# kkaytekin/Supervised-Depth-Estimation-from-Polarized-Images

Measured on AMD Instinct MI355X. Metric: train images/sec (512x612, 3-encoder), higher is better.
Workload: dtype f32; 1 GPU; BASELINE configs[2]: full 3-encoder (augment_xolp+augment_normals), multi-scale loss scales=[0,1,2,3], batch 16 per GPU, 512x612 frames (network/loss on 512x640 padded), dropout 0.1, Adam lr 1e-4, fp32; global_batch=16, height=512, width=640, frame_width=612, parallelism=dp1

## Files before the change

include/polardepth.h:

```cpp
#ifndef POLARDEPTH_H
#define POLARDEPTH_H

#include <stddef.h>
#include <stdint.h>

#ifdef __cplusplus
extern "C" {
#endif

#define PD_OK 0
#define PD_EINVAL (-22)
#define PD_ELAUNCH (-5)

const char* pd_last_error(void);
int pd_version(void);

#define PD_POLAR_LS 0
#define PD_POLAR_STOKES 1
#define PD_POLAR_PRECISE_NORMALS 1
#define PD_POLAR_IEEE_RHO 2
#define PD_POLAR_NT_LOADS 4
#define PD_POLAR_PLAIN_LOADS 8

size_t pd_polar_tables_bytes(int n_d, int n_s1, int n_s2);
int pd_polar_tables_pack(const double* x_d, const double* y_d, int n_d,
                         const double* x_s1, const double* y_s1, int n_s1,
                         const double* x_s2, const double* y_s2, int n_s2,
                         void* host_blob, size_t blob_bytes);
int pd_polar_tables_build(double n, void* host_blob, size_t blob_bytes, size_t* blob_bytes_used);

int pd_polar_fwd(const void* pol, const void* mask, void* xolp, void* xolp_std, void* normals,
                 void* ints, const void* tables, size_t tables_bytes,
                 int B, int H, int W, int Wout, int mode, int flags, void* stream);

int pd_polar_normals_from_xolp(const void* xolp, void* normals, const void* tables, size_t tables_bytes,
                               int B, int H, int W, int flags, void* stream);

int pd_polar_calc_normals(const void* phi, const void* theta, void* out, int B, long P, int phi_f64, int theta_f64,
                          void* stream);

int pd_polar_theta(const void* rho, void* theta_d, void* theta_s1, void* theta_s2, void* bins,
                   const void* tables, size_t tables_bytes, long n, void* stream);

int pd_polar_fit_matrix(const double angles_rad[4], double coef_out[12]);

#define PD_POLAR_U8 0
#define PD_POLAR_U16 1
#define PD_POLAR_F32 2
int pd_polar_general_fwd(const void* pol, int dtype, const double* coef, void* iun, void* xolp, void* xolp_std,
                         void* normals, const void* tables, size_t tables_bytes,
                         int B, int H, int W, int Wout, int flags, void* stream);

#define PD_XOLP_STATS_BYTES 4184
size_t pd_xolp_stats_workspace(int B, int H, int W);
int pd_xolp_stats(const void* xolp, const void* mask, void* stats, void* workspace, size_t ws_bytes,
                  int B, int H, int W, int ld, const float thresholds[2], int accumulate, void* stream);

#define PD_CONV_AUTO 0u
#define PD_CONV_FP32_MFMA 1u
#define PD_CONV_BF16X3 2u
#define PD_CONV_WGRAD_SPLIT_IN_REGS 4u
#define PD_CONV_GENERAL_KERNELS 8u
#define PD_CONV_X3_IM2COL 16u
#define PD_CONV_WGRAD_ROW_WORKGROUPS 32u
#define PD_CONV_BF16 128u
#define PD_CONV_FLAGS_ALL 191u
int pd_conv2d_tile_m(long M, int Cout);
long pd_conv2d_stats_rows(long M, int Cout);
int pd_conv2d_uses_x3(long M, int Cout, int C, int KH, int KW, int stride, int pad, int mode, int act, int has_out_scale,
                      int Ho, int Wo, unsigned flags);
int pd_conv2d_uses_bf16(long M, int Cout, int C, int KH, int KW, int stride, int pad, int mode, int act, int has_out_scale,
                        int Ho, int Wo, unsigned flags);
int pd_conv2d_route(long M, int Cout, int C, int KH, int KW, int stride, int pad, int mode, int act, int has_out_scale,
                    int Ho, int Wo, unsigned flags);
int pd_conv2d(const void* x, const void* w, const void* bias, const void* out_scale, void* y, void* stats,
              int N, int H, int W, int C, long sN, long sH, long sW, long sC,
              int Ho, int Wo, int Cout, int KH, int KW, int stride, int pad, int mode, int act,
              int affine, float sub, float div, long ldy, unsigned flags, void* stream);

int pd_conv16(const void* x, const void* w, const void* bias, void* y, int N, int H, int W, int C,
              long sN, long sH, long sW, int Ho, int Wo, int Cout, long ldy, int mode, int act, void* stream);

size_t pd_conv16_wgrad_workspace(int C);
int pd_conv16_wgrad(const void* x, const void* dz, void* dw, void* dbias, void* workspace, size_t ws_bytes,
                    int N, int H, int W, int C, long sN, long sH, long sW, long ldd, int accumulate, void* stream);

int pd_dgrad_s2_filters(const void* wt, void* wsub, int Cin, int Cout, void* stream);
int pd_conv2d_rect(const void* x, const void* w, void* y, int N, int H, int W, int C, long sN, long sH, long sW, long sC,
                   int Ho, int Wo, int Cout, int KH, int KW, int pad_h, int pad_w, int mode, long ldy, unsigned flags,
                   void* stream);
int pd_interleave4(const void* sub, void* dx, int N, int Ho, int Wo, int C, void* stream);

int pd_conv2d_add(const void* x, const void* w, const void* addend, long ld_add, void* y,
                  int N, int H, int W, int C, long sN, long sH, long sW, long sC,
                  int Ho, int Wo, int Cout, int KH, int KW, int stride, int pad, int mode, long ldy, unsigned flags,
                  void* stream);

size_t pd_conv2d_wgrad_workspace(long M, int Cout, int K, unsigned flags);
int pd_conv2d_wgrad(const void* x, const void* dy, void* dw, void* dbias, void* workspace, size_t ws_bytes,
                    int N, int H, int W, int C, long sN, long sH, long sW, long sC,
                    int Ho, int Wo, int Cout, int KH, int KW, int stride, int pad, int mode,
                    int affine, float sub, float div, long ldd, int accumulate, unsigned flags, void* stream);
int pd_conv2d_wgrad_uses_x3(long M, int Cout, int C, int KH, int KW, int stride, int pad, int mode, int H, int W, int Ho, int Wo,
                            unsigned flags);
int pd_conv2d_wgrad_uses_bf16(long M, int Cout, int C, int KH, int KW, int stride, int pad, int mode, int H, int W, int Ho, int Wo,
                              unsigned flags);
int pd_conv2d_wgrad_route(long M, int Cout, int C, int KH, int KW, int stride, int pad, int mode, int H, int W, int Ho, int Wo,
                          unsigned flags);

int pd_stem_s2d_input(const void* x, void* out, int N, int C, int H, int W, long sN, long sC, long sH, long sW,
                      int affine, float sub, float div, void* stream);
int pd_stem_s2d_weight(const void* w, void* w2, int Cout, int C, void* stream);
int pd_stem_s2d_weight_grad(const void* dw2, void* dw, int Cout, int C, int accumulate, void* stream);

int pd_weight_transpose(const void* w, void* wt, int Cout, int T, int Cin, void* stream);
int pd_weight_transpose_batched(const void* src, void* dst, const void* table, const void* blk, int n, int nblocks,
                                void* stream);

int pd_bn_fwd_finalize(const void* partial, long R, int C, double count, const void* gamma, const void* beta,
                       void* running_mean, void* running_var, float momentum, float eps, void* acc_ws, long acc_len,
                       void* scale, void* shift, void* save_mean, void* save_invstd, int training, void* stream);
int pd_bn_bwd_finalize(const void* partial, long R, int C, double count, void* acc_ws, long acc_len, void* dgamma,
                       void* dbeta, void* coef, int accumulate, void* stream);
long pd_chain_bwd_rows(int N, int H, int W, int C);
int pd_chain_fwd(const void* x, const void* scale, const void* shift, const void* res, void* out,
                 int N, int H, int W, int C, long ld_res, long ld_out, int relu_pre, int pool,
                 float drop_p, uint64_t seed, uint64_t offset, const void* step_state, int relu_post, void* stream);
int pd_chain_bwd_reduce(const void* dy, long ld_dy, const void* x, const void* out, long ld_out,
                        const void* scale, const void* shift, const void* mean, const void* invstd,
                        void* partial, int N, int H, int W, int C, int relu_pre, int pool, float drop_p,
                        uint64_t seed, uint64_t offset, const void* step_state, int relu_post, void* stream);
int pd_chain_bwd_apply(const void* dy, long ld_dy, const void* x, const void* out, long ld_out,
                       const void* scale, const void* shift, const void* mean, const void* invstd,
                       const void* coef, void* dx, void* dres, int N, int H, int W, int C, int relu_pre,
                       int pool, float drop_p, uint64_t seed, uint64_t offset, const void* step_state, int relu_post,
                       void* stream);

int pd_maxpool3s2_fwd(const void* x, void* y, void* idx, int N, int H, int W, int C, void* stream);
int pd_maxpool3s2_bwd(const void* idx, const void* dy, void* dx, int N, int H, int W, int C, void* stream);
int pd_maxpool3s2_bwd_add(const void* idx, const void* dy, const void* addend, long ld_add, void* dx, int N, int H, int W,
                          int C, void* stream);

int pd_upcat_fwd(const void* a, const void* skip, long ld_skip, void* out, int N, int H, int W, int Ca, int Cs,
                 void* stream);
int pd_up_bwd(const void* dout, long ld_d, void* da, int N, int H, int W, int Ca, void* stream);
int pd_up_bwd_elu(const void* dout, long ld_d, const void* elu_y, void* da, int N, int H, int W, int Ca, void* stream);

int pd_up2x_ac_fwd(const void* a, void* out, int N, int H, int W, int C, void* stream);
int pd_up2x_ac_bwd(const void* dout, void* da, int N, int H, int W, int C, void* stream);
int pd_relu_add(const void* x, const void* res, void* out, long n, int relu, void* stream);

int pd_act_bwd(const void* dy, const void* y, void* dz, long n, int act, void* stream);
int pd_reflect_fold(const void* dxp, void* dx, int N, int H, int W, int C, void* stream);
int pd_reflect_fold_pad(const void* dxp, void* dx, int N, int H, int W, int C, int pad, void* stream);
int pd_reflect_dgrad_border(const void* dz, long ldd, const void* w, void* dx, int N, int H, int W, int Cout, int Cin,
                            void* stream);
int pd_adam_step(void* p, void* g, void* m, void* v, long n, float lr, float beta1, float beta2, float eps,
                 float weight_decay, long step, const void* step_state, float grad_scale, int zero_grad, void* stream);
int pd_step_tick(void* step_state, int bump_dropout, int bump_adam, void* stream);
int pd_step_set_hyper(void* step_state, float lr, float grad_scale, void* stream);

int pd_loss_rows(long n);
int pd_disp_to_depth(const void* disp, void* depth, void* updisp, int N, int hs, int ws, int H, int W,
                     float min_depth, float max_depth, void* stream);
int pd_up_gather_bwd(const void* gup, void* gdisp, int N, int hs, int ws, int H, int W, int accumulate, int generic,
                     void* stream);
int pd_gt_normals(const void* gt, const void* K, void* gt_normals, int N, int H, int W, float min_depth, float max_depth,
                  void* stream);
int pd_sup_loss_fwd(const void* pred, const void* gt, const void* K, const void* gt_normals, void* partial, int N, int H,
                    int W, float min_depth, float max_depth, int with_normals, void* stream);
int pd_normals_loss_masked(const void* pred, const void* gt, const void* K, const void* mask, void* partial_ws, void* out,
                           int N, int H, int W, void* stream);
int pd_normals_pred_loss_fwd(const void* pred, long ld, const void* gt_normals, const void* gt, void* partial_ws, void* out,
                             int N, int H, int W, float min_depth, float max_depth, void* stream);
int pd_normals_pred_loss_bwd(const void* pred, long ld, const void* gt_normals, const void* gt, const void* gout,
                             const void* loss_count, void* dpred, long ld_dpred, int N, int H, int W, float min_depth,
                             float max_depth, void* stream);
int pd_multiscale_loss_fwd(const void* const* disps, const void* const* colors, const int* hs, const int* ws, int S,
                           const void* gt, const void* K, const void* gt_normals, void* const* depths, void* const* means,
                           void* const* edge_ws, void* sup_part, void* sm_part, int part_stride, int N, int H, int W,
                           float min_depth, float max_depth, int with_normals, void* stream);
int pd_multiscale_loss_bwd(const void* const* disps, const void* const* colors, const void* const* depths,
                           const void* const* means, const void* const* edge_ws, const int* hs, const int* ws, int S,
                           const void* gt, const void* K, const void* gt_normals, const void* wts, const void* sums,
                           void* gup_ws, void* g_ws, void* gd_acc, void* const* gdisps, int N, int H, int W,
                           float min_depth, float max_depth, void* stream);
int pd_sup_loss_bwd(const void* pred, const void* gt, const void* K, const void* gt_normals, const void* wts,
                    const void* sums, void* ab_ws, void* gout, int N, int H, int W, float min_depth, float max_depth,
                    int with_normals, int to_disp, int two_pass_form, void* stream);
int pd_smooth_fwd(const void* disp, const void* img, void* mean, void* partial, void* edge_w, int N, int h, int w,
                  void* stream);
int pd_smooth_bwd(const void* disp, const void* img, const void* mean, const void* wts, const void* edge_w, void* g_ws,
                  void* gd_acc, void* gdisp, int N, int h, int w, int accumulate, void* stream);
int pd_loss_finalize(const void* sup_part, const int* sup_rows, const void* sm_part, const int* sm_rows,
                     const int* dims, const int* scale_ids, int S, int part_stride, float w_normals,
                     float w_smooth, void* sums, void* vals, void* stream);
int pd_loss_from_sums(const void* sums, const int* dims, const int* scale_ids, int S, float w_normals,
                      float w_smooth, void* vals, void* stream);
int pd_loss_weights(const void* gvals, const int* scale_ids, int S, float w_normals, float w_smooth, void* wts,
                    void* stream);

int pd_ssim_fwd(const void* x, const void* y, void* out, int N, int C, int H, int W, int mode, int no_ssim,
                void* stream);
int pd_ssim_bwd(const void* x, const void* y, const void* gout, void* coef_ws, void* gx, void* gy, int N, int C, int H, int W,
                int mode, int no_ssim, void* stream);

#define PD_REPROJ_MAX_FRAMES 8
int pd_view_synth_fwd(const void* depth, const void* src, const void* K, const void* inv_K, const void* T, void* warped,
                      void* coords, int N, int C, int H, int W, void* stream);
int pd_view_synth_bwd(const void* gwarped, const void* src, const void* coords, const void* depth, const void* K,
                      const void* inv_K, const void* T, void* gdepth, int N, int C, int H, int W, int accumulate,
                      void* stream);
int pd_view_synth_pose_rows(int H, int W);
int pd_view_synth_bwd_pose(const void* gwarped, const void* src, const void* coords, const void* depth, const void* K,
                           const void* inv_K, const void* T, void* gdepth, void* partial_ws, void* gP, void* gT, int N, int C,
                           int H, int W, int accumulate, void* stream);
int pd_depth_to_updisp_bwd(const void* gdepth, const void* depth, void* gup, long n, float min_depth, float max_depth,
                           void* stream);
int pd_reproj_combine_rows(int N, int H, int W);
int pd_reproj_combine_fwd(const void* const* reproj, const void* const* identity, int F, const void* noise,
                          const void* valid, void* sel, void* partial_ws, void* sums, void* loss, int N, int H, int W,
                          int avg, void* stream);
int pd_reproj_combine_bwd(const void* gloss, const void* sel, const void* sums, const void* valid, void* const* greproj,
                          int F, int N, int H, int W, int avg, void* stream);

int pd_pose_matrix_fwd(const void* axisangle, const void* translation, void* T, int N, int invert, void* stream);
int pd_pose_matrix_bwd(const void* gT, const void* axisangle, const void* translation, void* gaxisangle, void* gtranslation,
                       int N, int invert, void* stream);
int pd_pose_head_fwd(const void* x, const void* w, const void* b, void* axisangle, void* translation, void* T, void* T_inv,
                     void* mean, int N, int h, int wd, int Cin, int Co, int invert, void* stream);
int pd_pose_head_bwd(const void* gT, const void* gT_inv, const void* gaxisangle, const void* gtranslation,
                     const void* axisangle, const void* translation, const void* w, const void* mean, void* gx, void* gw,
                     void* gb, void* gpre_ws, int N, int h, int wd, int Cin, int Co, int invert, int accumulate, void* stream);

int pd_cost_volume(const void* cur, const void* lookup, const void* T, const void* K, const void* inv_K, const void* bins,
                   const void* valid, void* cost, long ldc, void* missing, void* confidence, void* argmin, void* lowest,
                   int B, int F, int h, int w, int C, int D, int apply_confidence, void* stream);

#define PD_BINS_LINEAR 0
#define PD_BINS_INVERSE 1
int pd_student_masks_rows(int N, int h, int w);
int pd_student_masks(const void* lowest, const void* confidence, const void* mono_depth, const void* aug, int motion_masking,
                     void* rmask, void* cmask, void* lowest_up, void* minmax, void* partial_ws, int N, int h, int w, int H,
                     int W, void* stream);
int pd_depth_bins_update(const void* minmax, int N, void* tracker, double floor_depth, int D, int binning, void* bins,
                         void* stream);
int pd_student_combine_rows(int N, int H, int W);
int pd_student_combine_fwd(const void* const* reproj, int F, const void* valid, const void* rmask, const void* multi_depth,
                           const void* mono_depth, void* sel, void* partial_ws, void* sums, void* loss, int N, int H, int W,
                           int avg, void* stream);
int pd_student_combine_bwd(const void* gloss, const void* sel, const void* sums, const void* valid, const void* multi_depth,
                           const void* mono_depth, void* const* greproj, void* gmulti, int F, int N, int H, int W, int avg,
                           void* stream);

int pd_depth_metrics(const void* gt, const void* pred, const void* mask, int mask_value, void* partial_ws,
                     void* metrics, int N, long P, float min_depth, float max_depth, void* stream);

#define PD_NSTAT_BINS         720
#define PD_NSTAT_MAX_CLASSES  16
#define PD_NSTAT_RECORD_BYTES 2912
size_t pd_normals_stats_workspace(int N, int H, int W, int K);
int pd_normals_stats(const void* pred, long ld, const void* gtn, const void* gt, const void* mask,
                     const int* classes, int K, const void* cos_edges, int gate, void* err_deg,
                     void* stats, void* workspace, size_t ws_bytes, int N, int H, int W,
                     float min_depth, float max_depth, void* stream);

#define PD_PCD_TILE         256
#define PD_PCD_BINS         512
#define PD_PCD_MAX_CLASSES  16
#define PD_PCD_RECORD_BYTES 2096
// ... 82 lines not shown
```

supervised-depth-estimation-from-polarized-images_amd/csrc/conv.hip:

```cpp
#include "pd_common.h"
#include <cstdlib>
#include <type_traits>

namespace {

typedef float f32x16 __attribute__((ext_vector_type(16)));
typedef unsigned int u32x4 __attribute__((ext_vector_type(4)));

constexpr int BK = 32;
constexpr int LDT = BK;
constexpr int NT = 256;
constexpr unsigned OOB = 0x80000000u;

enum { MODE_ZERO = 0, MODE_REFLECT = 1, MODE_TRANSPOSED = 2 };
enum { ACT_NONE = 0, ACT_RELU = 1, ACT_ELU = 2, ACT_SIGMOID = 3 };

#define PD_I(n) std::integral_constant<int, n>{}
#define PD_SB __builtin_amdgcn_sched_barrier(0);

template <typename F> void with_mode(int mode, F&& f) {
    if (mode == MODE_ZERO) f(PD_I(MODE_ZERO)); else if (mode == MODE_REFLECT) f(PD_I(MODE_REFLECT)); else f(PD_I(MODE_TRANSPOSED));
}
template <typename F> void with_bool(bool b, F&& f) { if (b) f(std::true_type{}); else f(std::false_type{}); }

inline bool vec16_ok(const void* x, int C, long sN, long sH, long sW, long sC, int affine) {
    return (C % 4 == 0) && sC == 1 && (sW % 4 == 0) && (sH % 4 == 0) && (sN % 4 == 0) && !affine && pd::aligned16(x);
}

struct ConvArgs {
    const float* x;
    const float* w;
    const float* bias;
    const float* oscale;
    float* y;
    float* stats;
    const float* add;
    long ld_add;
    int N, H, W, C;
    long sN, sH, sW, sC;
    int Ho, Wo, Co;
    int KH, KW, stride, pad;
    int pad_w;
    int mode, act;
    int affine;
    float sub, div;
    int K;
    long M;
    long ldy;
    int mtiles, ntiles;
    int sshift;
    unsigned w_bytes;
    unsigned mg_hw, sh_hw, mg_wo, sh_wo;
    unsigned flags;
    int stats_rows;
    int nmajor;
};

__device__ __forceinline__ float4 ldg4(const float* p) { return *reinterpret_cast<const float4*>(p); }

__device__ __forceinline__ int swz(int row, int slot) { return 4 * (slot ^ ((row >> 1) & 7)); }

__device__ __forceinline__ __amdgpu_buffer_rsrc_t make_rsrc(const void* p, unsigned bytes) {
    return __builtin_amdgcn_make_buffer_rsrc(const_cast<void*>(p), 0, bytes, 0x00020000);
}
__device__ __forceinline__ float4 buf_ld4(__amdgpu_buffer_rsrc_t r, unsigned off) {
    return __builtin_bit_cast(float4, __builtin_amdgcn_raw_buffer_load_b128(r, off, 0, 0));
}
__device__ __forceinline__ float buf_ld1(__amdgpu_buffer_rsrc_t r, unsigned off) {
    return __builtin_bit_cast(float, __builtin_amdgcn_raw_buffer_load_b32(r, off, 0, 0));
}

template <int MODE>
__device__ __forceinline__ bool tap_in(int rh, int rw, int kh, int kw, int H, int W, int sshift, int& ih, int& iw) {
    if (MODE == MODE_TRANSPOSED) {
        const int th = rh - kh, tw = rw - kw;
        const int smask = (1 << sshift) - 1;
        ih = th >> sshift; iw = tw >> sshift;
        return ((th | tw) >= 0) & (((th | tw) & smask) == 0) & (ih < H) & (iw < W);
    }
    ih = rh + kh; iw = rw + kw;
    if (MODE == MODE_REFLECT) {
        ih = ih < 0 ? -ih : ih; ih = ih >= H ? 2 * H - 2 - ih : ih;
        iw = iw < 0 ? -iw : iw; iw = iw >= W ? 2 * W - 2 - iw : iw;
        return true;
    }
    return ((unsigned)ih < (unsigned)H) & ((unsigned)iw < (unsigned)W);
}

typedef __attribute__((address_space(3))) void lds_ptr_t;

__device__ __forceinline__ void dma16(__amdgpu_buffer_rsrc_t r, const void* lds_wave_base, unsigned voff) {
    const unsigned m0v = __builtin_amdgcn_readfirstlane((unsigned)(size_t)(lds_ptr_t*)lds_wave_base);
    asm volatile("s_mov_b32 m0, %0\n\ts_nop 0\n\tbuffer_load_dwordx4 %1, %2, 0 offen lds"
                 :: "s"(m0v), "v"(voff), "s"(r) : "memory");
}
__device__ __forceinline__ void dma_wait() { asm volatile("s_waitcnt vmcnt(0)" ::: "memory"); }

template <int BM, int BN, int WM, int WN, int MT, typename AccT>
__device__ __forceinline__ void conv_epilogue(const ConvArgs& a, AccT (&acc)[WM / MT][WN / MT], float* scratch, int mt,
                                              long m0, int n0, int wm, int wn, int lane, int wave, int tid) {
    constexpr int TM = WM / MT, TN = WN / MT, ACCN = MT == 32 ? 16 : 4, WAVES_N = BN / WN;
    float (*red)[WN][2] = reinterpret_cast<float (*)[WN][2]>(scratch);
    if constexpr (MT == 32 && WN == 32) {
        const bool lean = a.M - m0 >= BM && n0 + BN <= a.Co && !a.bias && !a.oscale && a.act == ACT_NONE &&
                          (a.ldy & 3) == 0 && ((size_t)a.y & 15) == 0 &&
                          (!a.add || ((a.ld_add & 3) == 0 && ((size_t)a.add & 15) == 0));
        if (lean) {
            float* T = scratch + wave * (WM * WN);
            red = reinterpret_cast<float (*)[WN][2]>(scratch + 4 * WM * WN);
            const int col_l = lane & 31, rbase = 4 * (lane >> 5);
            float4 addv[WM / 8];
            if (a.add) {
                const __amdgpu_buffer_rsrc_t ra = make_rsrc(a.add + m0 * a.ld_add, (unsigned)((long)BM * a.ld_add * 4));
                const unsigned off_a = (unsigned)((wm * WM + (lane >> 3)) * (int)a.ld_add + n0 + wn * WN + 4 * (lane & 7)) * 4u;
#pragma unroll
                for (int t = 0; t < WM / 8; ++t) addv[t] = buf_ld4(ra, off_a + (unsigned)(t * 8 * (int)a.ld_add * 4));
            }
            float s1 = 0.f, s2 = 0.f;
#pragma unroll
            for (int i = 0; i < TM; ++i)
#pragma unroll
                for (int r = 0; r < 16; ++r) {
                    const float v = acc[i][0][r];
                    T[(MT * i + (r & 3) + 8 * (r >> 2) + rbase) * WN + col_l] = v;
                    s1 += v;
                    s2 = __builtin_fmaf(v, v, s2);
                }
            const __amdgpu_buffer_rsrc_t ry = make_rsrc(a.y + m0 * a.ldy, (unsigned)((long)BM * a.ldy * 4));
            const unsigned off_l = (unsigned)((wm * WM + (lane >> 3)) * (int)a.ldy + n0 + wn * WN + 4 * (lane & 7)) * 4u;
            const float4* Tq = reinterpret_cast<const float4*>(T) + lane;
#pragma unroll
            for (int t = 0; t < WM / 8; ++t) {
                float4 v = Tq[t * 64];
                if (a.add) { v.x += addv[t].x; v.y += addv[t].y; v.z += addv[t].z; v.w += addv[t].w; }
                __builtin_amdgcn_raw_buffer_store_b128(__builtin_bit_cast(u32x4, v), ry, off_l, t * 8 * (int)a.ldy * 4, 0);
            }
            if (a.stats) {
                s1 += __shfl_xor(s1, 32); s2 += __shfl_xor(s2, 32);
                if (lane < 32) { red[wave][col_l][0] = s1; red[wave][col_l][1] = s2; }
                __syncthreads();
                if (tid < BN) {
                    const int w_n = tid / WN, cl = tid - w_n * WN;
                    float t1 = 0.f, t2 = 0.f;
#pragma unroll
                    for (int w_m = 0; w_m < BM / WM; ++w_m) {
                        t1 += red[w_m * WAVES_N + w_n][cl][0];
                        t2 += red[w_m * WAVES_N + w_n][cl][1];
                    }
                    float* o = a.stats + ((long)mt * a.Co + n0 + tid) * 2;
                    o[0] = t1; o[1] = t2;
                }
            }
            return;
        }
    }
    const int col_l = lane % MT;
    const int rbase = 4 * (lane / MT);
    {
        const long rows_left = a.M - m0;
        const int rows = rows_left < BM ? (int)rows_left : BM;
        const __amdgpu_buffer_rsrc_t ry = make_rsrc(a.y + m0 * a.ldy, (unsigned)((long)rows * a.ldy * 4));
        const __amdgpu_buffer_rsrc_t rb_ = make_rsrc(a.bias ? a.bias : a.w, a.bias ? (unsigned)a.Co * 4u : 0u);
        const __amdgpu_buffer_rsrc_t rs_ = make_rsrc(a.oscale ? a.oscale : a.w, a.oscale ? (unsigned)a.Co * 4u : 0u);
        const __amdgpu_buffer_rsrc_t ra_ = make_rsrc(a.add ? a.add + m0 * a.ld_add : a.w, a.add ? (unsigned)((long)rows * a.ld_add * 4) : 0u);
        auto body = [&](auto act_tag) {
            constexpr int ACT = decltype(act_tag)::value;
#pragma unroll
            for (int j = 0; j < TN; ++j) {
                const int col = n0 + wn * WN + MT * j + col_l;
                const bool cv = col < a.Co;
                const float bv = a.bias ? buf_ld1(rb_, cv ? (unsigned)col * 4u : OOB) : 0.f;
                const float sv = a.oscale ? buf_ld1(rs_, cv ? (unsigned)col * 4u : OOB) : 1.f;
                float s1 = 0.f, s2 = 0.f;
                const int row_l = wm * WM + rbase;
                const unsigned off_l = (unsigned)(row_l * (int)a.ldy + col) * 4u;
#pragma unroll
                for (int i = 0; i < TM; ++i) {
#pragma unroll
                    for (int r = 0; r < ACCN; ++r) {
                        const int rr = MT * i + (MT == 32 ? (r & 3) + 8 * (r >> 2) : r);
                        const bool ok = cv & (row_l < rows - rr);
                        float v = fmaf(acc[i][j][r], sv, bv);
                        const float vs = ok ? v : 0.f;
                        s1 += vs;
                        s2 += vs * vs;
                        if (ACT == ACT_RELU) v = fmaxf(v, 0.f);
                        else if (ACT == ACT_ELU) v = v > 0.f ? v : __builtin_amdgcn_exp2f(v * 1.44269504088896341f) - 1.f;
                        else if (ACT == ACT_SIGMOID) v = 1.f / (1.f + expf(-v));
                        if (a.add) v += buf_ld1(ra_, ok ? (unsigned)((row_l + rr) * (int)a.ld_add + col) * 4u : OOB);
                        __builtin_amdgcn_raw_buffer_store_b32(__builtin_bit_cast(unsigned, v), ry, ok ? off_l : OOB,
                                                              rr * (int)a.ldy * 4, 0);
                    }
                }
                if (a.stats) {
#pragma unroll
                    for (int m = MT; m < 64; m <<= 1) { s1 += __shfl_xor(s1, m); s2 += __shfl_xor(s2, m); }
                    if (lane < MT) { red[wave][MT * j + col_l][0] = s1; red[wave][MT * j + col_l][1] = s2; }
                }
            }
        };
        if (a.act == ACT_NONE) body(std::integral_constant<int, ACT_NONE>{});
        else if (a.act == ACT_RELU) body(std::integral_constant<int, ACT_RELU>{});
        else if (a.act == ACT_ELU) body(std::integral_constant<int, ACT_ELU>{});
        else body(std::integral_constant<int, ACT_SIGMOID>{});
    }
    if (a.stats) {
        __syncthreads();
        if (tid < BN) {
// ... 761 lines not shown
        const bool elu = a.act == ACT_ELU;
        const long rows_here = a.M - m0 < BM ? a.M - m0 : BM;
        const __amdgpu_buffer_rsrc_t ry = make_rsrc(a.y + m0 * a.ldy, (unsigned)(rows_here * a.ldy * 4));
        const __amdgpu_buffer_rsrc_t ra = make_rsrc(a.add ? a.add + m0 * a.ld_add : a.y, a.add ? (unsigned)(rows_here * a.ld_add * 4) : 0u);
#pragma unroll
        for (int j = 0; j < 2; ++j) {
            float4 addv[4 * RB];
            if (a.add) {
                const unsigned off_a = (unsigned)((RW * wave + (lane >> 3)) * (int)a.ld_add + n0 + 32 * j + 4 * (lane & 7)) * 4u;
#pragma unroll
                for (int t = 0; t < 4 * RB; ++t) addv[t] = buf_ld4(ra, off_a + (unsigned)(t * 8 * (int)a.ld_add * 4));
            }
            float s1 = 0.f, s2 = 0.f;
            const float bv = a.bias ? a.bias[n0 + 32 * j + col_l] : 0.f;
#pragma unroll
            for (int i = 0; i < RB; ++i)
#pragma unroll
                for (int r = 0; r < 16; ++r) {
                    const float v = (wsign ? -acc[i][j][r] : acc[i][j][r]) + bv;
                    T[(32 * i + (r & 3) + 8 * (r >> 2) + rbase) * 32 + col_l] =
                        elu ? (v > 0.f ? v : __builtin_amdgcn_exp2f(v * 1.44269504088896341f) - 1.f) : v;
                    s1 += v;
                    s2 = __builtin_fmaf(v, v, s2);
                }
            const unsigned off_l = (unsigned)((RW * wave + (lane >> 3)) * (int)a.ldy + n0 + 32 * j + 4 * (lane & 7)) * 4u;
            const float4* Tq = reinterpret_cast<const float4*>(T) + lane;
            float4 v[4 * RB];
#pragma unroll
            for (int t = 0; t < 4 * RB; ++t) {
                v[t] = Tq[t * 64];
                if (a.add) { v[t].x += addv[t].x; v[t].y += addv[t].y; v[t].z += addv[t].z; v[t].w += addv[t].w; }
            }
            __builtin_amdgcn_sched_barrier(0);
            if (rows_here == BM) {
#pragma unroll
                for (int t = 0; t < 4 * RB; ++t)
                    __builtin_amdgcn_raw_buffer_store_b128(__builtin_bit_cast(u32x4, v[t]), ry, off_l, t * 8 * (int)a.ldy * 4, 0);
            } else {
#pragma unroll
                for (int t = 0; t < 4 * RB; ++t)
                    if (RW * wave + (lane >> 3) + 8 * t < rows_here)
                        __builtin_amdgcn_raw_buffer_store_b128(__builtin_bit_cast(u32x4, v[t]), ry, off_l + (unsigned)(t * 8 * (int)a.ldy * 4), 0, 0);
            }
            asm volatile("s_nop 1");
            __builtin_amdgcn_sched_barrier(0);
            if (a.stats) {
                s1 += __shfl_xor(s1, 32); s2 += __shfl_xor(s2, 32);
                if (lane < 32) { red[wave][32 * j + col_l][0] = s1; red[wave][32 * j + col_l][1] = s2; }
            }
        }
        if (a.stats) {
            const int sgr = a.stats_rows, wps = sgr / RW, nrow = BM / sgr;
            __syncthreads();
            if (tid < nrow * BN) {
                const int row_l = tid >> 6, cl = tid & 63;
                float t1 = 0.f, t2 = 0.f;
                for (int w = 0; w < wps; ++w) { t1 += red[row_l * wps + w][cl][0]; t2 += red[row_l * wps + w][cl][1]; }
                float* o = a.stats + ((long)(mt * nrow + row_l) * a.Co + n0 + cl) * 2;
                o[0] = t1; o[1] = t2;
            }
        }
    }
}

constexpr long X3_MIN_WG = 512, X3_MIN_WG1 = 320;

static bool x3_common_ok(const ConvArgs& a, bool vec, bool has_scale) {
    const bool on = !(a.flags & PD_CONV_FP32_MFMA);
    return on && vec && a.KH * a.KW <= 31 && a.pad < a.KH && a.pad_w < a.KW &&
           (a.mode == MODE_ZERO || (a.mode == MODE_TRANSPOSED && a.sshift == 0) ||
            (a.mode == MODE_REFLECT && a.KH == 3 && a.KW == 3 && a.pad == 1 && a.pad_w == 1 && a.stride == 1 && a.Ho == a.H &&
             a.Wo == a.W && a.H >= 3 && a.W >= 3)) &&
           !has_scale && (a.act == ACT_NONE || a.act == ACT_ELU) && (a.ldy & 3) == 0 && ((size_t)a.y & 15) == 0 &&
           (!a.add || ((a.ld_add & 3) == 0 && ((size_t)a.add & 15) == 0)) && (long)a.Co * a.K * 4 < 0x7fffffffL;
}
static int x3_eligible(const ConvArgs& a) {
    const bool force = (a.flags & PD_CONV_BF16X3) != 0;
    if (!((a.C + x3::CK - 1) / x3::CK * x3::CK <= 2 * a.C && a.Co % x3::BN == 0 &&
          (a.M % 128 == 0 || (a.mode == MODE_TRANSPOSED && !a.stats))))
        return 0;
    const long ct = a.Co / x3::BN;
    if (a.M % 256 == 0 && (a.M / 256) * ct >= X3_MIN_WG) return 2;
    return (force || (a.M / 128) * ct >= X3_MIN_WG1) ? 1 : 0;
}

static int x3_nmajor(const ConvArgs& a, int ntiles) { return (long)a.Co * a.K * 4 > (3L << 20) && ntiles >= 8 && ntiles % 8 == 0; }
#include "conv_x3_halo.hpp"

enum ConvFamily { CONV_NONE = -1, CONV_GENERAL = 0, CONV_UNI = 1, CONV_X3 = 2, CONV_HALO = 3 };
struct ConvRoute {
    int family;
    int bm, bn, wm, wn;
    int mtiles, ntiles, nmajor;
    bool vec;
    int ns, rb;
    HaloPlan halo;
    int terms;
};

static ConvRoute route_conv(const ConvArgs& a, bool vec, bool has_scale) {
    ConvRoute r{};
    r.vec = vec; r.ns = 2; r.terms = 3;
    const auto tiles = [&](int family, int bm, int bn, int wm, int wn, long mtiles) {
        r.family = family; r.bm = bm; r.bn = bn; r.wm = wm; r.wn = wn;
        r.mtiles = (int)mtiles; r.ntiles = (a.Co + bn - 1) / bn;
    };
    if (x3_common_ok(a, vec, has_scale)) {
        if (!(a.flags & PD_CONV_X3_IM2COL) && x3_halo_plan(a, r.halo)) {
            tiles(CONV_HALO, 256, 32 * r.halo.ncb, 0, 0, (long)a.N * (a.Ho / (256 / r.halo.tw)) * (a.Wo / r.halo.tw));
            r.terms = (a.flags & PD_CONV_BF16) ? 1 : 3;
        } else if ((r.rb = x3_eligible(a)) != 0) {
            tiles(CONV_X3, 128 * r.rb, x3::BN, 32 * r.rb, x3::BN, (a.M + 128 * r.rb - 1) / (128 * r.rb));
        }
        if (r.rb || r.family == CONV_HALO) { r.nmajor = x3_nmajor(a, r.ntiles); return r; }
    }
    const int bm = pd_conv2d_tile_m(a.M, a.Co);
    const long mt = (a.M + bm - 1) / bm;
    if (a.Co == 96 && bm == 128) tiles(CONV_GENERAL, 128, 32, 32, 32, mt);
    else if (a.Co > 32 && bm == 128) tiles(CONV_GENERAL, 128, 64, 64, 32, mt);
    else if (a.Co > 32) tiles(CONV_GENERAL, 64, 64, 32, 32, mt);
    else if (a.Co > 16) tiles(CONV_GENERAL, 128, 32, 32, 32, mt);
    else tiles(CONV_GENERAL, 128, 16, 32, 16, mt);
    if (vec && !(a.flags & PD_CONV_GENERAL_KERNELS) && r.wn == 32 && a.C % BK == 0 && a.KH * a.KW <= 31 && a.pad < a.KH &&
        a.pad_w < a.KW && (a.mode == MODE_ZERO || a.mode == MODE_REFLECT || (a.mode == MODE_TRANSPOSED && a.sshift == 0))) {
        r.family = CONV_UNI;
        r.ns = (r.bm == 64 && a.mode != MODE_REFLECT) ? 3 : 2;
    } else if (a.pad_w != a.pad) {
        r.family = CONV_NONE;
    }
    return r;
}

template <int BM, int BN, int WM, int WN>
void launch_conv_fp32(const ConvArgs& a, const ConvRoute& r, dim3 grid, hipStream_t st) {
    const dim3 block(NT);
    constexpr bool dma = true;
    if constexpr (WN == 32)
        if (r.family == CONV_UNI) return with_mode(a.mode, [&](auto md) {
            constexpr int MD = decltype(md)::value;
            if (r.ns == 2) hipLaunchKernelGGL((conv_igemm_uni_kernel<BM, BN, WM, WN, MD, 2>), grid, block, 0, st, a);
            else if constexpr (MD != MODE_REFLECT) hipLaunchKernelGGL((conv_igemm_uni_kernel<BM, BN, WM, WN, MD, 3>), grid, block, 0, st, a);
        });
    with_mode(a.mode, [&](auto md) {
        constexpr int MD = decltype(md)::value;
        if (r.vec && dma) hipLaunchKernelGGL((conv_igemm_kernel<BM, BN, WM, WN, true, MD, true>), grid, block, 0, st, a);
        else if (r.vec) hipLaunchKernelGGL((conv_igemm_kernel<BM, BN, WM, WN, true, MD>), grid, block, 0, st, a);
        else hipLaunchKernelGGL((conv_igemm_kernel<BM, BN, WM, WN, false, MD>), grid, block, 0, st, a);
    });
}

static int launch_conv(ConvArgs& a, const ConvRoute& r, hipStream_t st) {
    a.mtiles = r.mtiles; a.ntiles = r.ntiles; a.nmajor = r.nmajor;
    const dim3 grid((unsigned)(((long)r.mtiles * r.ntiles + 7) / 8 * 8)), block(NT);
    if (r.family == CONV_HALO) {
        if (r.terms == 1) launch_conv_x3_halo<1>(a, r.halo, grid, st); else launch_conv_x3_halo<3>(a, r.halo, grid, st);
    } else if (r.family == CONV_X3) {
        with_mode(a.mode, [&](auto md) {
            constexpr int MD = decltype(md)::value;
            if (r.rb == 2) hipLaunchKernelGGL((conv_igemm_x3_kernel<MD, 2>), grid, block, 0, st, a);
            else hipLaunchKernelGGL((conv_igemm_x3_kernel<MD, 1>), grid, block, 0, st, a);
        });
    } else if (r.bn == 64 && r.bm == 128) launch_conv_fp32<128, 64, 64, 32>(a, r, grid, st);
    else if (r.bn == 64) launch_conv_fp32<64, 64, 32, 32>(a, r, grid, st);
    else if (r.bn == 32) launch_conv_fp32<128, 32, 32, 32>(a, r, grid, st);
    else launch_conv_fp32<128, 16, 32, 16>(a, r, grid, st);
    return pd::check_launch("pd_conv2d");
}

static void fill_conv_args(ConvArgs& a, int N, int H, int W, int C, long sN, long sH, long sW, long sC, int Ho, int Wo, int Co,
                           int KH, int KW, int stride, int pad, int pad_w, int mode, int act, int affine, float sub, float div,
                           long ldy, unsigned flags) {
    a.N = N; a.H = H; a.W = W; a.C = C; a.sN = sN; a.sH = sH; a.sW = sW; a.sC = sC;
    a.Ho = Ho; a.Wo = Wo; a.Co = Co; a.KH = KH; a.KW = KW; a.stride = stride; a.pad = pad; a.pad_w = pad_w;
    a.mode = mode; a.act = act; a.affine = affine; a.sub = sub; a.div = div;
    a.K = KH * KW * C; a.M = (long)N * Ho * Wo; a.ldy = ldy; a.flags = flags;
    a.sshift = 0;
    while ((1 << a.sshift) < stride) ++a.sshift;
    a.stats_rows = pd_conv2d_tile_m(a.M, Co);
    a.w_bytes = (unsigned)((long)Co * a.K * 4);
    const auto magic = [](long d, unsigned& mg, unsigned& sh) {
        if (d <= 1 || d >= (1L << 31)) { mg = 0; sh = 0; return; }
        int l = 0;
        while ((1L << l) < d) ++l;
        mg = (unsigned)((((unsigned long long)1 << (31 + l)) + (unsigned long long)d - 1) / (unsigned long long)d);
        sh = (unsigned)(l - 1);
    };
    magic((long)Ho * Wo, a.mg_hw, a.sh_hw);
    magic(Wo, a.mg_wo, a.sh_wo);
}
static bool conv_vec(const ConvArgs& a) { return vec16_ok(a.x, a.C, a.sN, a.sH, a.sW, a.sC, a.affine) && pd::aligned16(a.w); }

}

extern "C" int pd_conv2d_route(long M, int Co, int C, int KH, int KW, int stride, int pad, int mode, int act,
                               int has_out_scale, int Ho, int Wo, unsigned flags) {
    if (!pd::conv_flags_ok(flags)) flags &= ~PD_CONV_BF16;
    const bool grid = Ho > 0 && Wo > 0;
    const int H = grid ? Ho : 3, W = grid ? Wo : 3;
    ConvArgs a{};
    fill_conv_args(a, grid ? (int)(M / ((long)H * W)) : 1, H, W, C, (long)H * W * C, (long)W * C, C, 1, H, W, Co, KH, KW, stride, pad, pad,
                   mode, act, 0, 0.f, 1.f, Co, flags);
    a.M = M; a.stats_rows = pd_conv2d_tile_m(M, Co);
    const ConvRoute r = route_conv(a, conv_vec(a), has_out_scale != 0);
    return (r.family == CONV_HALO && r.terms == 1 ? 4 : r.family) | r.bn << 4 | r.bm << 12;
}

extern "C" int pd_conv2d_uses_x3(long M, int Co, int C, int KH, int KW, int stride, int pad, int mode, int act,
                                 int has_out_scale, int Ho, int Wo, unsigned flags) {
    const int r = pd_conv2d_route(M, Co, C, KH, KW, stride, pad, mode, act, has_out_scale, Ho, Wo, flags), family = r & 15;
    return family >= CONV_HALO ? 3 : family == CONV_X3 ? (r >> 12) / 128 : 0;
}

extern "C" int pd_conv2d_uses_bf16(long M, int Co, int C, int KH, int KW, int stride, int pad, int mode, int act,
                                   int has_out_scale, int Ho, int Wo, unsigned flags) {
    return (pd_conv2d_route(M, Co, C, KH, KW, stride, pad, mode, act, has_out_scale, Ho, Wo, flags) & 15) == 4 ? 3 : 0;
}

extern "C" int pd_conv2d_tile_m(long M, int Co) {
    if (Co <= 32) return 128;
    return M >= 64 * 1024 ? 128 : 64;
}

extern "C" long pd_conv2d_stats_rows(long M, int Co) {
    const int bm = pd_conv2d_tile_m(M, Co);
    return (M + bm - 1) / bm;
}

static int conv2d_impl(const void* x, const void* w, const void* bias, const void* out_scale, void* y, void* stats,
                       const void* addend, long ld_add,
                       int N, int H, int W, int C, long sN, long sH, long sW, long sC,
                       int Ho, int Wo, int Co, int KH, int KW, int stride, int pad, int mode, int act,
                       int affine, float sub, float div, long ldy, unsigned flags, void* stream, int pad_w = -1) {
    if (pad_w < 0) pad_w = pad;
    PD_REQUIRE(pd::conv_flags_ok(flags), "pd_conv2d: bad flags 0x%x", flags);
    PD_REQUIRE(x && w && y, "pd_conv2d: null tensor");
    PD_REQUIRE(N >= 0 && H > 0 && W > 0 && C > 0 && Ho > 0 && Wo > 0 && Co > 0, "pd_conv2d: bad dims");
    PD_REQUIRE(KH > 0 && KW > 0 && stride > 0 && pad >= 0, "pd_conv2d: bad filter geometry");
    PD_REQUIRE(mode >= 0 && mode <= 2 && act >= 0 && act <= 3, "pd_conv2d: bad mode/act");
    PD_REQUIRE(mode != MODE_REFLECT || (pad < H && pad < W), "pd_conv2d: reflect pad must be < input size");
    PD_REQUIRE(ldy >= Co && ldy < (1L << 22), "pd_conv2d: bad output row stride %ld (Cout=%d)", ldy, Co);
    if (mode == MODE_TRANSPOSED) {
        PD_REQUIRE((stride & (stride - 1)) == 0, "pd_conv2d: transposed mode needs a power-of-two stride");
        PD_REQUIRE(H <= (Ho + 2 * pad - KH) / stride + 1 && W <= (Wo + 2 * pad_w - KW) / stride + 1,
                   "pd_conv2d: transposed: x grid exceeds the forward output grid of a %dx%d input", Ho, Wo);
    } else {
        PD_REQUIRE(Ho <= (H + 2 * pad - KH) / stride + 1 && Wo <= (W + 2 * pad_w - KW) / stride + 1,
                   "pd_conv2d: output grid does not match input/filter geometry");
    }
    if (N == 0) return PD_OK;
    ConvArgs a;
    a.x = (const float*)x; a.w = (const float*)w; a.bias = (const float*)bias; a.oscale = (const float*)out_scale; a.y = (float*)y; a.stats = (float*)stats;
    a.add = (const float*)addend; a.ld_add = ld_add;
    fill_conv_args(a, N, H, W, C, sN, sH, sW, sC, Ho, Wo, Co, KH, KW, stride, pad, pad_w, mode, act, affine, sub, div, ldy, flags);
    PD_REQUIRE((long)Co * a.K * 4 < 0x7fffffffL, "pd_conv2d: weight tensor too large for 32-bit offsets");
    const long span = 256 / ((long)Ho * Wo) + 2;
    PD_REQUIRE(span * sN * 4 < 0x7fffffffL, "pd_conv2d: image too large for 32-bit offsets (%ld bytes per image)", sN * 4);
    const ConvRoute r = route_conv(a, conv_vec(a), out_scale != nullptr);
    if (r.family == CONV_NONE) return pd::fail(PD_EINVAL, "pd_conv2d_rect: shape outside the uniform-tap kernel (C %% 32, 16-byte aligned NHWC)");
    return launch_conv(a, r, (hipStream_t)stream);
}

extern "C" int pd_conv2d(const void* x, const void* w, const void* bias, const void* out_scale, void* y, void* stats,
                         int N, int H, int W, int C, long sN, long sH, long sW, long sC,
                         int Ho, int Wo, int Co, int KH, int KW, int stride, int pad, int mode, int act,
                         int affine, float sub, float div, long ldy, unsigned flags, void* stream) {
    return conv2d_impl(x, w, bias, out_scale, y, stats, nullptr, 0, N, H, W, C, sN, sH, sW, sC, Ho, Wo, Co, KH, KW, stride,
                       pad, mode, act, affine, sub, div, ldy, flags, stream);
}

extern "C" int pd_conv2d_add(const void* x, const void* w, const void* addend, long ld_add, void* y,
                             int N, int H, int W, int C, long sN, long sH, long sW, long sC,
                             int Ho, int Wo, int Co, int KH, int KW, int stride, int pad, int mode, long ldy, unsigned flags,
                             void* stream) {
    PD_REQUIRE(addend && ld_add >= Co, "pd_conv2d_add: bad addend");
    return conv2d_impl(x, w, nullptr, nullptr, y, nullptr, addend, ld_add, N, H, W, C, sN, sH, sW, sC, Ho, Wo, Co, KH, KW,
                       stride, pad, mode, ACT_NONE, 0, 0.f, 1.f, ldy, flags, stream);
}

extern "C" int pd_conv2d_rect(const void* x, const void* w, void* y, int N, int H, int W, int C, long sN, long sH, long sW,
                              long sC, int Ho, int Wo, int Co, int KH, int KW, int pad_h, int pad_w, int mode, long ldy,
                              unsigned flags, void* stream) {
    PD_REQUIRE(pad_w >= 0 && mode != MODE_REFLECT, "pd_conv2d_rect: bad padding / mode");
    PD_REQUIRE(!(flags & PD_CONV_GENERAL_KERNELS), "pd_conv2d_rect: the general kernel has no separate column padding");
    return conv2d_impl(x, w, nullptr, nullptr, y, nullptr, nullptr, 0, N, H, W, C, sN, sH, sW, sC, Ho, Wo, Co, KH, KW, 1,
                       pad_h, mode, ACT_NONE, 0, 0.f, 1.f, ldy, flags, stream, pad_w);
}

namespace {

constexpr int WG_K = 128;
constexpr int WG_MC = 32;
constexpr int WG_LDX = WG_K + 8;

struct WgradArgs {
    const float* x;
    const float* dy;
    float* part;
    float* bpart;
    int N, H, W, C;
    long sN, sH, sW, sC;
    int Ho, Wo, Co;
    int KH, KW, stride, pad, mode;
    int affine;
    float sub, div;
    int K;
    long M, ldd;
    long mper;
    int S, ktiles, ctiles;
};

template <int TCO, bool VEC, int MODE>
__global__ __launch_bounds__(NT) void conv_wgrad_kernel(const WgradArgs a) {
    constexpr int LDD = TCO + 8;
    constexpr int MT = TCO == 16 ? 16 : 32;
    constexpr int ACCN = MT == 32 ? 16 : 4;
    constexpr int WAVES_CO = TCO / MT;
    constexpr int WAVES_K = 4 / WAVES_CO;
    constexpr int TK = WG_K / WAVES_K / MT;
    constexpr int DY_ITERS = (WG_MC * TCO / 4 + NT - 1) / NT;
    constexpr int DY_PPR = TCO / 4;
    constexpr bool DY_ALL = WG_MC * TCO / 4 >= NT;
    __shared__ __attribute__((aligned(16))) float Ds[2][WG_MC][LDD];
    __shared__ __attribute__((aligned(16))) float Xs[2][WG_MC][WG_LDX];
    __shared__ int ktab[VEC ? 1 : WG_K][3];

    const int tid = threadIdx.x, lane = tid & 63, wave = tid >> 6;
    const int wm = wave / WAVES_K, wn = wave - wm * WAVES_K;
    const int nwg = a.ktiles * a.ctiles * a.S;
    int b = ((int)blockIdx.x & 7) * ((int)gridDim.x >> 3) + ((int)blockIdx.x >> 3);
    if (b >= nwg) return;
    const int kt = b % a.ktiles; b /= a.ktiles;
    const int ct = b % a.ctiles; b /= a.ctiles;
    const int s = b;
    const int co0 = ct * TCO, k0 = kt * WG_K;
    const long mbeg = (long)s * a.mper;
    const long mend = (mbeg + a.mper < a.M) ? mbeg + a.mper : a.M;
    const int nrows = (int)(mend - mbeg);
    const int nchunks = nrows > 0 ? (nrows + WG_MC - 1) / WG_MC : 0;
    const int hw = a.Ho * a.Wo;

    const int img0 = (int)(mbeg / hw);
    const long rest = ((long)a.N - img0) * a.sN * 4;
    const __amdgpu_buffer_rsrc_t rx = make_rsrc(a.x + (long)img0 * a.sN, rest > 0x7fffffffL ? 0x7fffffffu : (unsigned)rest);
    const long dbytes = (long)nrows * a.ldd * 4;
    const __amdgpu_buffer_rsrc_t rd = make_rsrc(a.dy + mbeg * a.ldd, dbytes > 0 ? (unsigned)dbytes : 0u);

    int vkh = 0, vkw = 0, vc = 0; bool vkv = false;
    if (VEC) {
        const int k = k0 + 4 * (tid & 31);
        vkv = k < a.K;
        const int tap = k / a.C;
        vc = k - tap * a.C; vkh = tap / a.KW; vkw = tap - vkh * a.KW;
    } else {
        if (tid < WG_K) {
            const int k = k0 + tid;
            const int tap = k / a.C;
            const int kh = tap / a.KW;
            ktab[tid][0] = k < a.K ? kh : -1; ktab[tid][1] = tap - kh * a.KW; ktab[tid][2] = (k - tap * a.C) * (int)a.sC;
        }
        __syncthreads();
    }
    constexpr int XR = VEC ? 4 : 1;
    int rb[XR], rloc[XR];
    int roh[XR], row_[XR];
    for (int i = 0; i < XR; ++i) {
        rloc[i] = VEC ? (tid >> 5) + 8 * i : (tid >> 3);
        const int m = (int)(mbeg - (long)img0 * hw) + rloc[i];
        const int n = m / hw;
        const int rem = m - n * hw;
        roh[i] = rem / a.Wo; row_[i] = rem - roh[i] * a.Wo;
        rb[i] = n * (int)a.sN;
    }
    constexpr bool INC = VEC && MODE == MODE_ZERO;
    int xih[INC ? XR : 1], xiw[INC ? XR : 1], xoff[INC ? XR : 1];
    const int c_w = WG_MC * a.stride, c_wo = c_w * (int)a.sW;
    const int c_row = a.Wo * a.stride, c_rowo = a.stride * (int)a.sH - c_row * (int)a.sW;
    const int c_img = a.Ho * a.stride, c_imgo = (int)a.sN - c_img * (int)a.sH;
    if (INC) {
        for (int i = 0; i < XR; ++i) {
            xih[i] = roh[i] * a.stride - a.pad + vkh;
            xiw[i] = row_[i] * a.stride - a.pad + vkw;
            xoff[i] = rb[i] + xih[i] * (int)a.sH + xiw[i] * (int)a.sW + vc;
        }
    }
    auto advance = [&](int i) {
        rloc[i] += WG_MC;
        row_[i] += WG_MC;
        if (INC) { xiw[i] += c_w; xoff[i] += c_wo; }
        while (row_[i] >= a.Wo) {
            row_[i] -= a.Wo;
            if (INC) { xiw[i] -= c_row; xih[i] += a.stride; xoff[i] += c_rowo; }
            if (++roh[i] == a.Ho) {
                roh[i] = 0; rb[i] += (int)a.sN;
                if (INC) { xih[i] -= c_img; xoff[i] += c_imgo; }
            }
        }
    };

    float4 pd[DY_ITERS], px[VEC ? 4 : 1];
    float sx[VEC ? 1 : 16];

    auto load_chunk = [&](int q) {
        const int rbase = q * WG_MC;
#pragma unroll
        for (int i = 0; i < DY_ITERS; ++i) {
            const int r = rbase + tid / DY_PPR + (NT / DY_PPR) * i;
            const int co = co0 + 4 * (tid % DY_PPR);
            const unsigned off = (unsigned)(r * (int)a.ldd + co) * 4u;
            if (!DY_ALL && tid >= WG_MC * DY_PPR) {
                pd[i] = make_float4(0.f, 0.f, 0.f, 0.f);
            } else if ((a.Co & 3) == 0) {
                pd[i] = buf_ld4(rd, (r < nrows && co < a.Co) ? off : OOB);
            } else {
                float4 v;
                v.x = buf_ld1(rd, (r < nrows && co < a.Co) ? off : OOB);
                v.y = buf_ld1(rd, (r < nrows && co + 1 < a.Co) ? off + 4 : OOB);
                v.z = buf_ld1(rd, (r < nrows && co + 2 < a.Co) ? off + 8 : OOB);
                v.w = buf_ld1(rd, (r < nrows && co + 3 < a.Co) ? off + 12 : OOB);
                pd[i] = v;
            }
        }
        if (VEC) {
#pragma unroll
            for (int i = 0; i < 4; ++i) {
                if (INC) {
                    const bool ok = ((unsigned)xih[i] < (unsigned)a.H) & ((unsigned)xiw[i] < (unsigned)a.W) & vkv & (rloc[i] < nrows);
                    px[i] = buf_ld4(rx, ok ? (unsigned)xoff[i] * 4u : OOB);
                } else {
                    int ih, iw;
// ... 600 lines not shown
                    fa[g][blk][t] = *reinterpret_cast<const u32x4*>(lds_c + pa_off + (BUF * P_BYTES + (unsigned)((t * 2 + g) * 2) * 1024u + blk * 512u));
#pragma unroll
        for (int e = 0; e < 8; ++e) x1[e] = *reinterpret_cast<const float*>(lds_c + fx_off + (BUF * X_BYTES + (unsigned)(8 + e) * 2 * X_ROW));
#pragma unroll
        for (int e = 0; e < 8; ++e) dv[e] = *reinterpret_cast<const float*>(lds_c + sd_off + (NXT * D_BYTES + (unsigned)e * 2 * D_ROW));
        x3::Terms t0, t1, td;
        auto mm = [&](const x3::Terms& t, auto g_tag, auto n_tag) {
            constexpr int G = decltype(g_tag)::value, N = decltype(n_tag)::value, T = N / 2, BLK = N % 2;
            const unsigned* bv = T < 3 ? t.h : T < 5 ? t.m : t.l;
            const u32x4 av = T == 0 ? fa[G][BLK][0] : T == 1 ? fa[G][BLK][1] : T == 2 ? fa[G][BLK][2] : T == 3 ? fa[G][BLK][0] : T == 4 ? fa[G][BLK][1] : fa[G][BLK][0];
            acc[BLK] = __builtin_amdgcn_mfma_f32_32x32x16_bf16(bf(av), bf(u32x4{bv[0], bv[1], bv[2], bv[3]}), acc[BLK], 0, 0, 0);
        };
        x3::sp_h<0>(x0, t0); x3::sp_h<1>(x0, t0); x3::sp_h<2>(x0, t0); x3::sp_h<3>(x0, t0);
        PD_SB
#define PD_XP(j) if constexpr (SPREAD) load_x_piece(nxt, PD_I(j));
#define PD_DP(j) if constexpr (SPREAD) load_d_piece(buf_tag, PD_I(j));
        mm(t0, PD_I(0), PD_I(0)); x3::sp_m<0>(x0, t0); PD_XP(0) PD_SB
        mm(t0, PD_I(0), PD_I(1)); x3::sp_m<1>(x0, t0); PD_XP(1) PD_SB
        mm(t0, PD_I(0), PD_I(2)); x3::sp_m<2>(x0, t0); PD_XP(2) PD_SB
        mm(t0, PD_I(0), PD_I(3)); x3::sp_m<3>(x0, t0); PD_XP(3) PD_SB
        mm(t0, PD_I(0), PD_I(4)); x3::sp_h<0>(dv, td); x3::sp_h<1>(dv, td); x3::sp_h<2>(dv, td); x3::sp_h<3>(dv, td); PD_DP(0) PD_SB
        mm(t0, PD_I(0), PD_I(5)); x3::sp_m<0>(dv, td); PD_DP(1) PD_SB
#undef PD_XP
#undef PD_DP
        mm(t0, PD_I(0), PD_I(6)); x3::sp_l<0>(t0); x3::sp_h<0>(x1, t1); PD_SB
        mm(t0, PD_I(0), PD_I(7)); x3::sp_l<1>(t0); x3::sp_h<1>(x1, t1); PD_SB
        mm(t0, PD_I(0), PD_I(8)); x3::sp_l<2>(t0); x3::sp_h<2>(x1, t1); PD_SB
        mm(t0, PD_I(0), PD_I(9)); x3::sp_l<3>(t0); x3::sp_h<3>(x1, t1); PD_SB
        mm(t0, PD_I(0), PD_I(10)); x3::sp_m<1>(dv, td); PD_SB
        mm(t0, PD_I(0), PD_I(11)); x3::sp_m<2>(dv, td); PD_SB
        mm(t1, PD_I(1), PD_I(0)); x3::sp_m<0>(x1, t1); PD_SB
        mm(t1, PD_I(1), PD_I(1)); x3::sp_m<1>(x1, t1); PD_SB
        mm(t1, PD_I(1), PD_I(2)); x3::sp_m<2>(x1, t1); PD_SB
        mm(t1, PD_I(1), PD_I(3)); x3::sp_m<3>(x1, t1); PD_SB
        mm(t1, PD_I(1), PD_I(4)); x3::sp_m<3>(dv, td); PD_SB
        mm(t1, PD_I(1), PD_I(5)); x3::sp_l<0>(td); x3::sp_l<1>(td); PD_SB
        mm(t1, PD_I(1), PD_I(6)); x3::sp_l<0>(t1); PD_SB
        mm(t1, PD_I(1), PD_I(7)); x3::sp_l<1>(t1); PD_SB
        mm(t1, PD_I(1), PD_I(8)); x3::sp_l<2>(t1); PD_SB
        mm(t1, PD_I(1), PD_I(9)); x3::sp_l<3>(t1); PD_SB
        mm(t1, PD_I(1), PD_I(10)); x3::sp_l<2>(td); x3::sp_l<3>(td); PD_SB
        mm(t1, PD_I(1), PD_I(11));
        if constexpr (BIAS) bsum += ((dv[0] + dv[1]) + (dv[2] + dv[3])) + ((dv[4] + dv[5]) + (dv[6] + dv[7]));
        *reinterpret_cast<u32x4*>(lds_c + sp_off + (NXT * P_BYTES + 0 * 4096u)) = u32x4{td.h[0], td.h[1], td.h[2], td.h[3]};
        *reinterpret_cast<u32x4*>(lds_c + sp_off + (NXT * P_BYTES + 1 * 4096u)) = u32x4{td.m[0], td.m[1], td.m[2], td.m[3]};
        *reinterpret_cast<u32x4*>(lds_c + sp_off + (NXT * P_BYTES + 2 * 4096u)) = u32x4{td.l[0], td.l[1], td.l[2], td.l[3]};
        dma_wait();
        __syncthreads();
    };

    {
        const std::integral_constant<unsigned, 0> d0{};
        const std::integral_constant<unsigned, 1> d1{};
        load_x_all(d0);
        load_d(d0);
        load_d(d1);
        dma_wait();
        __syncthreads();
        split_d(d0);
        __syncthreads();
    }
    for (int q = 0; q < nchunks; q += 2) {
        chunk(std::integral_constant<unsigned, 0>{});
        if (q + 1 < nchunks) chunk(std::integral_constant<unsigned, 1>{});
        if ((q & (FLUSH - 2)) == FLUSH - 2) flush();
    }
    flush();

#pragma unroll
    for (int blk = 0; blk < 2; ++blk) {
        const int k = k0 + wave * 32 + fi;
#pragma unroll
        for (int r = 0; r < 16; ++r) {
            const int co = co0 + 32 * blk + (r & 3) + 8 * (r >> 2) + 4 * fk;
            if (co < a.Co && k < a.K) a.part[((long)s * a.Co + co) * a.K + k] = acc_sum[blk][r];
        }
    }
    if constexpr (BIAS) {
        if (do_bias) {
            float* red = smem_all;
            red[wave * 64 + lane] = bsum;
            __syncthreads();
            if (tid < 64 && co0 + tid < a.Co) a.bpart[(long)s * a.Co + co0 + tid] = (red[tid] + red[64 + tid]) + (red[128 + tid] + red[192 + tid]);
        }
    }
}

#include "conv_wgrad_halo.hpp"
#include "conv_wgrad_roll.hpp"

__global__ __launch_bounds__(256) void reduce_rows_kernel(const float* __restrict__ part, float* __restrict__ out,
                                                          int S, long n, int accumulate) {
    __shared__ float red[4][64];
    const int col = threadIdx.x & 63, sl = threadIdx.x >> 6;
    const long i = blockIdx.x * 64L + col;
    float a0 = 0.f, a1 = 0.f, a2 = 0.f, a3 = 0.f;
    if (i < n) {
        int j = sl;
        for (; j + 12 < S; j += 16) {
            a0 += part[(long)j * n + i];
            a1 += part[(long)(j + 4) * n + i];
            a2 += part[(long)(j + 8) * n + i];
            a3 += part[(long)(j + 12) * n + i];
        }
        for (; j < S; j += 4) a0 += part[(long)j * n + i];
    }
    red[sl][col] = (a0 + a1) + (a2 + a3);
    __syncthreads();
    if (sl == 0 && i < n) {
        const float s = (red[0][col] + red[1][col]) + (red[2][col] + red[3][col]);
        out[i] = accumulate ? out[i] + s : s;
    }
}

__global__ __launch_bounds__(256) void weight_transpose_kernel(const float* __restrict__ w, float* __restrict__ wt,
                                                               int Co, int T, int Ci) {
    const long n = (long)Co * T * Ci;
    for (long i = blockIdx.x * 256L + threadIdx.x; i < n; i += (long)gridDim.x * 256) {
        const int co = (int)(i % Co);
        const long r = i / Co;
        const int t = (int)(r % T);
        const int ci = (int)(r / T);
        wt[i] = w[((long)co * T + t) * Ci + ci];
    }
}

__global__ __launch_bounds__(256) void weight_transpose_batched_kernel(const float* __restrict__ src, float* __restrict__ dst,
                                                                       const int* __restrict__ table,
                                                                       const int* __restrict__ blk, int n) {
    __shared__ float tile[32][33];
    int lo = 0, hi = n;
    while (hi - lo > 1) {
        const int mid = (lo + hi) >> 1;
        if (blk[mid] <= (int)blockIdx.x) lo = mid; else hi = mid;
    }
    const int off = table[4 * lo], Co = table[4 * lo + 1], T = table[4 * lo + 2], Ci = table[4 * lo + 3];
    const float* w = src + off;
    float* wt = dst + off;
    int lb = (int)blockIdx.x - blk[lo];
    const int tiles_ci = (Ci + 31) >> 5, tiles_co = (Co + 31) >> 5;
    const int ci0 = (lb % tiles_ci) << 5; lb /= tiles_ci;
    const int co0 = (lb % tiles_co) << 5;
    const int t = lb / tiles_co;
    const int x = threadIdx.x & 31, y = threadIdx.x >> 5;
#pragma unroll
    for (int r = y; r < 32; r += 8)
        if (co0 + r < Co && ci0 + x < Ci) tile[r][x] = w[((long)(co0 + r) * T + t) * Ci + ci0 + x];
    __syncthreads();
#pragma unroll
    for (int r = y; r < 32; r += 8)
        if (ci0 + r < Ci && co0 + x < Co) wt[((long)(ci0 + r) * T + t) * Co + co0 + x] = tile[x][r];
}

inline int wgrad_tco(int Co) { return Co > 32 ? 64 : (Co > 16 ? 32 : 16); }

inline bool wgrad_x3c_enabled(unsigned flags) { return !(flags & (PD_CONV_FP32_MFMA | PD_CONV_WGRAD_SPLIT_IN_REGS)); }
inline bool wgrad_x3_on(unsigned flags) { return (flags & PD_CONV_WGRAD_SPLIT_IN_REGS) && !(flags & PD_CONV_FP32_MFMA); }

void wgrad_plan(long M, int Co, int K, unsigned flags, int* S, long* mper) {
    const int tco = wgrad_tco(Co);
    const long tiles = (long)((Co + tco - 1) / tco) * ((K + WG_K - 1) / WG_K);
    const bool x3c = tco == 64 && wgrad_x3c_enabled(flags) && !(flags & PD_CONV_GENERAL_KERNELS);
    const long total = x3c ? (512 / tiles < 4 ? 1536 : M >= (1L << 20) ? 1024 : 512) : (tiles <= 32 ? 768 : 1536);
    long s = total / tiles;
    const long smax = (M + 511) / 512;
    if (s > smax) s = smax;
    if (s < 1) s = 1;
    long per = (M + s - 1) / s;
    per = (per + WG_MC - 1) / WG_MC * WG_MC;
    s = (M + per - 1) / per;
    if (s < 1) s = 1;
    *S = (int)s; *mper = per;
}

inline bool wgrad_halo_enabled(unsigned flags) { return wgrad_x3c_enabled(flags) && !(flags & (PD_CONV_GENERAL_KERNELS | PD_CONV_X3_IM2COL)); }

static int wgrad_rows_cap(long M, int Co, int K, unsigned flags) {
    int S; long mper;
    wgrad_plan(M, Co, K, flags, &S, &mper);
    if (!wgrad_halo_enabled(flags)) return S;
    const long own = std::min<long>(std::max(wgrad_halo_slices_bound(Co, K), wgrad_roll_slices_bound(Co, K)), (M + 63) / 64);
    return S > own ? S : (int)own;
}

enum WgradFamily { WGRAD_GENERAL = 0, WGRAD_UNI, WGRAD_UNI_X3, WGRAD_X3C, WGRAD_HALO, WGRAD_ROLL };
struct WgradRoute {
    int family;
    int rows;
    int tco, S; long mper;
    bool vec, row8;
    int nb, nbw;
    bool bf16;
    WgradHaloPlan halo;
    WgradRollPlan roll;
};

static WgradRoute route_wgrad(const WgradArgs& a, bool vec, unsigned flags) {
    WgradRoute r{};
    r.vec = vec; r.tco = wgrad_tco(a.Co);
    wgrad_plan(a.M, a.Co, a.K, flags, &r.S, &r.mper);
    r.rows = r.S;
    const bool refl_ok = a.mode == MODE_REFLECT && a.pad == 1 && a.KH == 3 && a.KW == 3 && a.stride == 1 && a.Ho == a.H && a.Wo == a.W && a.H >= 3;
    if (!(a.mode == MODE_ZERO || refl_ok)) return r;
    if (wgrad_halo_enabled(flags) && wgrad_halo_eligible(a, vec)) {
        r.bf16 = (flags & PD_CONV_BF16) != 0;
        const int cap = wgrad_rows_cap(a.M, a.Co, a.K, flags);
        if (!(flags & PD_CONV_WGRAD_ROW_WORKGROUPS) && wgrad_roll_eligible(a, vec, cap, r.roll)) {
            r.family = WGRAD_ROLL; r.rows = r.roll.S;
        } else {
            r.family = WGRAD_HALO; wgrad_halo_plan(a, cap, r.halo); r.rows = r.halo.S * r.halo.rps;
        }
        return r;
    }
    r.nb = (a.pad + a.stride - 1) / a.stride; r.nbw = (r.nb + 1) / 2;
    if (!(flags & PD_CONV_GENERAL_KERNELS) && (r.tco == 64 || r.tco == 32) && vec && a.Co % 4 == 0 && a.Wo % 2 == 0 && a.ldd % 4 == 0 &&
        a.Ho >= 2 * r.nb && a.Wo >= 4 * r.nbw && a.Wo >= 14 && (2 * r.nb + 1) * (2 * r.nbw + 1) <= 31 && r.mper % WG_MC == 0 &&
        a.M % 4 == 0 && a.K >= 4) {
        r.family = r.tco == 32 ? WGRAD_UNI : wgrad_x3c_enabled(flags) ? WGRAD_X3C : wgrad_x3_on(flags) ? WGRAD_UNI_X3 : WGRAD_UNI;
        r.row8 = a.Wo % 8 == 0 && r.mper % 8 == 0 && a.M % 8 == 0;
    }
    return r;
}

static int launch_wgrad_slices(const WgradArgs& a, const WgradRoute& r, bool bias, hipStream_t st) {
    const dim3 grid((unsigned)(((long)a.ktiles * a.ctiles * a.S + 7) / 8 * 8)), block(NT);
    const bool reflect = a.mode == MODE_REFLECT;
    if (r.family == WGRAD_GENERAL) {
        const auto gen = [&](auto tco) { with_bool(r.vec, [&](auto v) { with_bool(reflect, [&](auto refl) {
            hipLaunchKernelGGL((conv_wgrad_kernel<decltype(tco)::value, decltype(v)::value, decltype(refl)::value ? MODE_REFLECT : MODE_ZERO>), grid, block, 0, st, a);
        }); }); };
        if (r.tco == 64) gen(PD_I(64)); else if (r.tco == 32) gen(PD_I(32)); else gen(PD_I(16));
        return PD_OK;
    }
    WgradUniArgs ua; ua.g = a; ua.nb = r.nb; ua.nbw = r.nbw;
    if (r.family == WGRAD_X3C) {
        static const hipError_t lds_ok = [] {
            hipError_t e = hipSuccess;
            for (const void* f : {reinterpret_cast<const void*>(conv_wgrad_x3c_kernel<true, true>), reinterpret_cast<const void*>(conv_wgrad_x3c_kernel<false, true>),
                                  reinterpret_cast<const void*>(conv_wgrad_x3c_kernel<true, false>), reinterpret_cast<const void*>(conv_wgrad_x3c_kernel<false, false>),
                                  reinterpret_cast<const void*>(conv_wgrad_x3c_kernel<true, false, true>), reinterpret_cast<const void*>(conv_wgrad_x3c_kernel<false, false, true>)}) {
                const hipError_t rc = hipFuncSetAttribute(f, hipFuncAttributeMaxDynamicSharedMemorySize, x3c::LDS_BYTES);
                if (rc != hipSuccess) e = rc;
            }
            return e;
        }();
        PD_REQUIRE(lds_ok == hipSuccess, "pd_conv2d_wgrad: cannot reserve %u bytes of LDS", x3c::LDS_BYTES);
        with_bool(bias, [&](auto b) {
            constexpr bool B = decltype(b)::value;
            if (reflect) hipLaunchKernelGGL((conv_wgrad_x3c_kernel<B, false, true>), grid, block, x3c::LDS_BYTES, st, ua);
            else if (r.row8) hipLaunchKernelGGL((conv_wgrad_x3c_kernel<B, true>), grid, block, x3c::LDS_BYTES, st, ua);
            else hipLaunchKernelGGL((conv_wgrad_x3c_kernel<B, false>), grid, block, x3c::LDS_BYTES, st, ua);
        });
    } else if (r.tco == 32) {
        with_bool(reflect, [&](auto refl) { hipLaunchKernelGGL((conv_wgrad_uni_kernel<decltype(refl)::value, true, 32>), grid, block, 0, st, ua); });
    } else {
        with_bool(reflect, [&](auto refl) { with_bool(bias, [&](auto b) {
            constexpr bool R = decltype(refl)::value, B = decltype(b)::value;
            if (r.family == WGRAD_UNI_X3) hipLaunchKernelGGL((conv_wgrad_uni_kernel<R, B, 64, true>), grid, block, 0, st, ua);
            else hipLaunchKernelGGL((conv_wgrad_uni_kernel<R, B>), grid, block, 0, st, ua);
        }); });
    }
    return PD_OK;
}

static void fill_wgrad_args(WgradArgs& a, int N, int H, int W, int C, long sN, long sH, long sW, long sC, int Ho, int Wo, int Co,
                            int KH, int KW, int stride, int pad, int mode, int affine, float sub, float div, long ldd) {
    a.N = N; a.H = H; a.W = W; a.C = C; a.sN = sN; a.sH = sH; a.sW = sW; a.sC = sC;
    a.Ho = Ho; a.Wo = Wo; a.Co = Co; a.KH = KH; a.KW = KW; a.stride = stride; a.pad = pad; a.mode = mode;
    a.affine = affine; a.sub = sub; a.div = div;
    a.K = KH * KW * C; a.M = (long)N * Ho * Wo; a.ldd = ldd;
}

}

extern "C" size_t pd_conv2d_wgrad_workspace(long M, int Co, int K, unsigned flags) {
    const size_t rows = (size_t)wgrad_rows_cap(M, Co, K, flags);
    return (rows * Co * K + rows * Co) * sizeof(float);
}

extern "C" int pd_conv2d_wgrad_route(long M, int Co, int C, int KH, int KW, int stride, int pad, int mode, int H, int W, int Ho,
                                     int Wo, unsigned flags) {
    if (Ho <= 0 || Wo <= 0) return 1 << 4;
    if (!pd::conv_flags_ok(flags)) flags &= ~PD_CONV_BF16;
    WgradArgs a{};
    fill_wgrad_args(a, std::max(1, (int)(M / ((long)Ho * Wo))), H, W, C, (long)H * W * C, (long)W * C, C, 1, Ho, Wo, Co, KH, KW, stride,
                    pad, mode, 0, 0.f, 1.f, Co);
    a.M = M;
    const WgradRoute r = route_wgrad(a, vec16_ok(a.x, C, a.sN, a.sH, a.sW, a.sC, a.affine), flags);
    const int code = r.family == WGRAD_ROLL ? 3 : r.family == WGRAD_HALO ? 2 : r.family == WGRAD_X3C ? 1 : 0;
    return code | (r.bf16 ? 4 : 0) | r.rows << 4;
}

extern "C" int pd_conv2d_wgrad_uses_x3(long M, int Co, int C, int KH, int KW, int stride, int pad, int mode, int H, int W, int Ho,
                                       int Wo, unsigned flags) {
    return pd_conv2d_wgrad_route(M, Co, C, KH, KW, stride, pad, mode, H, W, Ho, Wo, flags) & 3;
}

extern "C" int pd_conv2d_wgrad_uses_bf16(long M, int Co, int C, int KH, int KW, int stride, int pad, int mode, int H, int W, int Ho,
                                         int Wo, unsigned flags) {
    const int r = pd_conv2d_wgrad_route(M, Co, C, KH, KW, stride, pad, mode, H, W, Ho, Wo, flags);
    return r & 4 ? r & 3 : 0;
}

extern "C" int pd_conv2d_wgrad(const void* x, const void* dy, void* dw, void* dbias, void* workspace, size_t ws_bytes,
                               int N, int H, int W, int C, long sN, long sH, long sW, long sC,
                               int Ho, int Wo, int Co, int KH, int KW, int stride, int pad, int mode,
                               int affine, float sub, float div, long ldd, int accumulate, unsigned flags, void* stream) {
    PD_REQUIRE(x && dy && dw && workspace, "pd_conv2d_wgrad: null tensor");
    PD_REQUIRE(pd::conv_flags_ok(flags), "pd_conv2d_wgrad: bad flags 0x%x", flags);
    PD_REQUIRE(mode == MODE_ZERO || mode == MODE_REFLECT, "pd_conv2d_wgrad: mode must be 0 or 1");
    PD_REQUIRE(Ho <= (H + 2 * pad - KH) / stride + 1 && Wo <= (W + 2 * pad - KW) / stride + 1,
               "pd_conv2d_wgrad: output grid does not match input/filter geometry");
    PD_REQUIRE(ldd >= Co && (ldd % 4 == 0 || Co < 4) , "pd_conv2d_wgrad: bad dy row stride");
    if (N == 0) return PD_OK;
    WgradArgs a;
    a.x = (const float*)x; a.dy = (const float*)dy;
    fill_wgrad_args(a, N, H, W, C, sN, sH, sW, sC, Ho, Wo, Co, KH, KW, stride, pad, mode, affine, sub, div, ldd);
    const size_t need = pd_conv2d_wgrad_workspace(a.M, Co, a.K, flags);
    PD_REQUIRE(ws_bytes >= need, "pd_conv2d_wgrad: workspace too small (%zu < %zu)", ws_bytes, need);
    PD_REQUIRE(pd::aligned16(dy) && (ldd % 4 == 0 || Co < 4), "pd_conv2d_wgrad: dy must be 16-byte aligned rows");
    const WgradRoute r = route_wgrad(a, vec16_ok(x, C, sN, sH, sW, sC, affine), flags);
    const int cap = wgrad_rows_cap(a.M, Co, a.K, flags);
    PD_REQUIRE(r.rows <= cap, "pd_conv2d_wgrad: %d partial rows planned, the workspace holds %d", r.rows, cap);
    a.S = r.S; a.mper = r.mper;
    PD_REQUIRE(a.mper * ldd * 4 < 0x7fffffffL, "pd_conv2d_wgrad: slice too large for 32-bit offsets");
    PD_REQUIRE((a.mper / ((long)Ho * Wo) + 2) * sN * 4 < 0x7fffffffL, "pd_conv2d_wgrad: image too large for 32-bit offsets");
    a.part = (float*)workspace;
    a.bpart = dbias ? a.part + (size_t)r.rows * Co * a.K : nullptr;
    a.ktiles = (a.K + WG_K - 1) / WG_K; a.ctiles = (Co + r.tco - 1) / r.tco;
    hipStream_t st = (hipStream_t)stream;
    if (r.family == WGRAD_ROLL) launch_wgrad_roll(a, r.roll, st, dbias != nullptr, r.bf16);
    else if (r.family == WGRAD_HALO) launch_wgrad_halo(a, r.halo, st, dbias != nullptr, r.bf16);
    else if (int rc = launch_wgrad_slices(a, r, dbias != nullptr, st)) return rc;
    if (int rc = pd::check_launch("pd_conv2d_wgrad")) return rc;
    const long nw = (long)Co * a.K;
    hipLaunchKernelGGL(reduce_rows_kernel, dim3((unsigned)((nw + 63) / 64)), dim3(256), 0, st, a.part, (float*)dw, r.rows, nw, accumulate);
    if (dbias)
        hipLaunchKernelGGL(reduce_rows_kernel, dim3((unsigned)((Co + 63) / 64)), dim3(256), 0, st, a.bpart, (float*)dbias, r.rows, (long)Co, accumulate);
    return pd::check_launch("pd_conv2d_wgrad/reduce");
}

extern "C" int pd_weight_transpose(const void* w, void* wt, int Co, int T, int Ci, void* stream) {
    PD_REQUIRE(w && wt && Co > 0 && T > 0 && Ci > 0, "pd_weight_transpose: bad arguments");
    const long n = (long)Co * T * Ci;
    const long blocks = (n + 255) / 256;
    hipLaunchKernelGGL(weight_transpose_kernel, dim3((unsigned)(blocks > 4096 ? 4096 : blocks)), dim3(256), 0,
                       (hipStream_t)stream, (const float*)w, (float*)wt, Co, T, Ci);
    return pd::check_launch("pd_weight_transpose");
}

extern "C" int pd_weight_transpose_batched(const void* src, void* dst, const void* table, const void* blk, int n,
                                           int nblocks, void* stream) {
    PD_REQUIRE(src && dst && table && blk && n > 0 && nblocks > 0, "pd_weight_transpose_batched: bad arguments");
    hipLaunchKernelGGL(weight_transpose_batched_kernel, dim3((unsigned)nblocks), dim3(256), 0, (hipStream_t)stream,
                       (const float*)src, (float*)dst, (const int*)table, (const int*)blk, n);
    return pd::check_launch("pd_weight_transpose_batched");
}

namespace {
__global__ __launch_bounds__(256) void dgrad_s2_filters_kernel(const float* __restrict__ wt, float* __restrict__ wsub,
                                                               int Ci, int Co) {
    const long cc = (long)Ci * Co, total = 9 * cc;
    for (long i = blockIdx.x * 256L + threadIdx.x; i < total; i += (long)gridDim.x * 256) {
        const int cls = i < cc ? 0 : i < 3 * cc ? 1 : i < 5 * cc ? 2 : 3, ph = cls >> 1, pw = cls & 1;
        const long base = cc * (cls == 0 ? 0 : cls == 1 ? 1 : cls == 2 ? 3 : 5);
        long r = i - base;
        const int co = (int)(r % Co); r /= Co;
        const int kw2 = pw ? (int)(r & 1) : 0; r >>= pw;
        const int kh2 = ph ? (int)(r & 1) : 0; r >>= ph;
        const int ci = (int)r;
        const int kh = ph ? (kh2 ? 2 : 0) : 1, kw = pw ? (kw2 ? 2 : 0) : 1;
        wsub[i] = wt[(((long)ci * 3 + kh) * 3 + kw) * Co + co];
    }
}
__global__ __launch_bounds__(256) void interleave4_kernel(const float* __restrict__ sub, float* __restrict__ dx, int N, int Ho,
                                                          int Wo, int C) {
    const int cq = C >> 2;
    const long per = (long)N * Ho * Wo * cq, total = 4 * per;
    for (long i = blockIdx.x * 256L + threadIdx.x; i < total; i += (long)gridDim.x * 256) {
        const int c4 = (int)(i % cq) * 4;
        long r = i / cq;
        const int pw = (int)(r & 1); r >>= 1;
        const int j = (int)(r % Wo); r /= Wo;
        const int ph = (int)(r & 1); r >>= 1;
        const int ii = (int)(r % Ho);
        const long n = r / Ho;
        const float4 v = ldg4(sub + ((long)(ph * 2 + pw) * N * Ho * Wo + (n * Ho + ii) * (long)Wo + j) * C + c4);
        *reinterpret_cast<float4*>(dx + ((n * 2 * Ho + 2 * ii + ph) * (long)(2 * Wo) + 2 * j + pw) * C + c4) = v;
    }
}
}

extern "C" int pd_dgrad_s2_filters(const void* wt, void* wsub, int Ci, int Co, void* stream) {
    PD_REQUIRE(wt && wsub && Ci > 0 && Co > 0, "pd_dgrad_s2_filters: bad arguments");
    const long total = 9L * Ci * Co, blocks = (total + 255) / 256;
    hipLaunchKernelGGL(dgrad_s2_filters_kernel, dim3((unsigned)(blocks > 2048 ? 2048 : blocks)), dim3(256), 0,
                       (hipStream_t)stream, (const float*)wt, (float*)wsub, Ci, Co);
    return pd::check_launch("pd_dgrad_s2_filters");
}

extern "C" int pd_interleave4(const void* sub, void* dx, int N, int Ho, int Wo, int C, void* stream) {
    PD_REQUIRE(sub && dx && N > 0 && Ho > 0 && Wo > 0 && C > 0 && C % 4 == 0, "pd_interleave4: bad arguments");
    const long total = 4L * N * Ho * Wo * (C / 4), blocks = (total + 255) / 256;
    hipLaunchKernelGGL(interleave4_kernel, dim3((unsigned)(blocks > 8192 ? 8192 : blocks)), dim3(256), 0,
                       (hipStream_t)stream, (const float*)sub, (float*)dx, N, Ho, Wo, C);
    return pd::check_launch("pd_interleave4");
}

namespace {

__global__ __launch_bounds__(256) void s2d_input_kernel(const float* __restrict__ x, float* __restrict__ out, int N,
                                                        int C, int H, int W, long sN, long sC, long sH, long sW,
                                                        int affine, float sub, float div) {
    const int H2 = H >> 1, W2 = W >> 1, C4 = 4 * C;
    const long total = (long)N * H2 * W2 * C4;
    for (long i = blockIdx.x * 256L + threadIdx.x; i < total; i += (long)gridDim.x * 256) {
        const int q = (int)(i % C4);
        long pix = i / C4;
        const int j = (int)(pix % W2); pix /= W2;
        const int ii = (int)(pix % H2);
        const long n = pix / H2;
        const int d = q / C, c = q - d * C;
        float v = x[n * sN + c * sC + (2 * ii + (d >> 1)) * sH + (2 * j + (d & 1)) * sW];
        if (affine) v = (v - sub) / div;
        out[i] = v;
    }
}

__global__ __launch_bounds__(256) void s2d_weight_kernel(const float* __restrict__ w, float* __restrict__ w2, int Co,
                                                         int C, int inverse, int accumulate, float* __restrict__ dw) {
    const int C4 = 4 * C;
    const long total = (long)Co * 16 * C4;
    for (long i = blockIdx.x * 256L + threadIdx.x; i < total; i += (long)gridDim.x * 256) {
        const int q = (int)(i % C4);
        long r = i / C4;
        const int b = (int)(r & 3); r >>= 2;
        const int a = (int)(r & 3);
        const long co = r >> 2;
        const int d = q / C, c = q - d * C;
        const int kh = 2 * a + (d >> 1) - 1, kw = 2 * b + (d & 1) - 1;
        const bool ok = kh >= 0 && kw >= 0;
        const long src = ((co * 7 + kh) * 7 + kw) * C + c;
        if (!inverse) w2[i] = ok ? w[src] : 0.f;
        else if (ok) dw[src] = (accumulate ? dw[src] : 0.f) + w2[i];
    }
}

constexpr int S2D_TW = 64;
__global__ __launch_bounds__(256) void s2d_input_tile_kernel(const float* __restrict__ x, float* __restrict__ out, int N,
                                                             int C, int H, int W, long sN, long sC, long sH, int affine,
                                                             float sub, float div, int tiles_w) {
    extern __shared__ float s2d_lds[];
    const int H2 = H >> 1, W2 = W >> 1, C4 = 4 * C, LDP = C4 + 1;
    const int tw = blockIdx.x % tiles_w;
    long r = blockIdx.x / tiles_w;
    const int ii = (int)(r % H2);
    const long n = r / H2;
    const int j0 = tw * S2D_TW, nj = min(S2D_TW, W2 - j0);
    const float* xb = x + n * sN + (long)(2 * ii) * sH + 2 * j0;
    for (int e = threadIdx.x; e < 2 * C * 2 * S2D_TW; e += 256) {
        const int col = e & (2 * S2D_TW - 1), cd = e >> 7;
        const int dy = cd & 1, c = cd >> 1;
        const int j = col >> 1, dx = col & 1;
        if (j < nj) {
            float v = xb[c * sC + dy * sH + col];
            if (affine) v = (v - sub) / div;
            s2d_lds[j * LDP + (dy * 2 + dx) * C + c] = v;
        }
    }
    __syncthreads();
    float* ob = out + ((n * H2 + ii) * (long)W2 + j0) * C4;
    for (int t = threadIdx.x; t < nj * C4; t += 256) {
        const int j = t / C4, q = t - j * C4;
        ob[t] = s2d_lds[j * LDP + q];
    }
}

}

extern "C" int pd_stem_s2d_input(const void* x, void* out, int N, int C, int H, int W, long sN, long sC, long sH,
                                 long sW, int affine, float sub, float div, void* stream) {
    PD_REQUIRE(x && out && N >= 0 && C > 0 && H > 0 && W > 0 && H % 2 == 0 && W % 2 == 0, "pd_stem_s2d_input: bad arguments");
    if (N == 0) return PD_OK;
    const long total = (long)N * H * W * C;
    const int tiles_w = (W / 2 + S2D_TW - 1) / S2D_TW;
    const long blocks = (long)N * (H / 2) * tiles_w;
    const size_t lds = (size_t)S2D_TW * (4 * C + 1) * sizeof(float);
    if (sW == 1 && lds <= 48 * 1024 && blocks < (1L << 31)) {
        hipLaunchKernelGGL(s2d_input_tile_kernel, dim3((unsigned)blocks), dim3(256), lds, (hipStream_t)stream, (const float*)x,
                           (float*)out, N, C, H, W, sN, sC, sH, affine, sub, div, tiles_w);
        return pd::check_launch("pd_stem_s2d_input");
    }
    hipLaunchKernelGGL(s2d_input_kernel, dim3((unsigned)((total + 255) / 256 > 8192 ? 8192 : (total + 255) / 256)), dim3(256),
                       0, (hipStream_t)stream, (const float*)x, (float*)out, N, C, H, W, sN, sC, sH, sW, affine, sub, div);
    return pd::check_launch("pd_stem_s2d_input");
}

extern "C" int pd_stem_s2d_weight(const void* w, void* w2, int Co, int C, void* stream) {
    PD_REQUIRE(w && w2 && Co > 0 && C > 0, "pd_stem_s2d_weight: bad arguments");
    const long total = (long)Co * 64 * C;
    hipLaunchKernelGGL(s2d_weight_kernel, dim3((unsigned)((total + 255) / 256)), dim3(256), 0, (hipStream_t)stream,
                       (const float*)w, (float*)w2, Co, C, 0, 0, (float*)nullptr);
    return pd::check_launch("pd_stem_s2d_weight");
}

extern "C" int pd_stem_s2d_weight_grad(const void* dw2, void* dw, int Co, int C, int accumulate, void* stream) {
    PD_REQUIRE(dw2 && dw && Co > 0 && C > 0, "pd_stem_s2d_weight_grad: bad arguments");
    const long total = (long)Co * 64 * C;
    hipLaunchKernelGGL(s2d_weight_kernel, dim3((unsigned)((total + 255) / 256)), dim3(256), 0, (hipStream_t)stream,
                       (const float*)nullptr, (float*)dw2, Co, C, 1, accumulate, (float*)dw);
    return pd::check_launch("pd_stem_s2d_weight_grad");
// ... 2 lines not shown
```

supervised-depth-estimation-from-polarized-images_amd/csrc/conv_x3_halo.hpp:

```cpp
namespace x3h {
constexpr int CK = 16;
template <int KH, int KW, int TW, int NCB, int TERMS = 3> struct Geo {
    static constexpr int TR = 256 / TW, BR = 32 / TW;
    static constexpr int HW = TW + KW - 1, HH = TR + KH - 1, HP = HW * HH;
    static constexpr unsigned BP_BYTES = 32 * NCB * CK * 2;
    static constexpr int NI = (HP * 4 + NT - 1) / NT;
    static constexpr unsigned AP_BYTES = TERMS * 2 * HP * 16;
    static constexpr unsigned BP_BASE = AP_BYTES;
    static constexpr unsigned EPI_BYTES = 4 * 64 * 32 * 4 + 4 * 64 * 2 * 4;
    static constexpr unsigned PLANE_BYTES = BP_BASE + 2 * TERMS * BP_BYTES;
    static constexpr unsigned LDS_BYTES = PLANE_BYTES > EPI_BYTES ? PLANE_BYTES : EPI_BYTES;
};
}

template <int MODE, int KH, int KW, int TW, int NCB, bool ROWWIN, int TERMS = 3>
__global__ __launch_bounds__(NT, 3) void conv_halo_x3_kernel(const ConvArgs a) {
    using namespace x3h;
    using G = Geo<KH, KW, TW, NCB, TERMS>;
    static_assert(TERMS == 1 || TERMS == 3, "bf16 terms per operand");
    constexpr int HW = G::HW, HP = G::HP, NI = G::NI, T = KH * KW, TR = G::TR, BR = G::BR, BNW = 32 * NCB;
    constexpr unsigned BP_BASE = G::BP_BASE, BP_BYTES = G::BP_BYTES;
    static_assert(!ROWWIN || (KW == 1 && MODE == MODE_ZERO), "row windows: zero padding, the filter row folded into the channels");
    __shared__ __attribute__((aligned(16))) float smem_all[G::LDS_BYTES / 4];

    const int tiles_w = a.Wo / TW, tiles_h = a.Ho / TR;
    const int ntile_m = a.N * tiles_h * tiles_w;
    const int nblk = ntile_m * a.ntiles;
    const int per_xcd = (int)gridDim.x >> 3;
    const int logical = ((int)blockIdx.x & 7) * per_xcd + ((int)blockIdx.x >> 3);
    if (logical >= nblk) return;
    const int mt = a.nmajor ? logical % ntile_m : logical / a.ntiles, nt = a.nmajor ? logical / ntile_m : logical - mt * a.ntiles;
    const int n0 = nt * BNW;
    const int img = mt / (tiles_h * tiles_w);
    const int trem = mt - img * (tiles_h * tiles_w);
    const int ty = trem / tiles_w, tx = trem - ty * tiles_w;
    const int oy0 = ty * TR, ox0 = tx * TW;
    const unsigned wsign = (mt & 1) ? 0x80008000u : 0u;

    const int tid = threadIdx.x;
    const int lane = tid & 63;
    const int wave = __builtin_amdgcn_readfirstlane(tid >> 6);
    const int padh = MODE == MODE_TRANSPOSED ? KH - 1 - a.pad : a.pad, padw = MODE == MODE_TRANSPOSED ? KW - 1 - a.pad_w : a.pad_w;

    const int by = oy0 - padh, bx = ox0 - padw;
    const long base_f = (long)by * a.sH + (long)bx * a.sW;
    const long left_bytes = ((long)a.sN - base_f) * 4;
    constexpr long XSPAN = ROWWIN ? 0xffff0L : 0x3fffc0L;
    const __amdgpu_buffer_rsrc_t rx = make_rsrc(a.x + (long)img * a.sN + base_f, (unsigned)(left_bytes < XSPAN ? left_bytes : XSPAN));
    const __amdgpu_buffer_rsrc_t rw_ = make_rsrc(a.w, a.w_bytes);

    unsigned hpk[(NI + 1) / 2];
    unsigned hmask = 0;
    const int hquad = tid & 3;
    const unsigned hdst0 = (unsigned)(((hquad >> 1) * HP + (tid >> 2)) * 16 + (hquad & 1) * 8);
    const bool hlast_ok = (tid >> 2) + 64 * (NI - 1) < HP;
    static_assert(64 * (NI - 1) < HP, "only the last halo item of a thread may be empty");
    const int sH16 = (int)a.sH >> (ROWWIN ? 2 : 4), sW16 = (int)a.sW >> (ROWWIN ? 2 : 4);
#pragma unroll
    for (int i = 0; i < NI; ++i) {
        const int p = (tid >> 2) + 64 * i;
        const int hy = p / HW, hx = p - hy * HW;
        int iy = by + hy, ix = bx + hx;
        if constexpr (MODE == MODE_REFLECT) {
            iy = iy < 0 ? -iy : iy; iy = iy >= a.H ? 2 * a.H - 2 - iy : iy;
            ix = ix < 0 ? -ix : ix; ix = ix >= a.W ? 2 * a.W - 2 - ix : ix;
        }
        bool ok = p < HP && (unsigned)iy < (unsigned)a.H;
        if constexpr (ROWWIN) {
            const int lo = ix < 0 ? -ix : 0, hi = ix + a.KW > a.W ? ix + a.KW - a.W : 0;
            ok = ok && lo < a.KW && hi < a.KW;
            hmask |= (unsigned)((lo & 3) | ((hi & 3) << 2)) << (4 * i);
        } else {
            ok = ok && (unsigned)ix < (unsigned)a.W;
        }
        const unsigned u = ok ? (unsigned)((iy - by) * sH16 + (ix - bx) * sW16) : 0xffffu;
        if (i & 1) hpk[i >> 1] |= u << 16; else hpk[i >> 1] = u;
    }
    const unsigned hq16 = 16u * (unsigned)hquad;
    const bool border_tile = ROWWIN && (tx == 0 || tx == tiles_w - 1);
    const int srow = NCB == 2 ? tid >> 2 : tid >> 3, sls = NCB == 2 ? tid & 3 : tid & 7;
    const unsigned vb = (unsigned)((n0 + srow) * a.K) * 4u + (NCB == 2 ? 16u : 8u) * (unsigned)sls;

    const int ngroups = (ROWWIN ? a.KW * a.C : a.C) / CK;
    const unsigned tap_bytes = (unsigned)(ROWWIN ? a.KW * a.C : a.C) * 4u;
    const int nchunks = ngroups * T;
    int s_qb = 0, sb_tap = 0;
    unsigned s_boff = 0, sb_c4 = 0;
    float4 wq;
    float2 wq2[2];
    auto load_b = [&](auto set_tag) {
        if constexpr (NCB == 2) {
            wq = __builtin_bit_cast(float4, __builtin_amdgcn_raw_buffer_load_b128(rw_, vb, s_qb < nchunks ? s_boff : 0u, 0));
        } else {
            wq2[decltype(set_tag)::value] = __builtin_bit_cast(float2, __builtin_amdgcn_raw_buffer_load_b64(rw_, vb, s_qb < nchunks ? s_boff : 0u, 0));
        }
        ++s_qb;
        s_boff += tap_bytes;
        if (++sb_tap == T) { sb_tap = 0; sb_c4 += CK * 4; s_boff = sb_c4; }
    };

    const int frow = lane & 31, fh = lane >> 5;
    const unsigned fa_base = (unsigned)((fh * HP + (2 * wave * BR + frow / TW) * HW + frow % TW) * 16);
    unsigned fb_off = BP_BASE + (unsigned)frow * (CK * 2) + 16u * (fh ^ ((frow >> 3) & 1));
    asm volatile("" : "+v"(fb_off));
    const unsigned sp_off = NCB == 2 ? BP_BASE + (unsigned)srow * (CK * 2) + 16u * ((sls >> 1) ^ ((srow >> 3) & 1)) + 8u * (sls & 1)
                                     : BP_BASE + (unsigned)srow * (CK * 2) + 16u * ((sls >> 2) ^ ((srow >> 3) & 1)) + 4u * (sls & 3);
    char* lds_c = reinterpret_cast<char*>(smem_all);

    typedef float accv_t __attribute__((ext_vector_type(16)));
    accv_t acc[2][NCB];
#pragma unroll
    for (int i = 0; i < 2; ++i)
#pragma unroll
        for (int j = 0; j < NCB; ++j)
#pragma unroll
            for (int r = 0; r < 16; ++r) acc[i][j][r] = 0.f;
    auto bf = [](u32x4 v) { return __builtin_bit_cast(x3::bf16x8, v); };

    float4 hv[NI];
    auto halo_load = [&](int g) {
        if constexpr (ROWWIN) {
            if (border_tile) {
                const int f = g * CK + 4 * hquad;
#pragma unroll
                for (int i = 0; i < NI; ++i) {
                    const unsigned u = (i & 1) ? hpk[i >> 1] >> 16 : hpk[i >> 1] & 0xffffu;
                    const int lo = (int)((hmask >> (4 * i)) & 3u) * a.C, hi = (a.KW - (int)((hmask >> (4 * i + 2)) & 3u)) * a.C;
                    hv[i] = __builtin_bit_cast(float4, __builtin_amdgcn_raw_buffer_load_b128(
                        rx, (f >= lo && f < hi) ? (u << 4) + hq16 : OOB, g * (CK * 4), 0));
                }
                return;
            }
        }
#pragma unroll
        for (int i = 0; i < NI; ++i)
            hv[i] = __builtin_bit_cast(float4, __builtin_amdgcn_raw_buffer_load_b128(
                rx, (((i & 1) ? hpk[i >> 1] >> 16 : hpk[i >> 1] & 0xffffu) << (ROWWIN ? 4 : 6)) + hq16, g * (CK * 4), 0));
    };

    auto split_b0 = [&]() {
        const float4 w4 = NCB == 2 ? wq : make_float4(wq2[0].x, wq2[0].y, 0.f, 0.f);
        uint2 h, m, l;
        if constexpr (TERMS == 1) {
            h.x = x3::cvt_pk_bf16(w4.x, w4.y);
            if constexpr (NCB == 2) {
                h.y = x3::cvt_pk_bf16(w4.z, w4.w);
                *reinterpret_cast<uint2*>(lds_c + sp_off) = uint2{h.x ^ wsign, h.y ^ wsign};
            } else {
                *reinterpret_cast<unsigned*>(lds_c + sp_off) = h.x ^ wsign;
            }
            return;
        }
        x3::split2(w4.x, w4.y, h.x, m.x, l.x);
        if constexpr (NCB == 2) {
            x3::split2(w4.z, w4.w, h.y, m.y, l.y);
            *reinterpret_cast<uint2*>(lds_c + sp_off + 0 * BP_BYTES) = uint2{h.x ^ wsign, h.y ^ wsign};
            *reinterpret_cast<uint2*>(lds_c + sp_off + 1 * BP_BYTES) = uint2{m.x ^ wsign, m.y ^ wsign};
            *reinterpret_cast<uint2*>(lds_c + sp_off + 2 * BP_BYTES) = uint2{l.x ^ wsign, l.y ^ wsign};
        } else {
            *reinterpret_cast<unsigned*>(lds_c + sp_off + 0 * BP_BYTES) = h.x ^ wsign;
            *reinterpret_cast<unsigned*>(lds_c + sp_off + 1 * BP_BYTES) = m.x ^ wsign;
            *reinterpret_cast<unsigned*>(lds_c + sp_off + 2 * BP_BYTES) = l.x ^ wsign;
        }
    };
    auto halo_item = [&](auto i_tag) {
        constexpr int I = decltype(i_tag)::value;
        if constexpr (I < NI && TERMS == 1) {
            const uint2 h = {x3::cvt_pk_bf16(hv[I].x, hv[I].y), x3::cvt_pk_bf16(hv[I].z, hv[I].w)};
            if (I < NI - 1 || hlast_ok) *reinterpret_cast<uint2*>(lds_c + hdst0 + 1024u * I) = h;
        } else if constexpr (I < NI) {
            uint2 h, m, l;
            x3::split2(hv[I].x, hv[I].y, h.x, m.x, l.x);
            x3::split2(hv[I].z, hv[I].w, h.y, m.y, l.y);
            if (I < NI - 1 || hlast_ok) {
                *reinterpret_cast<uint2*>(lds_c + hdst0 + (1024u * I + 0 * (2 * HP * 16))) = h;
                *reinterpret_cast<uint2*>(lds_c + hdst0 + (1024u * I + 1 * (2 * HP * 16))) = m;
                *reinterpret_cast<uint2*>(lds_c + hdst0 + (1024u * I + 2 * (2 * HP * 16))) = l;
            }
        }
    };
    auto halo_split = [&]() {
        halo_item(PD_I(0)); halo_item(PD_I(1)); halo_item(PD_I(2)); halo_item(PD_I(3)); halo_item(PD_I(4)); halo_item(PD_I(5)); halo_item(PD_I(6));
    };

    int s_kh = 0, s_kw = 0, s_g = 0;

    auto chunk = [&](auto buf_tag) {
        constexpr unsigned BUF = decltype(buf_tag)::value, NXT = BUF ^ 1;
        const bool LAST = s_kh == KH - 1 && s_kw == KW - 1 && s_g + 1 < ngroups;
        const bool halo_issue = (s_kh | s_kw) == 0 && s_g + 1 < ngroups;
        float ws[4];
        if constexpr (NCB == 2) {
            asm volatile("" : "+v"(wq.x), "+v"(wq.y), "+v"(wq.z), "+v"(wq.w));
            ws[0] = wq.x; ws[1] = wq.y; ws[2] = wq.z; ws[3] = wq.w;
        } else {
            asm volatile("" : "+v"(wq2[NXT].x), "+v"(wq2[NXT].y));
            ws[0] = wq2[NXT].x; ws[1] = wq2[NXT].y; ws[2] = 0.f; ws[3] = 0.f;
        }
        if (halo_issue) halo_load(s_g + 1);
        const int ey = MODE == MODE_TRANSPOSED ? KH - 1 - s_kh : s_kh, ex = MODE == MODE_TRANSPOSED ? KW - 1 - s_kw : s_kw;
        const unsigned fa = fa_base + (unsigned)((ey * HW + ex) * 16);
        if constexpr (TERMS == 1) {
            u32x4 a1[2], b1[NCB];
#pragma unroll
            for (int i = 0; i < 2; ++i) a1[i] = *reinterpret_cast<const u32x4*>(lds_c + fa + (unsigned)(i * BR * HW * 16));
#pragma unroll
            for (int j = 0; j < NCB; ++j)
                b1[j] = *reinterpret_cast<const u32x4*>(lds_c + fb_off + (BUF * BP_BYTES + (unsigned)j * 32 * CK * 2));
            if (LAST) __syncthreads();
#pragma unroll
            for (int j = 0; j < NCB; ++j)
#pragma unroll
                for (int i = 0; i < 2; ++i)
                    acc[i][j] = __builtin_amdgcn_mfma_f32_32x32x16_bf16(bf(a1[i]), bf(b1[j]), acc[i][j], 0, 0, 0);
            if constexpr (NCB == 2) {
                const uint2 h = {x3::cvt_pk_bf16(ws[0], ws[1]), x3::cvt_pk_bf16(ws[2], ws[3])};
                load_b(std::integral_constant<int, 0>{});
                *reinterpret_cast<uint2*>(lds_c + sp_off + NXT * BP_BYTES) = uint2{h.x ^ wsign, h.y ^ wsign};
            } else {
                const unsigned h = x3::cvt_pk_bf16(ws[0], ws[1]);
                load_b(std::integral_constant<int, (int)NXT>{});
                *reinterpret_cast<unsigned*>(lds_c + sp_off + NXT * BP_BYTES) = h ^ wsign;
            }
            if (LAST) {
                halo_item(PD_I(0)); halo_item(PD_I(1)); halo_item(PD_I(2)); halo_item(PD_I(3)); halo_item(PD_I(4)); halo_item(PD_I(5)); halo_item(PD_I(6));
            }
            static_assert(NI <= 7, "halo items per thread");
            if (++s_kw == KW) { s_kw = 0; if (++s_kh == KH) { s_kh = 0; ++s_g; } }
            __syncthreads();
            return;
        }
        u32x4 av[2][3], fb[NCB][3];
#pragma unroll
        for (int i = 0; i < 2; ++i)
#pragma unroll
            for (int t = 0; t < 3; ++t)
                av[i][t] = *reinterpret_cast<const u32x4*>(lds_c + fa + (unsigned)((t * 2 * HP + i * BR * HW) * 16));
        auto load_fb = [&](int j, int t) { fb[j][t] = *reinterpret_cast<const u32x4*>(lds_c + fb_off + ((BUF * 3 + t) * BP_BYTES + (unsigned)j * 32 * CK * 2)); };
        load_fb(0, 0); load_fb(0, 1);
        if constexpr (NCB == 2) { load_fb(1, 0); load_fb(1, 1); }
        if (LAST) __syncthreads();
        x3::Terms tw;
        auto mm = [&](auto i_tag, auto n_tag) {
            constexpr int I = decltype(i_tag)::value, N = decltype(n_tag)::value, TT = N / NCB, J = N % NCB;
            constexpr int TA = TT < 2 ? 0 : TT == 2 ? 2 : TT < 5 ? 1 : 0, TB = TT == 0 ? 0 : TT == 1 ? 1 : TT == 2 ? 0 : TT == 3 ? 0 : TT == 4 ? 1 : 2;
            acc[I][J] = __builtin_amdgcn_mfma_f32_32x32x16_bf16(bf(av[I][TA]), bf(fb[J][TB]), acc[I][J], 0, 0, 0);
        };
        if constexpr (NCB == 2) {
        PD_SB
        mm(PD_I(0), PD_I(0)); x3::sp_h<0, true>(ws, tw); PD_SB
        mm(PD_I(0), PD_I(1)); x3::sp_h<1, true>(ws, tw); PD_SB
        mm(PD_I(1), PD_I(0)); x3::sp_m<0, true>(ws, tw); PD_SB
        mm(PD_I(1), PD_I(1)); PD_SB
        mm(PD_I(0), PD_I(2)); x3::sp_m<1, true>(ws, tw); PD_SB
        mm(PD_I(0), PD_I(3)); PD_SB
        mm(PD_I(1), PD_I(2)); x3::sp_l<0, true>(tw); PD_SB
        mm(PD_I(1), PD_I(3)); x3::sp_l<1, true>(tw); PD_SB
        load_b(std::integral_constant<int, 0>{});
        mm(PD_I(0), PD_I(4)); PD_SB
        mm(PD_I(0), PD_I(5));
        *reinterpret_cast<uint2*>(lds_c + sp_off + (NXT * 3 + 0) * BP_BYTES) = uint2{tw.h[0] ^ wsign, tw.h[1] ^ wsign};
        *reinterpret_cast<uint2*>(lds_c + sp_off + (NXT * 3 + 1) * BP_BYTES) = uint2{tw.m[0] ^ wsign, tw.m[1] ^ wsign};
        *reinterpret_cast<uint2*>(lds_c + sp_off + (NXT * 3 + 2) * BP_BYTES) = uint2{tw.l[0] ^ wsign, tw.l[1] ^ wsign};
        PD_SB
        mm(PD_I(1), PD_I(4)); mm(PD_I(1), PD_I(5)); load_fb(0, 2); load_fb(1, 2); if (LAST) halo_item(PD_I(0)); PD_SB
        mm(PD_I(0), PD_I(6)); mm(PD_I(0), PD_I(7)); if (LAST) halo_item(PD_I(1)); PD_SB
        mm(PD_I(1), PD_I(6)); mm(PD_I(1), PD_I(7)); if (LAST) halo_item(PD_I(2)); PD_SB
        mm(PD_I(0), PD_I(8)); mm(PD_I(0), PD_I(9)); if (LAST) halo_item(PD_I(3)); PD_SB
        mm(PD_I(1), PD_I(8)); mm(PD_I(1), PD_I(9)); if (LAST) halo_item(PD_I(4)); PD_SB
        mm(PD_I(0), PD_I(10)); mm(PD_I(0), PD_I(11)); if (LAST) halo_item(PD_I(5)); PD_SB
        mm(PD_I(1), PD_I(10)); mm(PD_I(1), PD_I(11)); if (LAST) halo_item(PD_I(6));
        } else {
        PD_SB
        mm(PD_I(0), PD_I(0)); x3::sp_h<0, true>(ws, tw); PD_SB
        mm(PD_I(1), PD_I(0)); PD_SB
        mm(PD_I(0), PD_I(1)); x3::sp_m<0, true>(ws, tw); PD_SB
        mm(PD_I(1), PD_I(1)); PD_SB
        mm(PD_I(0), PD_I(2)); x3::sp_l<0, true>(tw); PD_SB
        mm(PD_I(1), PD_I(2)); PD_SB
        load_b(std::integral_constant<int, (int)NXT>{});
        mm(PD_I(0), PD_I(3));
        *reinterpret_cast<unsigned*>(lds_c + sp_off + (NXT * 3 + 0) * BP_BYTES) = tw.h[0] ^ wsign;
        *reinterpret_cast<unsigned*>(lds_c + sp_off + (NXT * 3 + 1) * BP_BYTES) = tw.m[0] ^ wsign;
        *reinterpret_cast<unsigned*>(lds_c + sp_off + (NXT * 3 + 2) * BP_BYTES) = tw.l[0] ^ wsign;
        PD_SB
        mm(PD_I(1), PD_I(3)); load_fb(0, 2); if (LAST) halo_item(PD_I(0)); PD_SB
        mm(PD_I(0), PD_I(4)); if (LAST) { halo_item(PD_I(1)); halo_item(PD_I(2)); } PD_SB
        mm(PD_I(1), PD_I(4)); if (LAST) { halo_item(PD_I(3)); halo_item(PD_I(4)); } PD_SB
        mm(PD_I(0), PD_I(5)); if (LAST) halo_item(PD_I(5)); PD_SB
        mm(PD_I(1), PD_I(5)); if (LAST) halo_item(PD_I(6));
        }
        static_assert(NI <= 7, "halo items per thread");
        if (++s_kw == KW) { s_kw = 0; if (++s_kh == KH) { s_kh = 0; ++s_g; } }
        __syncthreads();
    };

    {
        halo_load(0);
        load_b(std::integral_constant<int, 0>{});
        halo_split();
        split_b0();
        load_b(std::integral_constant<int, 1>{});
        if constexpr (NCB == 1) load_b(std::integral_constant<int, 0>{});
        __syncthreads();
    }
    for (int q = 0; q < nchunks; q += 2) {
        chunk(std::integral_constant<unsigned, 0>{});
        if (q + 1 < nchunks) chunk(std::integral_constant<unsigned, 1>{});
    }
    __syncthreads();

    {
        float* Tt = smem_all + wave * (64 * 32);
        float (*red)[64][2] = reinterpret_cast<float (*)[64][2]>(smem_all + 4 * 64 * 32);
        const int col_l = lane & 31, rbase = 4 * (lane >> 5);
        const bool elu = a.act == ACT_ELU;
        const long img_m = (long)img * a.Ho * a.Wo;
        const __amdgpu_buffer_rsrc_t ry = make_rsrc(a.y + img_m * a.ldy, (unsigned)((long)a.Ho * a.Wo * a.ldy * 4));
        const __amdgpu_buffer_rsrc_t ra = make_rsrc(a.add ? a.add + img_m * a.ld_add : a.y, a.add ? (unsigned)((long)a.Ho * a.Wo * a.ld_add * 4) : 0u);
        auto pix_of = [&](int t) {
            const int r = (t & 3) * 8 + (lane >> 3);
            return (oy0 + (2 * wave + (t >> 2)) * BR + r / TW) * a.Wo + ox0 + r % TW;
        };
#pragma unroll
        for (int j = 0; j < NCB; ++j) {
            float4 addv[8];
            if (a.add) {
#pragma unroll
                for (int t = 0; t < 8; ++t) {
                    const int pix = pix_of(t);
                    addv[t] = buf_ld4(ra, (unsigned)(pix * (int)a.ld_add + n0 + 32 * j + 4 * (lane & 7)) * 4u);
                }
            }
            float s1 = 0.f, s2 = 0.f;
            const float bv = a.bias ? a.bias[n0 + 32 * j + col_l] : 0.f;
#pragma unroll
            for (int i = 0; i < 2; ++i)
#pragma unroll
                for (int r = 0; r < 16; ++r) {
                    const float v = (wsign ? -acc[i][j][r] : acc[i][j][r]) + bv;
                    Tt[(32 * i + (r & 3) + 8 * (r >> 2) + rbase) * 32 + col_l] =
                        elu ? (v > 0.f ? v : __builtin_amdgcn_exp2f(v * 1.44269504088896341f) - 1.f) : v;
                    s1 += v;
                    s2 = __builtin_fmaf(v, v, s2);
                }
            const float4* Tq = reinterpret_cast<const float4*>(Tt) + lane;
            float4 v[8];
#pragma unroll
            for (int t = 0; t < 8; ++t) {
                v[t] = Tq[t * 64];
                if (a.add) { v[t].x += addv[t].x; v[t].y += addv[t].y; v[t].z += addv[t].z; v[t].w += addv[t].w; }
            }
            __builtin_amdgcn_sched_barrier(0);
#pragma unroll
            for (int t = 0; t < 8; ++t) {
                const int pix = pix_of(t);
                __builtin_amdgcn_raw_buffer_store_b128(__builtin_bit_cast(u32x4, v[t]), ry,
                                                      (unsigned)(pix * (int)a.ldy + n0 + 32 * j + 4 * (lane & 7)) * 4u, 0, 0);
            }
            asm volatile("s_nop 1");
            __builtin_amdgcn_sched_barrier(0);
            if (a.stats) {
                s1 += __shfl_xor(s1, 32); s2 += __shfl_xor(s2, 32);
                if (lane < 32) { red[wave][32 * j + col_l][0] = s1; red[wave][32 * j + col_l][1] = s2; }
            }
        }
        if (a.stats) {
            __syncthreads();
            if (a.stats_rows == 128) {
                if (tid < 2 * 64 && (tid & 63) < BNW) {
                    const int row_l = tid >> 6, cl = tid & 63;
                    const float t1 = red[2 * row_l][cl][0] + red[2 * row_l + 1][cl][0];
                    const float t2 = red[2 * row_l][cl][1] + red[2 * row_l + 1][cl][1];
                    float* o = a.stats + ((long)(mt * 2 + row_l) * a.Co + n0 + cl) * 2;
                    o[0] = t1; o[1] = t2;
                }
            } else {
                const int row_l = tid >> 6, cl = tid & 63;
                if (cl < BNW) {
                    float* o = a.stats + ((long)(mt * 4 + row_l) * a.Co + n0 + cl) * 2;
                    o[0] = red[row_l][cl][0]; o[1] = red[row_l][cl][1];
                }
            }
        }
    }
}

static int x3_halo_tw(int Ho, int Wo) {
    return (Wo % 32 == 0 && Ho % 8 == 0) ? 32 : (Wo % 16 == 0 && Ho % 16 == 0) ? 16 : (Wo % 8 == 0 && Ho % 32 == 0) ? 8 : 0;
}
struct HaloPlan { int tw, ncb; bool rowwin; };
static bool x3_halo_plan(const ConvArgs& a, HaloPlan& p) {
    p.tw = x3_halo_tw(a.Ho, a.Wo);
    p.rowwin = a.KH == 4 && a.KW == 4;
    p.ncb = (a.Co % 64 == 0 && (a.M / 256) * (a.Co / 64) >= 512) ? 2 : 1;
    if (p.tw == 0 || a.stride != 1 || a.sC != 1 || !(a.stats_rows == 128 || a.stats_rows == 64) || a.Co % 32 != 0) return false;
    if (!((long)a.sN * 4 < 0x7fffffffL && (long)a.Ho * a.Wo * a.ldy * 4 < 0x7fffffffL && (!a.add || (long)a.Ho * a.Wo * a.ld_add * 4 < 0x7fffffffL)))
        return false;
    if ((a.M / 256) * (a.Co / (32 * p.ncb)) < 512) return false;
    const long unit = p.rowwin ? 4 : 16;
    const long hh = 256 / p.tw + a.KH - 1, hw = p.tw + a.KW - 1;
    if (a.sH % unit != 0 || a.sW % unit != 0 || (hh + 1) * (a.sH / unit) + (hw + 1) * (a.sW / unit) >= 0xffffL) return false;
    if (p.rowwin)
        return a.mode == MODE_ZERO && a.sW == a.C && (a.KW * a.C) % x3h::CK == 0 && p.ncb == 2 && p.tw == 32 && a.pad < a.KH && a.pad_w < a.KW;
    if (!((a.KH == 3 || a.KH == 5) && a.KW == a.KH && a.C % x3h::CK == 0)) return false;
    if (!(a.mode == MODE_ZERO || (a.mode == MODE_TRANSPOSED && a.sshift == 0) || (a.mode == MODE_REFLECT && a.pad < a.H && a.pad_w < a.W))) return false;
    return p.ncb == 2 || (a.KH == 3 && p.tw != 8) || (a.KH == 5 && p.tw == 8);
}

template <int TERMS>
static void launch_conv_x3_halo(const ConvArgs& a, const HaloPlan& p, dim3 grid, hipStream_t st) {
    const int tw = p.tw;
    const dim3 block(NT);
#define PD_HALO(KHV, KWV, TWV, NCBV, RW) do { \
        if (a.mode == MODE_ZERO) hipLaunchKernelGGL((conv_halo_x3_kernel<MODE_ZERO, KHV, KWV, TWV, NCBV, RW, TERMS>), grid, block, 0, st, a); \
        else if constexpr (!RW) { \
            if (a.mode == MODE_REFLECT) hipLaunchKernelGGL((conv_halo_x3_kernel<MODE_REFLECT, KHV, KWV, TWV, NCBV, false, TERMS>), grid, block, 0, st, a); \
            else hipLaunchKernelGGL((conv_halo_x3_kernel<MODE_TRANSPOSED, KHV, KWV, TWV, NCBV, false, TERMS>), grid, block, 0, st, a); } } while (0)
    if (p.rowwin) PD_HALO(4, 1, 32, 2, true);
    else if (p.ncb == 1 && a.KH == 3) { if (tw == 32) PD_HALO(3, 3, 32, 1, false); else PD_HALO(3, 3, 16, 1, false); }
    else if (p.ncb == 1) PD_HALO(5, 5, 8, 1, false);
    else if (a.KH == 3) { if (tw == 32) PD_HALO(3, 3, 32, 2, false); else if (tw == 16) PD_HALO(3, 3, 16, 2, false); else PD_HALO(3, 3, 8, 2, false); }
    else { if (tw == 32) PD_HALO(5, 5, 32, 2, false); else if (tw == 16) PD_HALO(5, 5, 16, 2, false); else PD_HALO(5, 5, 8, 2, false); }
#undef PD_HALO
}
```

supervised-depth-estimation-from-polarized-images_amd/polardepth/_lib.py:

```python
import ctypes
import os

_HERE = os.path.dirname(os.path.abspath(__file__))
_SO = os.environ.get("PD_LIB") or os.path.join(_HERE, "libpolardepth.so")


class LibraryMissing(RuntimeError):
    pass


class PolarDepthError(RuntimeError):
    pass


_c = ctypes
_vp, _i, _sz, _dbl = _c.c_void_p, _c.c_int, _c.c_size_t, _c.c_double
_dp = _c.POINTER(_c.c_double)
_l, _f = _c.c_long, _c.c_float
_u64 = _c.c_uint64
_ip = _c.POINTER(_c.c_int)
_u = _c.c_uint
_vpp = _c.POINTER(_c.c_void_p)

SIGNATURES = {
    "pd_last_error": (_c.c_char_p, []),
    "pd_version": (_i, []),
    "pd_polar_tables_bytes": (_sz, [_i, _i, _i]),
    "pd_polar_tables_pack": (_i, [_dp, _dp, _i, _dp, _dp, _i, _dp, _dp, _i, _vp, _sz]),
    "pd_polar_tables_build": (_i, [_dbl, _vp, _sz, _c.POINTER(_sz)]),
    "pd_polar_fwd": (_i, [_vp, _vp, _vp, _vp, _vp, _vp, _vp, _sz, _i, _i, _i, _i, _i, _i, _vp]),
    "pd_polar_normals_from_xolp": (_i, [_vp, _vp, _vp, _sz, _i, _i, _i, _i, _vp]),
    "pd_polar_theta": (_i, [_vp, _vp, _vp, _vp, _vp, _vp, _sz, _l, _vp]),
    "pd_polar_calc_normals": (_i, [_vp, _vp, _vp, _i, _l, _i, _i, _vp]),
    "pd_polar_fit_matrix": (_i, [_dp, _dp]),
    "pd_polar_general_fwd": (_i, [_vp, _i, _dp, _vp, _vp, _vp, _vp, _vp, _sz, _i, _i, _i, _i, _i, _vp]),
    "pd_xolp_stats_workspace": (_sz, [_i, _i, _i]),
    "pd_xolp_stats": (_i, [_vp, _vp, _vp, _vp, _sz, _i, _i, _i, _i, _c.POINTER(_f), _i, _vp]),
    "pd_conv2d_tile_m": (_i, [_l, _i]),
    "pd_conv2d_stats_rows": (_l, [_l, _i]),
    "pd_conv2d_uses_x3": (_i, [_l, _i, _i, _i, _i, _i, _i, _i, _i, _i, _i, _i, _u]),
    "pd_conv2d_wgrad_uses_x3": (_i, [_l, _i, _i, _i, _i, _i, _i, _i, _i, _i, _i, _i, _u]),
    "pd_conv2d_uses_bf16": (_i, [_l, _i, _i, _i, _i, _i, _i, _i, _i, _i, _i, _i, _u]),
    "pd_conv2d_route": (_i, [_l, _i, _i, _i, _i, _i, _i, _i, _i, _i, _i, _i, _u]),
    "pd_conv2d_wgrad_uses_bf16": (_i, [_l, _i, _i, _i, _i, _i, _i, _i, _i, _i, _i, _i, _u]),
    "pd_conv2d_wgrad_route": (_i, [_l, _i, _i, _i, _i, _i, _i, _i, _i, _i, _i, _i, _u]),
    "pd_conv2d": (_i, [_vp, _vp, _vp, _vp, _vp, _vp, _i, _i, _i, _i, _l, _l, _l, _l, _i, _i, _i, _i, _i, _i, _i, _i, _i,
                       _i, _f, _f, _l, _u, _vp]),
    "pd_conv16": (_i, [_vp, _vp, _vp, _vp, _i, _i, _i, _i, _l, _l, _l, _i, _i, _i, _l, _i, _i, _vp]),
    "pd_conv16_wgrad_workspace": (_sz, [_i]),
    "pd_conv16_wgrad": (_i, [_vp, _vp, _vp, _vp, _vp, _sz, _i, _i, _i, _i, _l, _l, _l, _l, _i, _vp]),
    "pd_dgrad_s2_filters": (_i, [_vp, _vp, _i, _i, _vp]),
    "pd_conv2d_rect": (_i, [_vp, _vp, _vp, _i, _i, _i, _i, _l, _l, _l, _l, _i, _i, _i, _i, _i, _i, _i, _i, _l, _u, _vp]),
    "pd_interleave4": (_i, [_vp, _vp, _i, _i, _i, _i, _vp]),
    "pd_conv2d_add": (_i, [_vp, _vp, _vp, _l, _vp, _i, _i, _i, _i, _l, _l, _l, _l, _i, _i, _i, _i, _i, _i, _i, _i, _l, _u, _vp]),
    "pd_conv2d_wgrad_workspace": (_sz, [_l, _i, _i, _u]),
    "pd_conv2d_wgrad": (_i, [_vp, _vp, _vp, _vp, _vp, _sz, _i, _i, _i, _i, _l, _l, _l, _l, _i, _i, _i, _i, _i, _i, _i,
                             _i, _i, _f, _f, _l, _i, _u, _vp]),
    "pd_weight_transpose": (_i, [_vp, _vp, _i, _i, _i, _vp]),
    "pd_weight_transpose_batched": (_i, [_vp, _vp, _vp, _vp, _i, _i, _vp]),
    "pd_stem_s2d_input": (_i, [_vp, _vp, _i, _i, _i, _i, _l, _l, _l, _l, _i, _f, _f, _vp]),
    "pd_stem_s2d_weight": (_i, [_vp, _vp, _i, _i, _vp]),
    "pd_stem_s2d_weight_grad": (_i, [_vp, _vp, _i, _i, _i, _vp]),
    "pd_bn_fwd_finalize": (_i, [_vp, _l, _i, _dbl, _vp, _vp, _vp, _vp, _f, _f, _vp, _l, _vp, _vp, _vp, _vp, _i, _vp]),
    "pd_bn_bwd_finalize": (_i, [_vp, _l, _i, _dbl, _vp, _l, _vp, _vp, _vp, _i, _vp]),
    "pd_chain_bwd_rows": (_l, [_i, _i, _i, _i]),
    "pd_chain_fwd": (_i, [_vp, _vp, _vp, _vp, _vp, _i, _i, _i, _i, _l, _l, _i, _i, _f, _u64, _u64, _vp, _i, _vp]),
    "pd_chain_bwd_reduce": (_i, [_vp, _l, _vp, _vp, _l, _vp, _vp, _vp, _vp, _vp, _i, _i, _i, _i, _i, _i, _f, _u64,
                                 _u64, _vp, _i, _vp]),
    "pd_chain_bwd_apply": (_i, [_vp, _l, _vp, _vp, _l, _vp, _vp, _vp, _vp, _vp, _vp, _vp, _i, _i, _i, _i, _i, _i, _f,
                                _u64, _u64, _vp, _i, _vp]),
    "pd_maxpool3s2_fwd": (_i, [_vp, _vp, _vp, _i, _i, _i, _i, _vp]),
    "pd_maxpool3s2_bwd": (_i, [_vp, _vp, _vp, _i, _i, _i, _i, _vp]),
    "pd_maxpool3s2_bwd_add": (_i, [_vp, _vp, _vp, _l, _vp, _i, _i, _i, _i, _vp]),
    "pd_upcat_fwd": (_i, [_vp, _vp, _l, _vp, _i, _i, _i, _i, _i, _vp]),
    "pd_up_bwd": (_i, [_vp, _l, _vp, _i, _i, _i, _i, _vp]),
    "pd_up_bwd_elu": (_i, [_vp, _l, _vp, _vp, _i, _i, _i, _i, _vp]),
    "pd_act_bwd": (_i, [_vp, _vp, _vp, _l, _i, _vp]),
    "pd_up2x_ac_fwd": (_i, [_vp, _vp, _i, _i, _i, _i, _vp]),
    "pd_up2x_ac_bwd": (_i, [_vp, _vp, _i, _i, _i, _i, _vp]),
    "pd_relu_add": (_i, [_vp, _vp, _vp, _l, _i, _vp]),
    "pd_reflect_fold": (_i, [_vp, _vp, _i, _i, _i, _i, _vp]),
    "pd_reflect_fold_pad": (_i, [_vp, _vp, _i, _i, _i, _i, _i, _vp]),
    "pd_reflect_dgrad_border": (_i, [_vp, _l, _vp, _vp, _i, _i, _i, _i, _i, _vp]),
    "pd_adam_step": (_i, [_vp, _vp, _vp, _vp, _l, _f, _f, _f, _f, _f, _l, _vp, _f, _i, _vp]),
    "pd_step_tick": (_i, [_vp, _i, _i, _vp]),
    "pd_step_set_hyper": (_i, [_vp, _f, _f, _vp]),
    "pd_loss_rows": (_i, [_l]),
    "pd_disp_to_depth": (_i, [_vp, _vp, _vp, _i, _i, _i, _i, _i, _f, _f, _vp]),
    "pd_up_gather_bwd": (_i, [_vp, _vp, _i, _i, _i, _i, _i, _i, _i, _vp]),
    "pd_gt_normals": (_i, [_vp, _vp, _vp, _i, _i, _i, _f, _f, _vp]),
    "pd_sup_loss_fwd": (_i, [_vp, _vp, _vp, _vp, _vp, _i, _i, _i, _f, _f, _i, _vp]),
    "pd_normals_loss_masked": (_i, [_vp, _vp, _vp, _vp, _vp, _vp, _i, _i, _i, _vp]),
    "pd_normals_pred_loss_fwd": (_i, [_vp, _l, _vp, _vp, _vp, _vp, _i, _i, _i, _f, _f, _vp]),
    "pd_normals_pred_loss_bwd": (_i, [_vp, _l, _vp, _vp, _vp, _vp, _vp, _l, _i, _i, _i, _f, _f, _vp]),
    "pd_multiscale_loss_fwd": (_i, [_vpp, _vpp, _ip, _ip, _i, _vp, _vp, _vp, _vpp, _vpp, _vpp, _vp, _vp, _i, _i, _i, _i, _f, _f,
                                    _i, _vp]),
    "pd_multiscale_loss_bwd": (_i, [_vpp, _vpp, _vpp, _vpp, _vpp, _ip, _ip, _i, _vp, _vp, _vp, _vp, _vp, _vp, _vp, _vp, _vpp,
                                    _i, _i, _i, _f, _f, _vp]),
    "pd_sup_loss_bwd": (_i, [_vp, _vp, _vp, _vp, _vp, _vp, _vp, _vp, _i, _i, _i, _f, _f, _i, _i, _i, _vp]),
    "pd_smooth_fwd": (_i, [_vp, _vp, _vp, _vp, _vp, _i, _i, _i, _vp]),
    "pd_smooth_bwd": (_i, [_vp, _vp, _vp, _vp, _vp, _vp, _vp, _vp, _i, _i, _i, _i, _vp]),
    "pd_loss_finalize": (_i, [_vp, _ip, _vp, _ip, _ip, _ip, _i, _i, _f, _f, _vp, _vp, _vp]),
    "pd_loss_from_sums": (_i, [_vp, _ip, _ip, _i, _f, _f, _vp, _vp]),
    "pd_loss_weights": (_i, [_vp, _ip, _i, _f, _f, _vp, _vp]),
    "pd_softmax_rows_fwd": (_i, [_vp, _l, _l, _f, _vp]),
    "pd_softmax_rows_bwd": (_i, [_vp, _vp, _l, _l, _f, _vp]),
    "pd_resize_u8_pass": (_i, [_vp, _vp, _vp, _vp, _i, _i, _i, _i, _i, _i, _vp]),
    "pd_resize_wide_pass": (_i, [_vp, _vp, _i, _vp, _vp, _i, _i, _i, _i, _i, _i, _vp]),
    "pd_dofp_demosaic": (_i, [_vp, _i, _vp, _i, _ip, _i, _i, _i, _vp]),
    "pd_cdofp_demosaic": (_i, [_vp, _i, _ip, _ip, _dp, _dbl, _vp, _vp, _vp, _i, _i, _i, _vp]),
    "pd_frame_moments": (_i, [_vp, _i, _vp, _vp, _vp, _i, _i, _i, _i, _i, _vp]),
    "pd_dofp_cal_solve": (_i, [_vp, _dp, _dp, _dbl, _vp, _vp, _i, _i, _vp]),
    "pd_dofp_calibrate": (_i, [_vp, _i, _vp, _vp, _i, _vp, _i, _i, _i, _vp]),
    "pd_color_jitter_u8": (_i, [_vp, _vp, _vp, _vp, _vp, _i, _i, _i, _vp]),
    "pd_attn_fwd": (_i, [_vp, _vp, _vp, _vp, _vp, _i, _i, _i, _f, _vp]),
    "pd_attn_bwd": (_i, [_vp, _vp, _vp, _vp, _vp, _vp, _vp, _vp, _vp, _vp, _i, _i, _i, _f, _vp]),
    "pd_attn_bf16_workspace": (_sz, [_i, _i, _i, _i]),
    "pd_attn_bf16_fwd": (_i, [_vp, _vp, _vp, _vp, _vp, _vp, _sz, _i, _i, _i, _f, _vp]),
    "pd_attn_bf16_bwd": (_i, [_vp, _vp, _vp, _vp, _vp, _vp, _vp, _vp, _vp, _vp, _vp, _sz, _i, _i, _i, _f, _vp]),
    "pd_attn_bf16_bwd_parts": (_i, [_vp, _vp, _vp, _vp, _vp, _vp, _vp, _vp, _vp, _vp, _vp, _sz, _i, _i, _i, _f, _i, _vp]),
    "pd_disphead_fwd": (_i, [_vp, _vp, _vp, _vp, _i, _i, _i, _i, _vp]),
    "pd_disphead_bwd_data": (_i, [_vp, _vp, _vp, _vp, _i, _i, _i, _i, _vp]),
    "pd_disphead_workspace": (_sz, [_i]),
    "pd_disphead_bwd_weight": (_i, [_vp, _vp, _vp, _vp, _vp, _vp, _sz, _i, _i, _i, _i, _i, _vp]),
    "pd_disphead_bwd": (_i, [_vp, _vp, _vp, _vp, _vp, _i, _vp, _vp, _vp, _vp, _sz, _i, _i, _i, _i, _i, _vp]),
    "pd_ssim_bwd": (_i, [_vp, _vp, _vp, _vp, _vp, _vp, _i, _i, _i, _i, _i, _i, _vp]),
    "pd_ssim_fwd": (_i, [_vp, _vp, _vp, _i, _i, _i, _i, _i, _i, _vp]),
    "pd_depth_metrics": (_i, [_vp, _vp, _vp, _i, _vp, _vp, _i, _l, _f, _f, _vp]),
    "pd_view_synth_fwd": (_i, [_vp, _vp, _vp, _vp, _vp, _vp, _vp, _i, _i, _i, _i, _vp]),
    "pd_view_synth_bwd": (_i, [_vp, _vp, _vp, _vp, _vp, _vp, _vp, _vp, _i, _i, _i, _i, _i, _vp]),
    "pd_view_synth_pose_rows": (_i, [_i, _i]),
    "pd_view_synth_bwd_pose": (_i, [_vp, _vp, _vp, _vp, _vp, _vp, _vp, _vp, _vp, _vp, _vp, _i, _i, _i, _i, _i, _vp]),
    "pd_pose_matrix_fwd": (_i, [_vp, _vp, _vp, _i, _i, _vp]),
    "pd_pose_matrix_bwd": (_i, [_vp, _vp, _vp, _vp, _vp, _i, _i, _vp]),
    "pd_pose_head_fwd": (_i, [_vp, _vp, _vp, _vp, _vp, _vp, _vp, _vp, _i, _i, _i, _i, _i, _i, _vp]),
    "pd_pose_head_bwd": (_i, [_vp, _vp, _vp, _vp, _vp, _vp, _vp, _vp, _vp, _vp, _vp, _vp, _i, _i, _i, _i, _i, _i, _i, _vp]),
    "pd_depth_to_updisp_bwd": (_i, [_vp, _vp, _vp, _l, _f, _f, _vp]),
    "pd_reproj_combine_rows": (_i, [_i, _i, _i]),
    "pd_reproj_combine_fwd": (_i, [_vpp, _vpp, _i, _vp, _vp, _vp, _vp, _vp, _vp, _i, _i, _i, _i, _vp]),
    "pd_reproj_combine_bwd": (_i, [_vp, _vp, _vp, _vp, _vpp, _i, _i, _i, _i, _i, _vp]),
    "pd_cost_volume": (_i, [_vp, _vp, _vp, _vp, _vp, _vp, _vp, _vp, _l, _vp, _vp, _vp, _vp, _i, _i, _i, _i, _i, _i, _i, _vp]),
    "pd_student_masks_rows": (_i, [_i, _i, _i]),
    "pd_student_masks": (_i, [_vp, _vp, _vp, _vp, _i, _vp, _vp, _vp, _vp, _vp, _i, _i, _i, _i, _i, _vp]),
    "pd_depth_bins_update": (_i, [_vp, _i, _vp, _dbl, _i, _i, _vp, _vp]),
    "pd_student_combine_rows": (_i, [_i, _i, _i]),
    "pd_student_combine_fwd": (_i, [_vpp, _i, _vp, _vp, _vp, _vp, _vp, _vp, _vp, _vp, _i, _i, _i, _i, _vp]),
    "pd_student_combine_bwd": (_i, [_vp, _vp, _vp, _vp, _vp, _vp, _vpp, _vp, _i, _i, _i, _i, _i, _vp]),
    "pd_normals_stats_workspace": (_sz, [_i, _i, _i, _i]),
    "pd_normals_stats": (_i, [_vp, _l, _vp, _vp, _vp, _ip, _i, _vp, _i, _vp, _vp, _vp, _sz, _i, _i, _i, _f, _f, _vp]),
    "pd_backproject": (_i, [_vp, _vp, _vp, _vp, _vp, _i, _i, _i, _f, _f, _vp]),
    "pd_cloud_nn": (_i, [_vp, _vp, _i, _vp, _vp, _i, _vp, _vp, _u, _i, _vp]),
    "pd_cloud_stats_workspace": (_sz, [_i, _i, _i, _i]),
    "pd_cloud_stats": (_i, [_vp, _vp, _vp, _ip, _i, _vp, _vp, _vp, _vp, _sz, _i, _i, _i, _vp]),
    "pd_depth_medians_workspace": (_sz, [_i, _i]),
    "pd_depth_medians": (_i, [_vp, _vp, _vp, _ip, _i, _vp, _vp, _vp, _sz, _i, _i, _i, _f, _f, _vp]),
    "pd_depth_stats_workspace": (_sz, [_i, _i, _i, _i]),
    "pd_depth_stats": (_i, [_vp, _vp, _vp, _ip, _i, _vp, _vp, _vp, _vp, _vp, _sz, _i, _i, _i, _f, _f, _vp]),
}


class _Lib:

    def __init__(self):
        self._h = None

    def _load(self):
        if self._h is None:
            if not os.path.exists(_SO):
                raise LibraryMissing(
                    f"{_SO} not found: build it with `make -C {os.path.join(os.path.dirname(_HERE), 'csrc')}` "
                    "(or python -c 'import __graft_entry__ as g; g.build()'). There is no CPU fallback.")
            import torch
            h = ctypes.CDLL(_SO)
            for name, (res, args) in SIGNATURES.items():
                fn = getattr(h, name)
                fn.restype = res
                fn.argtypes = args
            self._h = h
        return self._h

    def __getattr__(self, name):
        return getattr(self._load(), name)

    @property
    def path(self):
        return _SO


lib = _Lib()


def check(rc, what=""):
    if rc != 0:
        msg = lib.pd_last_error()
        raise PolarDepthError(f"{what} failed ({rc}): {msg.decode() if msg else ''}")


def ptr(t):
    return None if t is None else ctypes.c_void_p(t.data_ptr())


def stream_ptr():
    import torch
    return ctypes.c_void_p(torch.cuda.current_stream().cuda_stream)
```

supervised-depth-estimation-from-polarized-images_amd/polardepth/engine.py:

```python
import os

import torch
import torch.distributed as dist

from ._lib import lib, check, ptr, stream_ptr


class ParamStore:
    def __init__(self, models, order=None, unused=lambda model_name, param_name: False, device=None):
        names = list(order) if order is not None else list(models.keys())
        fwd, tail = [], []
        for mn in names:
            for pn, p in models[mn].named_parameters():
                (tail if unused(mn, pn) else fwd).append((f"{mn}.{pn}", p))
        used = list(reversed(fwd))
        self.entries = used + tail
        self.n_used_params = len(used)
        device = device or self.entries[0][1].device
        align = 4
        offs, total = [], 0
        for _, p in self.entries:
            offs.append(total)
            total += (p.numel() + align - 1) // align * align
        self.models = models
        self.numel = total
        self.n_used = offs[self.n_used_params] if self.n_used_params < len(offs) else total
        self.flat = torch.zeros(total, dtype=torch.float32, device=device)
        self.grad = torch.zeros(total, dtype=torch.float32, device=device)
        self.grad_is_zero = True
        self._zero_version = self.grad._version
        self.offsets = {}
        for (name, p), off in zip(self.entries, offs):
            self.offsets[name] = (off, p.numel())
            self._adopt(p, off)
        self.flat_t = None
        self._wt_epoch = -1
        self._wt_index, rows, blk = {}, [], [0]
        for (name, p), off in zip(self.entries, offs):
            if p.dim() == 4 and p.numel() < 2 ** 31:
                co, ci, kh, kw = p.shape
                self._wt_index[self.flat.data_ptr() + 4 * off] = (off, co, ci, kh, kw)
                rows.append([off, co, kh * kw, ci])
                blk.append(blk[-1] + kh * kw * ((co + 31) // 32) * ((ci + 31) // 32))
        if rows:
            self._wt_table = torch.tensor(rows, dtype=torch.int32, device=device)
            self._wt_blk = torch.tensor(blk, dtype=torch.int32, device=device)
            self._wt_n, self._wt_blocks = len(rows), blk[-1]
            from . import ops as _ops
            _ops.WT_PROVIDERS[:] = [pr for pr in _ops.WT_PROVIDERS if pr.flat.data_ptr() != self.flat.data_ptr()]
            _ops.WT_PROVIDERS.append(self)

    def weights_changed(self):
        self._wt_epoch = -1

    def transposed(self, w):
        e = self._wt_index.get(w.data_ptr())
        if e is None or tuple(w.shape) != (e[1], e[2], e[3], e[4]) or not w.is_cuda:
            return None
        off, co, ci, kh, kw = e
        from . import ops as _ops
        if self._wt_epoch != _ops.FWD_EPOCH:
            if self.flat_t is None:
                self.flat_t = torch.empty_like(self.flat)
            from ._lib import lib, check, ptr, stream_ptr
            check(lib.pd_weight_transpose_batched(ptr(self.flat), ptr(self.flat_t), ptr(self._wt_table), ptr(self._wt_blk),
                                                  self._wt_n, self._wt_blocks, stream_ptr()), "pd_weight_transpose_batched")
            self._wt_epoch = _ops.FWD_EPOCH
            self._wt_event = torch.cuda.Event()
            self._wt_event.record()
        else:
            torch.cuda.current_stream().wait_event(self._wt_event)
        return self.flat_t[off:off + co * ci * kh * kw].view(ci, kh, kw, co).permute(0, 3, 1, 2)

    def _view(self, buf, p, off):
        flat = buf[off:off + p.numel()]
        if p.dim() == 4 and p.data.is_contiguous(memory_format=torch.channels_last) and not p.data.is_contiguous():
            co, ci, kh, kw = p.shape
            return flat.view(co, kh, kw, ci).permute(0, 3, 1, 2)
        return flat.view(p.shape)

    def _adopt(self, p, off):
        src = p.data
        if p.dim() == 4:
            src = src.contiguous(memory_format=torch.channels_last)
            pv = self.flat[off:off + p.numel()].view(p.shape[0], p.shape[2], p.shape[3], p.shape[1]).permute(0, 3, 1, 2)
            gv = self.grad[off:off + p.numel()].view(p.shape[0], p.shape[2], p.shape[3], p.shape[1]).permute(0, 3, 1, 2)
        else:
            pv = self.flat[off:off + p.numel()].view(p.shape)
            gv = self.grad[off:off + p.numel()].view(p.shape)
        pv.copy_(src.to(self.flat.device))
        p.data = pv
        p.grad = gv
        p._pd_store = self

    def zero_grad(self):
        if not (self.grad_is_zero and self.grad._version == self._zero_version):
            self.grad.zero_()
        self.mark_zeroed()

    def mark_zeroed(self):
        self.grad_is_zero = True
        self._zero_version = self.grad._version

    def used_params(self):
        return [p for _, p in self.entries[:self.n_used_params]]


class FusedAdam(torch.optim.Optimizer):

    def __init__(self, store, lr=1e-3, betas=(0.9, 0.999), eps=1e-8, weight_decay=0.0, reducer=None,
                 zero_grad_in_step=True):
        self.store = store
        self.reducer = reducer
        self.zero_grad_in_step = zero_grad_in_step and os.environ.get("PD_ADAM_KEEP_GRAD") != "1"
        params = [p for _, p in store.entries]
        super().__init__(params, dict(lr=lr, betas=betas, eps=eps, weight_decay=weight_decay))
        self.exp_avg = torch.zeros_like(store.flat)
        self.exp_avg_sq = torch.zeros_like(store.flat)
        self.step_count = 0
        self.grad_scale = 1.0
        self.device_step = False
        self.dev_state = None
        self._dev_hyper = None

    def use_device_step(self, on=True):
        self.device_step = bool(on)
        if on:
            if self.dev_state is None:
                self.dev_state = torch.zeros(4, dtype=torch.int64, device=self.store.flat.device)
            self.dev_state[1] = self.step_count
            self._dev_hyper = None
            self.sync_hyper()

    def sync_hyper(self):
        if not self.device_step:
            return
        cur = (float(self.param_groups[0]["lr"]), float(self.grad_scale))
        if cur != self._dev_hyper:
            check(lib.pd_step_set_hyper(ptr(self.dev_state), cur[0], cur[1], stream_ptr()), "pd_step_set_hyper")
            self._dev_hyper = cur

    def zero_grad(self, set_to_none=False):
        from . import functional as PF
        PF.sync_wgrad_stream()
        PF.reset_backward_state()
        self.store.zero_grad()
        if self.store.flat.is_cuda:
            PF.DropoutState.begin_step(self.store.flat.device)
        if self.reducer is not None:
            self.reducer.reset()

    @torch.no_grad()
    def step(self, closure=None):
        from . import functional as PF
        PF.sync_wgrad_stream()
        if self.reducer is not None:
            self.reducer.finish()
        g = self.param_groups[0]
        self.step_count += 1
        n = self.store.n_used
        b1, b2 = g["betas"]
        state = None
        if self.device_step:
            state = self.dev_state
            if not torch.cuda.is_current_stream_capturing():
                self.sync_hyper()
            check(lib.pd_step_tick(ptr(state), 0, 1, stream_ptr()), "pd_step_tick")
        check(lib.pd_adam_step(ptr(self.store.flat), ptr(self.store.grad), ptr(self.exp_avg), ptr(self.exp_avg_sq), n,
                               float(g["lr"]), float(b1), float(b2), float(g["eps"]), float(g["weight_decay"]),
                               self.step_count, ptr(state), float(self.grad_scale), int(self.zero_grad_in_step), stream_ptr()),
              "pd_adam_step")
        self.store.weights_changed()
        if self.zero_grad_in_step:
            self.store.mark_zeroed()

    REFERENCE_MODEL_ORDER = ("normals_encoder", "xolp_encoder", "joint_encoder", "rgb_encoder", "mono_depth")

    def reference_order(self):
        by_model = {}
        for name, _ in self.store.entries:
            by_model.setdefault(name.split(".", 1)[0], []).append(name)
        names = []
        for m in list(self.REFERENCE_MODEL_ORDER) + [k for k in by_model if k not in self.REFERENCE_MODEL_ORDER]:
            if m in by_model:
                if m in getattr(self.store, "models", {}):
                    names += [f"{m}.{pn}" for pn, _ in self.store.models[m].named_parameters()]
                else:
                    names += by_model[m]
        return names

    def state_dict(self):
        names = self.reference_order()
        entries = dict(self.store.entries)
        used = {n for n, _ in self.store.entries[:self.store.n_used_params]}
        state = {}
        for i, name in enumerate(names):
            if name in used and self.step_count > 0:
                off, n = self.store.offsets[name]
                p = entries[name]
                state[i] = {"step": torch.tensor(float(self.step_count)),
                            "exp_avg": self.store._view(self.exp_avg, p, off).clone(),
                            "exp_avg_sq": self.store._view(self.exp_avg_sq, p, off).clone()}
        g = {k: v for k, v in self.param_groups[0].items() if k != "params"}
        g["params"] = list(range(len(names)))
        return {"state": state, "param_groups": [g], "pd_order": names}

    def load_state_dict(self, sd):
        g = sd["param_groups"][0]
        names = sd.get("pd_order") or self.reference_order()
        if len(g.get("params", names)) != len(names):
            raise ValueError(f"adam.pth holds {len(g['params'])} parameters, this model has {len(names)}")
        entries = dict(self.store.entries)
        todo, steps = [], []
        for i, st in sd["state"].items():
            name = names[int(i)]
            if name not in self.store.offsets:
                raise ValueError(f"adam.pth: unknown parameter {name!r}")
            p = entries[name]
            for k in ("exp_avg", "exp_avg_sq"):
                if tuple(st[k].shape) != tuple(p.shape):
                    raise ValueError(f"adam.pth: {k} of parameter {int(i)} has shape {tuple(st[k].shape)}, "
                                     f"{name} needs {tuple(p.shape)} (parameter order mismatch?)")
            todo.append((name, p, st))
            steps.append(int(float(st["step"])))
        for k in ("lr", "betas", "eps", "weight_decay"):
            if k in g:
                self.param_groups[0][k] = g[k]
        self.exp_avg.zero_(); self.exp_avg_sq.zero_()
        for name, p, st in todo:
            off, n = self.store.offsets[name]
            self.store._view(self.exp_avg, p, off).copy_(st["exp_avg"])
            self.store._view(self.exp_avg_sq, p, off).copy_(st["exp_avg_sq"])
        self.step_count = max(steps) if steps else 0


class GradReducer:

    def __init__(self, store, bucket_bytes=16 << 20, process_group=None):
        self.store = store
        self.group = process_group
        self.world = dist.get_world_size(process_group) if dist.is_initialized() else 1
        self.active = self.world > 1 or (dist.is_initialized() and os.environ.get("PD_DIST_TEST") == "1")
        self.buckets = []
        self.bucket_of = {}
        cap = max(bucket_bytes // 4, 1)
        start, cur = 0, 0
# ... 105 lines not shown
```

supervised-depth-estimation-from-polarized-images_amd/polardepth/ops.py:

```python
import os

import torch

from ._lib import lib, check, ptr, stream_ptr

MODE_ZERO, MODE_REFLECT, MODE_TRANSPOSED = 0, 1, 2
ACT_NONE, ACT_RELU, ACT_ELU, ACT_SIGMOID = 0, 1, 2, 3
CL = torch.channels_last
PROFILE = None

CONV_AUTO, CONV_FP32_MFMA, CONV_BF16X3, CONV_WGRAD_SPLIT_IN_REGS, CONV_GENERAL_KERNELS, CONV_X3_IM2COL = 0, 1, 2, 4, 8, 16
CONV_WGRAD_ROW_WORKGROUPS = 32
CONV_BF16 = 128
CONV_FLAGS = (CONV_FP32_MFMA if os.environ.get("PD_CONV_X3", "1") == "0" else
              CONV_X3_IM2COL if os.environ.get("PD_CONV_HALO", "1") == "0" else CONV_AUTO)
WGRAD_FLAGS = (CONV_FP32_MFMA if os.environ.get("PD_WGRAD_X3C", "1") == "0" else
               CONV_X3_IM2COL if os.environ.get("PD_CONV_HALO", "1") == "0" else
               CONV_WGRAD_ROW_WORKGROUPS if os.environ.get("PD_WGRAD_ROLL", "1") == "0" else CONV_AUTO)


class conv_flags:

    def __init__(self, conv=None, wgrad=None):
        self.new = (conv, wgrad)

    def __enter__(self):
        global CONV_FLAGS, WGRAD_FLAGS
        self.old = (CONV_FLAGS, WGRAD_FLAGS)
        if self.new[0] is not None:
            CONV_FLAGS = int(self.new[0])
        if self.new[1] is not None:
            WGRAD_FLAGS = int(self.new[1])
        return self

    def __exit__(self, *exc):
        global CONV_FLAGS, WGRAD_FLAGS
        CONV_FLAGS, WGRAD_FLAGS = self.old
        return False


def conv_bf16_mode():
    return (bool(CONV_FLAGS & CONV_BF16), bool(WGRAD_FLAGS & CONV_BF16))


def _with_bf16(word, bf16):
    if bf16 is None:
        return word
    if bf16 and not (word & (CONV_FP32_MFMA | CONV_BF16X3)):
        return word | CONV_BF16
    return word & ~CONV_BF16


def _profiled(label, flops, fn, shape=None):
    if PROFILE is None:
        return fn()
    e0, e1 = torch.cuda.Event(enable_timing=True), torch.cuda.Event(enable_timing=True)
    e0.record()
    r = fn()
    e1.record()
    PROFILE.append((label, flops, e0, e1, shape))
    return r


_IGEMM_LABELS = ("conv_igemm_kernel<{bm},{bn},{gather}>", "conv_igemm_uni_kernel<{bm},{bn}>", "conv_igemm_x3_kernel<{bm},{bn}>",
                 "conv_halo_x3_kernel<8x32,64>", "conv_halo_bf16_kernel<8x32,64>")


def _igemm_label(M, Co, vec, kind, C=0, KH=1, KW=1, stride=1, pad=0, mode=0, act=ACT_NONE, out_scale=False, out_hw=(0, 0),
                 flags=None):
    flags = CONV_FLAGS if flags is None else flags
    if not vec:
        flags = CONV_FP32_MFMA | CONV_GENERAL_KERNELS
    r = lib.pd_conv2d_route(M, Co, C, KH, KW, stride, pad, mode, act, int(out_scale), out_hw[0], out_hw[1], flags)
    return _IGEMM_LABELS[r & 15].format(bm=r >> 12, bn=(r >> 4) & 255, gather="vec" if vec else "scalar")


def _require_cuda(*ts):
    for t in ts:
        if t is not None and not t.is_cuda:
            raise RuntimeError("polardepth ops need CUDA(HIP) tensors; there is no CPU fallback")


def empty_nhwc(n, c, h, w, device):
    return torch.empty((n, c, h, w), dtype=torch.float32, device=device, memory_format=CL)


def is_nhwc(t):
    n, c, h, w = t.shape
    return t.stride() == (h * w * c, 1, w * c, c) or t.is_contiguous(memory_format=CL)


def as_nhwc(t):
    return t if is_nhwc(t) else t.contiguous(memory_format=CL)


def weight_cl(w):
    return w if w.is_contiguous(memory_format=CL) else w.contiguous(memory_format=CL)


def conv_out_size(h, k, s, p):
    return (h + 2 * p - k) // s + 1


def conv2d_fwd(x, w, bias=None, stride=1, pad=0, mode=MODE_ZERO, act=ACT_NONE, want_stats=False,
               affine=None, out=None, out_hw=None, out_scale=None, alg_k=None):
    _require_cuda(x, w, bias, out_scale)
    global FWD_EPOCH
    FWD_EPOCH += 1
    N, C, H, W = x.shape
    Co, Ci, KH, KW = w.shape
    assert Ci == C, f"channel mismatch {Ci} vs {C}"
    w = weight_cl(w)
    Ho, Wo = conv_out_size(H, KH, stride, pad), conv_out_size(W, KW, stride, pad)
    if out_hw is not None:
        assert out_hw[0] <= Ho and out_hw[1] <= Wo
        Ho, Wo = out_hw
    if out is None:
        out = empty_nhwc(N, Co, Ho, Wo, x.device)
    assert out.shape == (N, Co, Ho, Wo) and out.stride(1) == 1
    ldy = out.stride(3)
    assert out.stride(2) == Wo * ldy and out.stride(0) == Ho * Wo * ldy
    stats = None
    if want_stats:
        rows = lib.pd_conv2d_stats_rows(N * Ho * Wo, Co)
        stats = torch.empty((rows, Co, 2), dtype=torch.float32, device=x.device)
    sub, div = (affine if affine is not None else (0.0, 1.0))
    sN, sC, sH, sW = x.stride()
    vec = C % 4 == 0 and sC == 1 and affine is None
    if (USE_CONV16 and mode == MODE_REFLECT and Co == 16 and C in (16, 32) and KH == 3 and KW == 3 and stride == 1 and pad == 1
            and vec and not want_stats and out_scale is None and act in (ACT_NONE, ACT_ELU) and out_hw is None
            and H >= 2 and W >= 2 and sN % 4 == 0 and sH % 4 == 0 and sW % 4 == 0):
        _profiled("conv16_halo_kernel", 2.0 * N * Ho * Wo * Co * C * 9,
                  lambda: check(lib.pd_conv16(ptr(x), ptr(w), ptr(bias), ptr(out), N, H, W, C, sN, sH, sW, Ho, Wo, Co, ldy,
                                              0, act, stream_ptr()), "pd_conv16"),
                  shape=("fwd", N, C, H, W, Co, KH, stride, mode))
        return out
    _profiled(_igemm_label(N * Ho * Wo, Co, vec, "fwd", C, KH, KW, stride, pad, mode, act, out_scale is not None, (Ho, Wo)), 2.0 * N * Ho * Wo * Co * (alg_k if alg_k is not None else C * KH * KW),
              lambda: check(lib.pd_conv2d(ptr(x), ptr(w), ptr(bias), ptr(out_scale), ptr(out), ptr(stats), N, H, W, C, sN, sH, sW, sC,
                                          Ho, Wo, Co, KH, KW, stride, pad, mode, act, int(affine is not None), sub,
                                          div, ldy, CONV_FLAGS, stream_ptr()), "pd_conv2d"),
              shape=("fwd", N, C, H, W, Co, KH, stride, mode))
    return (out, stats) if want_stats else out


USE_S2_PHASES = os.environ.get("PD_S2_PHASES", "1") != "0"
USE_CONV16 = os.environ.get("PD_CONV16", "1") != "0"
WT_PROVIDERS = []
FWD_EPOCH = 0


def weight_transposed(w):
    Co, Ci, KH, KW = w.shape
    w = weight_cl(w)
    for prov in WT_PROVIDERS:
        wt = prov.transposed(w)
        if wt is not None:
            return wt
    wt = torch.empty((Ci, Co, KH, KW), dtype=torch.float32, device=w.device, memory_format=CL)
    check(lib.pd_weight_transpose(ptr(w), ptr(wt), Co, KH * KW, Ci, stream_ptr()), "pd_weight_transpose")
    return wt


def conv2d_dgrad(dy, w, in_hw, stride=1, pad=0, wt=None, addend=None, bf16=None):
    _require_cuda(dy, w)
    flags = _with_bf16(CONV_FLAGS, bf16)
    dy = as_nhwc(dy)
    N, Co, Hy, Wy = dy.shape
    _, Ci, KH, KW = w.shape
    H, W = in_hw
    if wt is None:
        wt = weight_transposed(w)
    dx = empty_nhwc(N, Ci, H, W, dy.device)
    sN, sC, sH, sW = dy.stride()
    if (USE_S2_PHASES and not (flags & CONV_GENERAL_KERNELS) and addend is None and stride == 2 and KH == 3 and KW == 3 and pad == 1 and H == 2 * Hy and W == 2 * Wy
            and Co % 32 == 0 and Ci % 4 == 0 and Ci > 16 and sC == 1 and sN % 4 == 0 and sH % 4 == 0 and sW % 4 == 0):
        def _phases():
            wsub = torch.empty(9 * Ci * Co, dtype=torch.float32, device=dy.device)
            check(lib.pd_dgrad_s2_filters(ptr(wt), ptr(wsub), Ci, Co, stream_ptr()), "pd_dgrad_s2_filters")
            sub = torch.empty((4, N, Hy, Wy, Ci), dtype=torch.float32, device=dy.device)
            for c, off in enumerate((0, 1, 3, 5)):
                ph, pw = c >> 1, c & 1
                check(lib.pd_conv2d_rect(ptr(dy), wsub.data_ptr() + 4 * off * Ci * Co, ptr(sub[c]), N, Hy, Wy, Co, sN, sH, sW,
                                         sC, Hy, Wy, Ci, 1 + ph, 1 + pw, ph, pw, MODE_TRANSPOSED, Ci, flags, stream_ptr()),
                      "pd_conv2d_rect(dgrad s2 phase)")
            check(lib.pd_interleave4(ptr(sub), ptr(dx), N, Hy, Wy, Ci, stream_ptr()), "pd_interleave4")
        _profiled("conv_dgrad_s2_phases", 2.0 * N * Hy * Wy * Co * Ci * KH * KW, _phases,
                  shape=("dgrad", N, Ci, H, W, Co, KH, stride, MODE_TRANSPOSED))
        return dx
    c16_mode = 1 if (pad == 0 and H == Hy + 2 and W == Wy + 2) else (2 if (pad == 1 and H == Hy and W == Wy) else 0)
    if (USE_CONV16 and addend is None and Co == 16 and Ci in (16, 32) and KH == 3 and KW == 3 and stride == 1 and c16_mode
            and sC == 1 and sN % 4 == 0 and sH % 4 == 0 and sW % 4 == 0 and Hy >= 2 and Wy >= 2):
        _profiled("conv16_halo_kernel", 2.0 * N * Hy * Wy * Co * Ci * 9,
                  lambda: check(lib.pd_conv16(ptr(dy), ptr(wt), None, ptr(dx), N, Hy, Wy, Co, sN, sH, sW, H, W, Ci, Ci, c16_mode,
                                              0, stream_ptr()), "pd_conv16(dgrad)"),
                  shape=("dgrad", N, Ci, H, W, Co, KH, stride, MODE_TRANSPOSED))
        return dx
    if addend is not None:
        assert addend.shape == dx.shape and addend.stride(1) == 1 and addend.is_cuda
        ld_add = addend.stride(3)
        assert addend.stride(2) == W * ld_add and addend.stride(0) == H * W * ld_add
        _profiled(_igemm_label(N * H * W, Ci, True, "dgrad", Co, KH, KW, stride, pad, MODE_TRANSPOSED, out_hw=(H, W), flags=flags),
                  2.0 * N * Hy * Wy * Co * Ci * KH * KW,
                  lambda: check(lib.pd_conv2d_add(ptr(dy), ptr(wt), ptr(addend), ld_add, ptr(dx), N, Hy, Wy, Co, sN, sH, sW,
                                                  sC, H, W, Ci, KH, KW, stride, pad, MODE_TRANSPOSED, Ci, flags, stream_ptr()),
                                "pd_conv2d_add(dgrad)"),
                  shape=("dgrad", N, Ci, H, W, Co, KH, stride, MODE_TRANSPOSED))
        return dx
    _profiled(_igemm_label(N * H * W, Ci, True, "dgrad", Co, KH, KW, stride, pad, MODE_TRANSPOSED, out_hw=(H, W), flags=flags), 2.0 * N * Hy * Wy * Co * Ci * KH * KW,
              lambda: check(lib.pd_conv2d(ptr(dy), ptr(wt), None, None, ptr(dx), None, N, Hy, Wy, Co, sN, sH, sW, sC,
                                          H, W, Ci, KH, KW, stride, pad, MODE_TRANSPOSED, ACT_NONE, 0, 0.0, 1.0, Ci,
                                          flags, stream_ptr()), "pd_conv2d(dgrad)"),
              shape=("dgrad", N, Ci, H, W, Co, KH, stride, MODE_TRANSPOSED))
    return dx


_ws_cache = {}


def _workspace(nbytes, device):
    key = (device.index, torch.cuda.current_stream(device).cuda_stream)
    buf = _ws_cache.get(key)
    if buf is None or buf.numel() < nbytes:
        buf = torch.empty(max(nbytes, 1 << 20), dtype=torch.uint8, device=device)
        _ws_cache[key] = buf
    return buf


_WGRAD_LABELS = ("conv_wgrad_kernel", "conv_wgrad_x3c_kernel", "conv_wgrad_halo_x3_kernel", "conv_wgrad_roll_x3_kernel",
                 None, None, "conv_wgrad_halo_bf16_kernel", "conv_wgrad_roll_bf16_kernel")


def conv2d_wgrad(x, dy, w_shape, stride=1, pad=0, mode=MODE_ZERO, affine=None, dw=None, dbias=None,
                 want_bias=False, accumulate=False, alg_k=None, bf16=None):
    _require_cuda(x, dy)
    flags = _with_bf16(WGRAD_FLAGS, bf16)
    dy = as_nhwc(dy)
    N, C, H, W = x.shape
    Co, Ci, KH, KW = w_shape
    assert Ci == C
    Ho, Wo = dy.shape[2], dy.shape[3]
    if dw is None:
        dw = torch.empty(tuple(w_shape), dtype=torch.float32, device=x.device, memory_format=CL)
        accumulate = False
    assert dw.is_contiguous(memory_format=CL) or dw.numel() == dw.shape[0] * dw.shape[1]
    if want_bias and dbias is None:
        dbias = torch.empty(Co, dtype=torch.float32, device=x.device)
    M, K = N * Ho * Wo, KH * KW * C
    sN, sC, sH, sW = x.stride()
    if (USE_CONV16 and mode == MODE_REFLECT and Co == 16 and C in (16, 32) and KH == 3 and KW == 3 and stride == 1 and pad == 1
            and affine is None and sC == 1 and sN % 4 == 0 and sH % 4 == 0 and sW % 4 == 0 and H >= 2 and W >= 2
            and dy.stride(3) % 4 == 0):
        ws = _workspace(lib.pd_conv16_wgrad_workspace(C), x.device)
        _profiled("conv16_wgrad_kernel", 2.0 * M * Co * K,
                  lambda: check(lib.pd_conv16_wgrad(ptr(x), ptr(dy), ptr(dw), ptr(dbias), ptr(ws), ws.numel(), N, H, W, C,
                                                    sN, sH, sW, dy.stride(3), int(accumulate), stream_ptr()),
                                "pd_conv16_wgrad"),
                  shape=("wgrad", N, C, H, W, Co, KH, stride, mode))
        return (dw, dbias) if (want_bias or dbias is not None) else dw
    nbytes = lib.pd_conv2d_wgrad_workspace(M, Co, K, flags)
    ws = _workspace(nbytes, x.device)
    sub, div = (affine if affine is not None else (0.0, 1.0))
    sN, sC, sH, sW = x.stride()
    fits = affine is None and sC == 1 and sN % 4 == 0 and sH % 4 == 0 and sW % 4 == 0 and dy.stride(3) % 4 == 0
    route = lib.pd_conv2d_wgrad_route(M, Co, C, KH, KW, stride, pad, mode, H, W, Ho, Wo, flags) if fits else 0
    _profiled(_WGRAD_LABELS[route & 7],
              2.0 * M * Co * (alg_k if alg_k is not None else K),
              lambda: check(lib.pd_conv2d_wgrad(ptr(x), ptr(dy), ptr(dw), ptr(dbias), ptr(ws), ws.numel(), N, H, W, C,
                                                sN, sH, sW, sC, Ho, Wo, Co, KH, KW, stride, pad, mode,
                                                int(affine is not None), sub, div, dy.stride(3), int(accumulate),
                                                flags, stream_ptr()), "pd_conv2d_wgrad"),
              shape=("wgrad", N, C, H, W, Co, KH, stride, mode))
    return (dw, dbias) if (want_bias or dbias is not None) else dw


class _SSIMFn(torch.autograd.Function):

    @staticmethod
    def forward(ctx, x, y, mode, no_ssim):
        x, y = x.float().contiguous(), y.float().contiguous()
        N, C, H, W = x.shape
        out = torch.empty((N, C if mode == 0 else 1, H, W), dtype=torch.float32, device=x.device)
        check(lib.pd_ssim_fwd(ptr(x), ptr(y), ptr(out), N, C, H, W, mode, int(no_ssim), stream_ptr()), "pd_ssim_fwd")
        ctx.args = (mode, int(no_ssim))
        ctx.save_for_backward(x, y)
        return out

    @staticmethod
    def backward(ctx, gout):
        x, y = ctx.saved_tensors
        mode, no_ssim = ctx.args
        N, C, H, W = x.shape
        gout = gout.float().contiguous()
        ws = torch.empty(5 * x.numel(), dtype=torch.float32, device=x.device)
        gx = torch.empty_like(x)
        gy = torch.empty_like(y) if ctx.needs_input_grad[1] else None
        check(lib.pd_ssim_bwd(ptr(x), ptr(y), ptr(gout), ptr(ws), ptr(gx), ptr(gy), N, C, H, W, mode, no_ssim, stream_ptr()),
              "pd_ssim_bwd")
        return gx, gy, None, None


def ssim(x, y):
    _require_cuda(x, y)
    return _SSIMFn.apply(x, y, 0, False)


def reprojection_loss(pred, target, no_ssim=False):
    _require_cuda(pred, target)
    return _SSIMFn.apply(pred, target, 1, bool(no_ssim))


REPROJ_MAX_FRAMES = 8


def _dev_ptrs(tensors):
    import ctypes
    return (ctypes.c_void_p * len(tensors))(*[t.data_ptr() for t in tensors])


class _ViewSynthFn(torch.autograd.Function):

    @staticmethod
    def forward(ctx, depth, src, K, inv_K, T):
        N, C, H, W = src.shape
        warped = torch.empty_like(src)
        coords = torch.empty((N, H, W, 2), dtype=torch.float32, device=src.device)
        check(lib.pd_view_synth_fwd(ptr(depth), ptr(src), ptr(K), ptr(inv_K), ptr(T), ptr(warped), ptr(coords), N, C, H, W,
                                    stream_ptr()), "pd_view_synth_fwd")
        ctx.save_for_backward(depth, src, K, inv_K, T, coords)
        ctx.mark_non_differentiable(coords)
        return warped, coords

    @staticmethod
    def backward(ctx, gwarped, _gcoords):
        depth, src, K, inv_K, T, coords = ctx.saved_tensors
        N, C, H, W = src.shape
        if ctx.needs_input_grad[4]:
            gdepth = torch.empty_like(depth) if ctx.needs_input_grad[0] else None
            part = torch.empty((N, lib.pd_view_synth_pose_rows(H, W), 12), dtype=torch.float64, device=src.device)
            gT = torch.empty((N, 4, 4), dtype=torch.float32, device=src.device)
            check(lib.pd_view_synth_bwd_pose(ptr(gwarped.float().contiguous()), ptr(src), ptr(coords), ptr(depth), ptr(K),
                                             ptr(inv_K), ptr(T), ptr(gdepth), ptr(part), None, ptr(gT), N, C, H, W, 0,
                                             stream_ptr()), "pd_view_synth_bwd_pose")
            return gdepth, None, None, None, gT
        gdepth = torch.empty_like(depth)
        check(lib.pd_view_synth_bwd(ptr(gwarped.float().contiguous()), ptr(src), ptr(coords), ptr(depth), ptr(K), ptr(inv_K),
                                    ptr(T), ptr(gdepth), N, C, H, W, 0, stream_ptr()), "pd_view_synth_bwd")
        return gdepth, None, None, None, None


def view_synthesis(depth, src, K, inv_K, T):
    _require_cuda(depth, src, K, inv_K, T)
    if src.dim() != 4 or depth.dim() != 4 or depth.shape[1] != 1 or depth.shape[0] != src.shape[0] or \
            depth.shape[2:] != src.shape[2:]:
# ... 397 lines not shown
```

Baseline: 353.3 images/s.

## Pre-split conv weights into bf16x3 planes once per optimizer step

Adds a batched kernel that splits fp32 conv weights into three bf16 planes (high, mid, low) in the LDS-ready swizzled layout, cached per weight version in the parameter store. The halo 3-term conv kernel gets a WP variant that loads these pre-split planes with buffer loads instead of splitting the weights in registers on every tile, for both forward and dgrad. This removes redundant per-workgroup split ALU work from the MFMA loop. In exchange it adds extra weight memory traffic (1.5x the fp32 bytes), a plane-production kernel after each weight update, and version, event and graph-capture bookkeeping on the Python side.

Measured after the change: 355.3 images/s (median of 6 runs). No clear change (+0.6%).

```diff
diff --git a/include/polardepth.h b/include/polardepth.h
--- a/include/polardepth.h
+++ b/include/polardepth.h
@@ -64,7 +64,8 @@
 #define PD_CONV_X3_IM2COL 16u
 #define PD_CONV_WGRAD_ROW_WORKGROUPS 32u
 #define PD_CONV_BF16 128u
-#define PD_CONV_FLAGS_ALL 191u
+#define PD_CONV_NO_WEIGHT_PLANES 256u
+#define PD_CONV_FLAGS_ALL 447u
 int pd_conv2d_tile_m(long M, int Cout);
 long pd_conv2d_stats_rows(long M, int Cout);
 int pd_conv2d_uses_x3(long M, int Cout, int C, int KH, int KW, int stride, int pad, int mode, int act, int has_out_scale,
@@ -116,6 +117,14 @@
 int pd_weight_transpose(const void* w, void* wt, int Cout, int T, int Cin, void* stream);
 int pd_weight_transpose_batched(const void* src, void* dst, const void* table, const void* blk, int n, int nblocks,
                                 void* stream);
+
+int pd_weight_planes_batched(const void* src, void* dst, const void* table, const void* blk, int n, int nblocks,
+                             void* stream);
+int pd_conv2d_planes(const void* x, const void* w, const void* w_planes, const void* bias, const void* out_scale,
+                     void* y, void* stats, const void* addend, long ld_add,
+                     int N, int H, int W, int C, long sN, long sH, long sW, long sC,
+                     int Ho, int Wo, int Cout, int KH, int KW, int stride, int pad, int mode, int act,
+                     long ldy, unsigned flags, void* stream);
 
 int pd_bn_fwd_finalize(const void* partial, long R, int C, double count, const void* gamma, const void* beta,
                        void* running_mean, void* running_var, float momentum, float eps, void* acc_ws, long acc_len,
diff --git a/supervised-depth-estimation-from-polarized-images_amd/csrc/conv.hip b/supervised-depth-estimation-from-polarized-images_amd/csrc/conv.hip
--- a/supervised-depth-estimation-from-polarized-images_amd/csrc/conv.hip
+++ b/supervised-depth-estimation-from-polarized-images_amd/csrc/conv.hip
@@ -54,6 +54,8 @@
     unsigned flags;
     int stats_rows;
     int nmajor;
+    const void* wp;
+    unsigned wp_bytes;
 };
 
 __device__ __forceinline__ float4 ldg4(const float* p) { return *reinterpret_cast<const float4*>(p); }
@@ -1121,8 +1123,15 @@
 static int launch_conv(ConvArgs& a, const ConvRoute& r, hipStream_t st) {
     a.mtiles = r.mtiles; a.ntiles = r.ntiles; a.nmajor = r.nmajor;
     const dim3 grid((unsigned)(((long)r.mtiles * r.ntiles + 7) / 8 * 8)), block(NT);
+    const long wp_bytes = (long)((a.Co + 63) / 64) * 64 * a.K * 6;
+    const bool planes = a.wp && !(a.flags & PD_CONV_NO_WEIGHT_PLANES) && r.family == CONV_HALO && r.terms == 3 && !r.halo.rowwin &&
+                        wp_bytes < 0x7fffffffL && ((size_t)a.wp & 15) == 0;
+    if (!planes) a.wp = nullptr;
+    a.wp_bytes = planes ? (unsigned)wp_bytes : 0u;
     if (r.family == CONV_HALO) {
-        if (r.terms == 1) launch_conv_x3_halo<1>(a, r.halo, grid, st); else launch_conv_x3_halo<3>(a, r.halo, grid, st);
+        if (r.terms == 1) launch_conv_x3_halo<1>(a, r.halo, grid, st);
+        else if (planes) launch_conv_x3_halo<3, true>(a, r.halo, grid, st);
+        else launch_conv_x3_halo<3>(a, r.halo, grid, st);
     } else if (r.family == CONV_X3) {
         with_mode(a.mode, [&](auto md) {
             constexpr int MD = decltype(md)::value;
@@ -1199,7 +1208,8 @@
                        const void* addend, long ld_add,
                        int N, int H, int W, int C, long sN, long sH, long sW, long sC,
                        int Ho, int Wo, int Co, int KH, int KW, int stride, int pad, int mode, int act,
-                       int affine, float sub, float div, long ldy, unsigned flags, void* stream, int pad_w = -1) {
+                       int affine, float sub, float div, long ldy, unsigned flags, void* stream, int pad_w = -1,
+                       const void* w_planes = nullptr) {
     if (pad_w < 0) pad_w = pad;
     PD_REQUIRE(pd::conv_flags_ok(flags), "pd_conv2d: bad flags 0x%x", flags);
     PD_REQUIRE(x && w && y, "pd_conv2d: null tensor");
@@ -1220,6 +1230,7 @@
     ConvArgs a;
     a.x = (const float*)x; a.w = (const float*)w; a.bias = (const float*)bias; a.oscale = (const float*)out_scale; a.y = (float*)y; a.stats = (float*)stats;
     a.add = (const float*)addend; a.ld_add = ld_add;
+    a.wp = w_planes; a.wp_bytes = 0;
     fill_conv_args(a, N, H, W, C, sN, sH, sW, sC, Ho, Wo, Co, KH, KW, stride, pad, pad_w, mode, act, affine, sub, div, ldy, flags);
     PD_REQUIRE((long)Co * a.K * 4 < 0x7fffffffL, "pd_conv2d: weight tensor too large for 32-bit offsets");
     const long span = 256 / ((long)Ho * Wo) + 2;
@@ -1244,6 +1255,17 @@
     PD_REQUIRE(addend && ld_add >= Co, "pd_conv2d_add: bad addend");
     return conv2d_impl(x, w, nullptr, nullptr, y, nullptr, addend, ld_add, N, H, W, C, sN, sH, sW, sC, Ho, Wo, Co, KH, KW,
                        stride, pad, mode, ACT_NONE, 0, 0.f, 1.f, ldy, flags, stream);
+}
+
+extern "C" int pd_conv2d_planes(const void* x, const void* w, const void* w_planes, const void* bias, const void* out_scale,
+                                void* y, void* stats, const void* addend, long ld_add,
+                                int N, int H, int W, int C, long sN, long sH, long sW, long sC,
+                                int Ho, int Wo, int Co, int KH, int KW, int stride, int pad, int mode, int act,
+                                long ldy, unsigned flags, void* stream) {
+    PD_REQUIRE(!addend || ld_add >= Co, "pd_conv2d_planes: bad addend");
+    PD_REQUIRE(!addend || (!bias && !out_scale && !stats && act == ACT_NONE), "pd_conv2d_planes: an addend excludes bias, scale, statistics and activation");
+    return conv2d_impl(x, w, bias, out_scale, y, stats, addend, addend ? ld_add : 0, N, H, W, C, sN, sH, sW, sC, Ho, Wo, Co, KH, KW,
+                       stride, pad, mode, act, 0, 0.f, 1.f, ldy, flags, stream, -1, w_planes);
 }
 
 extern "C" int pd_conv2d_rect(const void* x, const void* w, void* y, int N, int H, int W, int C, long sN, long sH, long sW,
@@ -2150,6 +2172,32 @@
         if (ci0 + r < Ci && co0 + x < Co) wt[((long)(ci0 + r) * T + t) * Co + co0 + x] = tile[x][r];
 }
 
+__global__ __launch_bounds__(256) void weight_planes_batched_kernel(const float* __restrict__ src, char* __restrict__ dst,
+                                                                    const int* __restrict__ table,
+                                                                    const int* __restrict__ blk, int n) {
+    int lo = 0, hi = n;
+    while (hi - lo > 1) {
+        const int mid = (lo + hi) >> 1;
+        if (blk[mid] <= (int)blockIdx.x) lo = mid; else hi = mid;
+    }
+    const int off = table[5 * lo], Co = table[5 * lo + 1], T = table[5 * lo + 2], Ci = table[5 * lo + 3], c0 = table[5 * lo + 4];
+    const int lb = (int)blockIdx.x - blk[lo];
+    const int nch = (Ci / x3::CK) * T;
+    const int b = lb / nch, q = lb - b * nch;
+    const int g = q / T, tap = q - g * T;
+    const int row = threadIdx.x >> 2, sls = threadIdx.x & 3;
+    const int co = 64 * b + row;
+    float4 w4 = make_float4(0.f, 0.f, 0.f, 0.f);
+    if (co < Co) w4 = ldg4(src + off + ((long)co * T + tap) * Ci + x3::CK * g + 4 * sls);
+    uint2 h, m, l;
+    x3::split2(w4.x, w4.y, h.x, m.x, l.x);
+    x3::split2(w4.z, w4.w, h.y, m.y, l.y);
+    char* d = dst + ((long)c0 + lb) * (3 * x3::BP_BYTES) + row * (x3::CK * 2) + 16 * ((sls >> 1) ^ ((row >> 3) & 1)) + 8 * (sls & 1);
+    *reinterpret_cast<uint2*>(d + 0 * x3::BP_BYTES) = h;
+    *reinterpret_cast<uint2*>(d + 1 * x3::BP_BYTES) = m;
+    *reinterpret_cast<uint2*>(d + 2 * x3::BP_BYTES) = l;
+}
+
 inline int wgrad_tco(int Co) { return Co > 32 ? 64 : (Co > 16 ? 32 : 16); }
 
 inline bool wgrad_x3c_enabled(unsigned flags) { return !(flags & (PD_CONV_FP32_MFMA | PD_CONV_WGRAD_SPLIT_IN_REGS)); }
@@ -2355,6 +2403,15 @@
     return pd::check_launch("pd_weight_transpose_batched");
 }
 
+extern "C" int pd_weight_planes_batched(const void* src, void* dst, const void* table, const void* blk, int n, int nblocks,
+                                        void* stream) {
+    PD_REQUIRE(src && dst && table && blk && n > 0 && nblocks > 0, "pd_weight_planes_batched: bad arguments");
+    PD_REQUIRE(pd::aligned16(src) && pd::aligned16(dst), "pd_weight_planes_batched: src and dst must be 16-byte aligned");
+    hipLaunchKernelGGL(weight_planes_batched_kernel, dim3((unsigned)nblocks), dim3(256), 0, (hipStream_t)stream,
+                       (const float*)src, (char*)dst, (const int*)table, (const int*)blk, n);
+    return pd::check_launch("pd_weight_planes_batched");
+}
+
 namespace {
 __global__ __launch_bounds__(256) void dgrad_s2_filters_kernel(const float* __restrict__ wt, float* __restrict__ wsub,
                                                                int Ci, int Co) {
diff --git a/supervised-depth-estimation-from-polarized-images_amd/csrc/conv_x3_halo.hpp b/supervised-depth-estimation-from-polarized-images_amd/csrc/conv_x3_halo.hpp
--- a/supervised-depth-estimation-from-polarized-images_amd/csrc/conv_x3_halo.hpp
+++ b/supervised-depth-estimation-from-polarized-images_amd/csrc/conv_x3_halo.hpp
@@ -13,11 +13,12 @@
 };
 }
 
-template <int MODE, int KH, int KW, int TW, int NCB, bool ROWWIN, int TERMS = 3>
+template <int MODE, int KH, int KW, int TW, int NCB, bool ROWWIN, int TERMS = 3, bool WP = false>
 __global__ __launch_bounds__(NT, 3) void conv_halo_x3_kernel(const ConvArgs a) {
     using namespace x3h;
     using G = Geo<KH, KW, TW, NCB, TERMS>;
     static_assert(TERMS == 1 || TERMS == 3, "bf16 terms per operand");
+    static_assert(!WP || (TERMS == 3 && !ROWWIN), "pre-split weights: the three-term per-tap form only");
     constexpr int HW = G::HW, HP = G::HP, NI = G::NI, T = KH * KW, TR = G::TR, BR = G::BR, BNW = 32 * NCB;
     constexpr unsigned BP_BASE = G::BP_BASE, BP_BYTES = G::BP_BYTES;
     static_assert(!ROWWIN || (KW == 1 && MODE == MODE_ZERO), "row windows: zero padding, the filter row folded into the channels");
@@ -84,11 +85,32 @@
     const int ngroups = (ROWWIN ? a.KW * a.C : a.C) / CK;
     const unsigned tap_bytes = (unsigned)(ROWWIN ? a.KW * a.C : a.C) * 4u;
     const int nchunks = ngroups * T;
+    constexpr unsigned WP_CHUNK = 3 * 64 * CK * 2;
+    const __amdgpu_buffer_rsrc_t rp_ = make_rsrc(WP ? a.wp : a.w, WP ? a.wp_bytes : 0u);
+    const unsigned pblk = (unsigned)((NCB == 2 ? nt : nt >> 1) * nchunks) * WP_CHUNK;
+    const unsigned pv0 = NCB == 2 ? pblk + 16u * (unsigned)tid : pblk + 2048u * (unsigned)(tid >> 7) + 1024u * (unsigned)(nt & 1) + 8u * (unsigned)(tid & 127);
+    const unsigned pv1 = NCB == 2 ? pblk + 4096u + 8u * (unsigned)tid : pblk + 4096u + 1024u * (unsigned)(nt & 1) + 4u * (unsigned)tid;
+    const unsigned pd0 = BP_BASE + (NCB == 2 ? 16u : 8u) * (unsigned)tid, pd1 = BP_BASE + 2 * BP_BYTES + (NCB == 2 ? 8u : 4u) * (unsigned)tid;
+    unsigned pw[NCB == 2 ? 1 : 2][3 * NCB];
     int s_qb = 0, sb_tap = 0;
     unsigned s_boff = 0, sb_c4 = 0;
     float4 wq;
     float2 wq2[2];
     auto load_b = [&](auto set_tag) {
+        if constexpr (WP) {
+            const unsigned so = s_qb < nchunks ? (unsigned)s_qb * WP_CHUNK : 0u;
+            unsigned* d = pw[NCB == 2 ? 0 : decltype(set_tag)::value];
+            if constexpr (NCB == 2) {
+                const u32x4 v = __builtin_amdgcn_raw_buffer_load_b128(rp_, pv0, so, 0);
+                const uint2 l = __builtin_bit_cast(uint2, __builtin_amdgcn_raw_buffer_load_b64(rp_, pv1, so, 0));
+                d[0] = v.x; d[1] = v.y; d[2] = v.z; d[3] = v.w; d[4] = l.x; d[5] = l.y;
+            } else {
+                const uint2 v = __builtin_bit_cast(uint2, __builtin_amdgcn_raw_buffer_load_b64(rp_, pv0, so, 0));
+                d[0] = v.x; d[1] = v.y; d[2] = __builtin_amdgcn_raw_buffer_load_b32(rp_, pv1, so, 0);
+            }
+            ++s_qb;
+            return;
+        }
         if constexpr (NCB == 2) {
             wq = __builtin_bit_cast(float4, __builtin_amdgcn_raw_buffer_load_b128(rw_, vb, s_qb < nchunks ? s_boff : 0u, 0));
         } else {
@@ -138,7 +160,23 @@
                 rx, (((i & 1) ? hpk[i >> 1] >> 16 : hpk[i >> 1] & 0xffffu) << (ROWWIN ? 4 : 6)) + hq16, g * (CK * 4), 0));
     };
 
+    auto store_planes = [&](const unsigned* d, unsigned buf) {
+        if constexpr (NCB == 2) {
+            *reinterpret_cast<u32x4*>(lds_c + pd0 + buf * 3 * BP_BYTES) = u32x4{d[0], d[1], d[2], d[3]};
+            *reinterpret_cast<uint2*>(lds_c + pd1 + buf * 3 * BP_BYTES) = uint2{d[4], d[5]};
+        } else {
+            *reinterpret_cast<uint2*>(lds_c + pd0 + buf * 3 * BP_BYTES) = uint2{d[0], d[1]};
+            *reinterpret_cast<unsigned*>(lds_c + pd1 + buf * 3 * BP_BYTES) = d[2];
+        }
+    };
     auto split_b0 = [&]() {
+        if constexpr (WP) {
+            unsigned d[3 * NCB];
+#pragma unroll
+            for (int e = 0; e < 3 * NCB; ++e) d[e] = pw[0][e] ^ wsign;
+            store_planes(d, 0u);
+            return;
+        }
         const float4 w4 = NCB == 2 ? wq : make_float4(wq2[0].x, wq2[0].y, 0.f, 0.f);
         uint2 h, m, l;
         if constexpr (TERMS == 1) {
@@ -190,7 +228,14 @@
         const bool LAST = s_kh == KH - 1 && s_kw == KW - 1 && s_g + 1 < ngroups;
         const bool halo_issue = (s_kh | s_kw) == 0 && s_g + 1 < ngroups;
         float ws[4];
-        if constexpr (NCB == 2) {
+        unsigned px[3 * NCB];
+        if constexpr (WP) {
+            unsigned* d = pw[NCB == 2 ? 0 : NXT];
+            if constexpr (NCB == 2) asm volatile("" : "+v"(d[0]), "+v"(d[1]), "+v"(d[2]), "+v"(d[3]), "+v"(d[4]), "+v"(d[5]));
+            else asm volatile("" : "+v"(d[0]), "+v"(d[1]), "+v"(d[2]));
+#pragma unroll
+            for (int e = 0; e < 3 * NCB; ++e) px[e] = d[e];
+        } else if constexpr (NCB == 2) {
             asm volatile("" : "+v"(wq.x), "+v"(wq.y), "+v"(wq.z), "+v"(wq.w));
             ws[0] = wq.x; ws[1] = wq.y; ws[2] = wq.z; ws[3] = wq.w;
         } else {
@@ -246,22 +291,42 @@
             constexpr int TA = TT < 2 ? 0 : TT == 2 ? 2 : TT < 5 ? 1 : 0, TB = TT == 0 ? 0 : TT == 1 ? 1 : TT == 2 ? 0 : TT == 3 ? 0 : TT == 4 ? 1 : 2;
             acc[I][J] = __builtin_amdgcn_mfma_f32_32x32x16_bf16(bf(av[I][TA]), bf(fb[J][TB]), acc[I][J], 0, 0, 0);
         };
+        auto wstep = [&](auto s_tag) {
+            constexpr int S = decltype(s_tag)::value;
+            if constexpr (WP) { if constexpr (S < 3 * NCB) px[S] ^= wsign; }
+            else if constexpr (S == 0) x3::sp_h<0, true>(ws, tw);
+            else if constexpr (S == 1) x3::sp_h<1, true>(ws, tw);
+            else if constexpr (S == 2) x3::sp_m<0, true>(ws, tw);
+            else if constexpr (S == 3) x3::sp_m<1, true>(ws, tw);
+            else if constexpr (S == 4) x3::sp_l<0, true>(tw);
+            else x3::sp_l<1, true>(tw);
+        };
+        auto wstore = [&]() {
+            if constexpr (WP) { store_planes(px, NXT); return; }
+            if constexpr (NCB == 2) {
+                *reinterpret_cast<uint2*>(lds_c + sp_off + (NXT * 3 + 0) * BP_BYTES) = uint2{tw.h[0] ^ wsign, tw.h[1] ^ wsign};
+                *reinterpret_cast<uint2*>(lds_c + sp_off + (NXT * 3 + 1) * BP_BYTES) = uint2{tw.m[0] ^ wsign, tw.m[1] ^ wsign};
+                *reinterpret_cast<uint2*>(lds_c + sp_off + (NXT * 3 + 2) * BP_BYTES) = uint2{tw.l[0] ^ wsign, tw.l[1] ^ wsign};
+            } else {
+                *reinterpret_cast<unsigned*>(lds_c + sp_off + (NXT * 3 + 0) * BP_BYTES) = tw.h[0] ^ wsign;
+                *reinterpret_cast<unsigned*>(lds_c + sp_off + (NXT * 3 + 1) * BP_BYTES) = tw.m[0] ^ wsign;
+                *reinterpret_cast<unsigned*>(lds_c + sp_off + (NXT * 3 + 2) * BP_BYTES) = tw.l[0] ^ wsign;
+            }
+        };
         if constexpr (NCB == 2) {
         PD_SB
-        mm(PD_I(0), PD_I(0)); x3::sp_h<0, true>(ws, tw); PD_SB
-        mm(PD_I(0), PD_I(1)); x3::sp_h<1, true>(ws, tw); PD_SB
-        mm(PD_I(1), PD_I(0)); x3::sp_m<0, true>(ws, tw); PD_SB
+        mm(PD_I(0), PD_I(0)); wstep(PD_I(0)); PD_SB
+        mm(PD_I(0), PD_I(1)); wstep(PD_I(1)); PD_SB
+        mm(PD_I(1), PD_I(0)); wstep(PD_I(2)); PD_SB
         mm(PD_I(1), PD_I(1)); PD_SB
-        mm(PD_I(0), PD_I(2)); x3::sp_m<1, true>(ws, tw); PD_SB
+        mm(PD_I(0), PD_I(2)); wstep(PD_I(3)); PD_SB
         mm(PD_I(0), PD_I(3)); PD_SB
-        mm(PD_I(1), PD_I(2)); x3::sp_l<0, true>(tw); PD_SB
-        mm(PD_I(1), PD_I(3)); x3::sp_l<1, true>(tw); PD_SB
+        mm(PD_I(1), PD_I(2)); wstep(PD_I(4)); PD_SB
+        mm(PD_I(1), PD_I(3)); wstep(PD_I(5)); PD_SB
         load_b(std::integral_constant<int, 0>{});
         mm(PD_I(0), PD_I(4)); PD_SB
         mm(PD_I(0), PD_I(5));
-        *reinterpret_cast<uint2*>(lds_c + sp_off + (NXT * 3 + 0) * BP_BYTES) = uint2{tw.h[0] ^ wsign, tw.h[1] ^ wsign};
-        *reinterpret_cast<uint2*>(lds_c + sp_off + (NXT * 3 + 1) * BP_BYTES) = uint2{tw.m[0] ^ wsign, tw.m[1] ^ wsign};
-        *reinterpret_cast<uint2*>(lds_c + sp_off + (NXT * 3 + 2) * BP_BYTES) = uint2{tw.l[0] ^ wsign, tw.l[1] ^ wsign};
+        wstore();
         PD_SB
         mm(PD_I(1), PD_I(4)); mm(PD_I(1), PD_I(5)); load_fb(0, 2); load_fb(1, 2); if (LAST) halo_item(PD_I(0)); PD_SB
         mm(PD_I(0), PD_I(6)); mm(PD_I(0), PD_I(7)); if (LAST) halo_item(PD_I(1)); PD_SB
@@ -272,17 +337,15 @@
         mm(PD_I(1), PD_I(10)); mm(PD_I(1), PD_I(11)); if (LAST) halo_item(PD_I(6));
         } else {
         PD_SB
-        mm(PD_I(0), PD_I(0)); x3::sp_h<0, true>(ws, tw); PD_SB
+        mm(PD_I(0), PD_I(0)); wstep(PD_I(0)); if constexpr (WP) wstep(PD_I(1)); PD_SB
         mm(PD_I(1), PD_I(0)); PD_SB
-        mm(PD_I(0), PD_I(1)); x3::sp_m<0, true>(ws, tw); PD_SB
+        mm(PD_I(0), PD_I(1)); wstep(PD_I(2)); PD_SB
         mm(PD_I(1), PD_I(1)); PD_SB
-        mm(PD_I(0), PD_I(2)); x3::sp_l<0, true>(tw); PD_SB
+        mm(PD_I(0), PD_I(2)); if constexpr (!WP) wstep(PD_I(4)); PD_SB
         mm(PD_I(1), PD_I(2)); PD_SB
         load_b(std::integral_constant<int, (int)NXT>{});
         mm(PD_I(0), PD_I(3));
-        *reinterpret_cast<unsigned*>(lds_c + sp_off + (NXT * 3 + 0) * BP_BYTES) = tw.h[0] ^ wsign;
-        *reinterpret_cast<unsigned*>(lds_c + sp_off + (NXT * 3 + 1) * BP_BYTES) = tw.m[0] ^ wsign;
-        *reinterpret_cast<unsigned*>(lds_c + sp_off + (NXT * 3 + 2) * BP_BYTES) = tw.l[0] ^ wsign;
+        wstore();
         PD_SB
         mm(PD_I(1), PD_I(3)); load_fb(0, 2); if (LAST) halo_item(PD_I(0)); PD_SB
         mm(PD_I(0), PD_I(4)); if (LAST) { halo_item(PD_I(1)); halo_item(PD_I(2)); } PD_SB
@@ -408,15 +471,16 @@
     return p.ncb == 2 || (a.KH == 3 && p.tw != 8) || (a.KH == 5 && p.tw == 8);
 }
 
-template <int TERMS>
+template <int TERMS, bool WP = false>
 static void launch_conv_x3_halo(const ConvArgs& a, const HaloPlan& p, dim3 grid, hipStream_t st) {
     const int tw = p.tw;
     const dim3 block(NT);
 #define PD_HALO(KHV, KWV, TWV, NCBV, RW) do { \
-        if (a.mode == MODE_ZERO) hipLaunchKernelGGL((conv_halo_x3_kernel<MODE_ZERO, KHV, KWV, TWV, NCBV, RW, TERMS>), grid, block, 0, st, a); \
+        constexpr bool P = WP && !RW; \
+        if (a.mode == MODE_ZERO) hipLaunchKernelGGL((conv_halo_x3_kernel<MODE_ZERO, KHV, KWV, TWV, NCBV, RW, TERMS, P>), grid, block, 0, st, a); \
         else if constexpr (!RW) { \
-            if (a.mode == MODE_REFLECT) hipLaunchKernelGGL((conv_halo_x3_kernel<MODE_REFLECT, KHV, KWV, TWV, NCBV, false, TERMS>), grid, block, 0, st, a); \
-            else hipLaunchKernelGGL((conv_halo_x3_kernel<MODE_TRANSPOSED, KHV, KWV, TWV, NCBV, false, TERMS>), grid, block, 0, st, a); } } while (0)
+            if (a.mode == MODE_REFLECT) hipLaunchKernelGGL((conv_halo_x3_kernel<MODE_REFLECT, KHV, KWV, TWV, NCBV, false, TERMS, P>), grid, block, 0, st, a); \
+            else hipLaunchKernelGGL((conv_halo_x3_kernel<MODE_TRANSPOSED, KHV, KWV, TWV, NCBV, false, TERMS, P>), grid, block, 0, st, a); } } while (0)
     if (p.rowwin) PD_HALO(4, 1, 32, 2, true);
     else if (p.ncb == 1 && a.KH == 3) { if (tw == 32) PD_HALO(3, 3, 32, 1, false); else PD_HALO(3, 3, 16, 1, false); }
     else if (p.ncb == 1) PD_HALO(5, 5, 8, 1, false);
diff --git a/supervised-depth-estimation-from-polarized-images_amd/polardepth/_lib.py b/supervised-depth-estimation-from-polarized-images_amd/polardepth/_lib.py
--- a/supervised-depth-estimation-from-polarized-images_amd/polardepth/_lib.py
+++ b/supervised-depth-estimation-from-polarized-images_amd/polardepth/_lib.py
@@ -58,6 +58,9 @@
                              _i, _i, _f, _f, _l, _i, _u, _vp]),
     "pd_weight_transpose": (_i, [_vp, _vp, _i, _i, _i, _vp]),
     "pd_weight_transpose_batched": (_i, [_vp, _vp, _vp, _vp, _i, _i, _vp]),
+    "pd_weight_planes_batched": (_i, [_vp, _vp, _vp, _vp, _i, _i, _vp]),
+    "pd_conv2d_planes": (_i, [_vp, _vp, _vp, _vp, _vp, _vp, _vp, _vp, _l, _i, _i, _i, _i, _l, _l, _l, _l, _i, _i, _i, _i, _i,
+                              _i, _i, _i, _i, _l, _u, _vp]),
     "pd_stem_s2d_input": (_i, [_vp, _vp, _i, _i, _i, _i, _l, _l, _l, _l, _i, _f, _f, _vp]),
     "pd_stem_s2d_weight": (_i, [_vp, _vp, _i, _i, _vp]),
     "pd_stem_s2d_weight_grad": (_i, [_vp, _vp, _i, _i, _i, _vp]),
diff --git a/supervised-depth-estimation-from-polarized-images_amd/polardepth/engine.py b/supervised-depth-estimation-from-polarized-images_amd/polardepth/engine.py
--- a/supervised-depth-estimation-from-polarized-images_amd/polardepth/engine.py
+++ b/supervised-depth-estimation-from-polarized-images_amd/polardepth/engine.py
@@ -4,6 +4,29 @@
 import torch.distributed as dist
 
 from ._lib import lib, check, ptr, stream_ptr
+
+
+_TRACKED = {}
+
+
+def _tracked_data_class(base):
+    cls = _TRACKED.get(base)
+    if cls is None:
+        def _get(self):
+            store = self.__dict__.get("_pd_store")
+            if store is not None:
+                store._wp_serial += 1
+            return base.data.__get__(self)
+
+        def _set(self, value):
+            store = self.__dict__.get("_pd_store")
+            if store is not None:
+                store._wp_serial += 1
+            base.data.__set__(self, value)
+
+        cls = _TRACKED[base] = type(base.__name__, (base,), {"data": property(_get, _set), "_pd_tracked": True,
+                                                             "__module__": base.__module__})
+    return cls
 
 
 class ParamStore:
@@ -29,6 +52,10 @@
         self.grad = torch.zeros(total, dtype=torch.float32, device=device)
         self.grad_is_zero = True
         self._zero_version = self.grad._version
+        self._wp_serial, self._wp_launches, self._wp_param = 0, 0, {}
+        self._wp_chunk0, self._wp_rows = {}, {}
+        self._wp_tables, self._wp_buf, self._wp_listed = [None, None], [None, None], [[], []]
+        self._wp_made, self._wp_versions, self._wp_cap_done, self._wp_event = [-1, -1], [{}, {}], [False, False], [None, None]
         self.offsets = {}
         for (name, p), off in zip(self.entries, offs):
             self.offsets[name] = (off, p.numel())
@@ -40,6 +67,7 @@
             if p.dim() == 4 and p.numel() < 2 ** 31:
                 co, ci, kh, kw = p.shape
                 self._wt_index[self.flat.data_ptr() + 4 * off] = (off, co, ci, kh, kw)
+                self._wp_param[off] = p
                 rows.append([off, co, kh * kw, ci])
                 blk.append(blk[-1] + kh * kw * ((co + 31) // 32) * ((ci + 31) // 32))
         if rows:
@@ -52,6 +80,63 @@
 
     def weights_changed(self):
         self._wt_epoch = -1
+        self._wp_serial += 1
+
+    WP_CHUNK = 6144
+
+    def planes(self, w, orient):
+        e = self._wt_index.get(w.data_ptr())
+        if e is None or tuple(w.shape) != (e[1], e[2], e[3], e[4]) or not w.is_cuda:
+            return None
+        off, co, ci, kh, kw = e
+        rows, depth = (co, ci) if orient == 0 else (ci, co)
+        if depth % 16 != 0:
+            return None
+        capturing = torch.cuda.is_current_stream_capturing()
+        key = (off, orient)
+        if key not in self._wp_chunk0:
+            if capturing:
+                return None
+            self._wp_chunk0[key] = -1
+            self._wp_rows[key] = [off, rows, kh * kw, depth]
+            self._wp_tables[orient] = None
+        if not capturing:
+            self._wp_cap_done[orient] = False
+        fresh = (self._wp_tables[orient] is not None and self._wp_made[orient] == self._wp_serial
+                 and self._wp_versions[orient].get(off) == self._wp_param[off]._version
+                 and (not capturing or self._wp_cap_done[orient]))
+        if not fresh:
+            if orient == 1:
+                self.transposed(w)
+            self._wp_produce(orient, capturing)
+        else:
+            torch.cuda.current_stream().wait_event(self._wp_event[orient])
+        return self._wp_buf[orient].data_ptr() + self.WP_CHUNK * self._wp_chunk0[key]
+
+    def _wp_produce(self, orient, capturing):
+        dev = self.flat.device
+        if self._wp_tables[orient] is None:
+            rows, blk, chunk = [], [0], 0
+            for k in sorted(k for k in self._wp_rows if k[1] == orient):
+                off, r, t, d = self._wp_rows[k]
+                n = (r + 63) // 64 * (d // 16) * t
+                self._wp_chunk0[k] = chunk
+                rows.append([off, r, t, d, chunk])
+                blk.append(blk[-1] + n)
+                chunk += n
+            self._wp_tables[orient] = (torch.tensor(rows, dtype=torch.int32, device=dev),
+                                       torch.tensor(blk, dtype=torch.int32, device=dev), len(rows), blk[-1])
+            self._wp_buf[orient] = torch.empty(chunk * self.WP_CHUNK, dtype=torch.uint8, device=dev)
+            self._wp_listed[orient] = [r[0] for r in rows]
+        table, blk, n, nblocks = self._wp_tables[orient]
+        check(lib.pd_weight_planes_batched(ptr(self.flat if orient == 0 else self.flat_t), ptr(self._wp_buf[orient]), ptr(table),
+                                           ptr(blk), n, nblocks, stream_ptr()), "pd_weight_planes_batched")
+        self._wp_made[orient] = self._wp_serial
+        self._wp_versions[orient] = {o: self._wp_param[o]._version for o in self._wp_listed[orient]}
+        self._wp_cap_done[orient] = capturing
+        self._wp_launches += 1
+        self._wp_event[orient] = torch.cuda.Event()
+        self._wp_event[orient].record()
 
     def transposed(self, w):
         e = self._wt_index.get(w.data_ptr())
@@ -92,6 +177,8 @@
         p.data = pv
         p.grad = gv
         p._pd_store = self
+        if p.dim() == 4 and not getattr(type(p), "_pd_tracked", False):
+            p.__class__ = _tracked_data_class(type(p))
 
     def zero_grad(self):
         if not (self.grad_is_zero and self.grad._version == self._zero_version):
diff --git a/supervised-depth-estimation-from-polarized-images_amd/polardepth/ops.py b/supervised-depth-estimation-from-polarized-images_amd/polardepth/ops.py
--- a/supervised-depth-estimation-from-polarized-images_amd/polardepth/ops.py
+++ b/supervised-depth-estimation-from-polarized-images_amd/polardepth/ops.py
@@ -12,8 +12,11 @@
 CONV_AUTO, CONV_FP32_MFMA, CONV_BF16X3, CONV_WGRAD_SPLIT_IN_REGS, CONV_GENERAL_KERNELS, CONV_X3_IM2COL = 0, 1, 2, 4, 8, 16
 CONV_WGRAD_ROW_WORKGROUPS = 32
 CONV_BF16 = 128
+CONV_NO_WEIGHT_PLANES = 256
 CONV_FLAGS = (CONV_FP32_MFMA if os.environ.get("PD_CONV_X3", "1") == "0" else
               CONV_X3_IM2COL if os.environ.get("PD_CONV_HALO", "1") == "0" else CONV_AUTO)
+if os.environ.get("PD_WEIGHT_PLANES", "1") == "0":
+    CONV_FLAGS |= CONV_NO_WEIGHT_PLANES
 WGRAD_FLAGS = (CONV_FP32_MFMA if os.environ.get("PD_WGRAD_X3C", "1") == "0" else
                CONV_X3_IM2COL if os.environ.get("PD_CONV_HALO", "1") == "0" else
                CONV_WGRAD_ROW_WORKGROUPS if os.environ.get("PD_WGRAD_ROLL", "1") == "0" else CONV_AUTO)
@@ -135,6 +138,14 @@
                                               0, act, stream_ptr()), "pd_conv16"),
                   shape=("fwd", N, C, H, W, Co, KH, stride, mode))
         return out
+    wp = weight_planes(w, 0, N * Ho * Wo, Co, C, KH, KW, stride, pad, mode, act, out_scale is not None, Ho, Wo, CONV_FLAGS) if vec else None
+    if wp is not None:
+        _profiled(_igemm_label(N * Ho * Wo, Co, vec, "fwd", C, KH, KW, stride, pad, mode, act, out_scale is not None, (Ho, Wo)), 2.0 * N * Ho * Wo * Co * (alg_k if alg_k is not None else C * KH * KW),
+                  lambda: check(lib.pd_conv2d_planes(ptr(x), ptr(w), wp, ptr(bias), ptr(out_scale), ptr(out), ptr(stats), None, 0, N, H, W, C,
+                                                     sN, sH, sW, sC, Ho, Wo, Co, KH, KW, stride, pad, mode, act, ldy, CONV_FLAGS,
+                                                     stream_ptr()), "pd_conv2d_planes"),
+                  shape=("fwd", N, C, H, W, Co, KH, stride, mode))
+        return (out, stats) if want_stats else out
     _profiled(_igemm_label(N * Ho * Wo, Co, vec, "fwd", C, KH, KW, stride, pad, mode, act, out_scale is not None, (Ho, Wo)), 2.0 * N * Ho * Wo * Co * (alg_k if alg_k is not None else C * KH * KW),
               lambda: check(lib.pd_conv2d(ptr(x), ptr(w), ptr(bias), ptr(out_scale), ptr(out), ptr(stats), N, H, W, C, sN, sH, sW, sC,
                                           Ho, Wo, Co, KH, KW, stride, pad, mode, act, int(affine is not None), sub,
@@ -147,6 +158,25 @@
 USE_CONV16 = os.environ.get("PD_CONV16", "1") != "0"
 WT_PROVIDERS = []
 FWD_EPOCH = 0
+
+
+_PLANE_ROUTES = {}
+
+
+def weight_planes(w, orient, M, Co, C, KH, KW, stride, pad, mode, act, has_scale, Ho, Wo, flags):
+    if (flags & CONV_NO_WEIGHT_PLANES) or not WT_PROVIDERS or C % 16 != 0 or KH != KW:
+        return None
+    key = (M, Co, C, KH, stride, pad, mode, act, has_scale, Ho, Wo, flags)
+    r = _PLANE_ROUTES.get(key)
+    if r is None:
+        r = _PLANE_ROUTES[key] = (lib.pd_conv2d_route(M, Co, C, KH, KW, stride, pad, mode, act, int(has_scale), Ho, Wo, flags) & 15) == 3
+    if not r:
+        return None
+    for prov in WT_PROVIDERS:
+        a = prov.planes(w, orient)
+        if a is not None:
+            return a
+    return None
 
 
 def weight_transposed(w):
@@ -199,6 +229,18 @@
         assert addend.shape == dx.shape and addend.stride(1) == 1 and addend.is_cuda
         ld_add = addend.stride(3)
         assert addend.stride(2) == W * ld_add and addend.stride(0) == H * W * ld_add
+    wp = (weight_planes(weight_cl(w), 1, N * H * W, Ci, Co, KH, KW, stride, pad, MODE_TRANSPOSED, ACT_NONE, False, H, W, flags)
+          if sC == 1 and Co % 4 == 0 else None)
+    if wp is not None:
+        _profiled(_igemm_label(N * H * W, Ci, True, "dgrad", Co, KH, KW, stride, pad, MODE_TRANSPOSED, out_hw=(H, W), flags=flags),
+                  2.0 * N * Hy * Wy * Co * Ci * KH * KW,
+                  lambda: check(lib.pd_conv2d_planes(ptr(dy), ptr(wt), wp, None, None, ptr(dx), None, ptr(addend),
+                                                     ld_add if addend is not None else 0, N, Hy, Wy, Co, sN, sH, sW, sC, H, W, Ci,
+                                                     KH, KW, stride, pad, MODE_TRANSPOSED, ACT_NONE, Ci, flags, stream_ptr()),
+                                "pd_conv2d_planes(dgrad)"),
+                  shape=("dgrad", N, Ci, H, W, Co, KH, stride, MODE_TRANSPOSED))
+        return dx
+    if addend is not None:
         _profiled(_igemm_label(N * H * W, Ci, True, "dgrad", Co, KH, KW, stride, pad, MODE_TRANSPOSED, out_hw=(H, W), flags=flags),
                   2.0 * N * Hy * Wy * Co * Ci * KH * KW,
                   lambda: check(lib.pd_conv2d_add(ptr(dy), ptr(wt), ptr(addend), ld_add, ptr(dx), N, Hy, Wy, Co, sN, sH, sW,
```
